# KyungMinJin/OTPose

Hardware: AMD Instinct MI355X
Metric: frames/sec at 384x288, 5-frame window, batch 16; heatmap max-abs delta vs ref (higher is better)
Workload: dtype f32 storage+accumulate / f16x3 split products; 1 GPU; BASELINE configs[1]: batch 16 x 5-frame x 384x288, HRNet-W48 + DCN warp + ConvVideoTransformer, fp32 forward (eval), seeded synthetic weights; clips_per_gpu=16, parallelism=dp1, outputs_finite=True

## Files before the change

### include/otpose_hip.h

```cpp
#ifndef OTPOSE_HIP_H
#define OTPOSE_HIP_H

#include <stddef.h>

#ifdef __cplusplus
extern "C" {
#endif

#define OTP_OK 0
#define OTP_ERR_BAD_ARG (-1)
#define OTP_ERR_UNSUPPORTED (-2)
#define OTP_ERR_LAUNCH (-3)
#define OTP_ERR_WORKSPACE (-4)

#define OTP_DTYPE_F32 0
#define OTP_DTYPE_F16 1
#define OTP_DTYPE_BF16 2
#define OTP_DTYPE_F64 3

#define OTP_ACT_NONE 0
#define OTP_ACT_RELU 1
#define OTP_ACT_GELU 2

int otp_version(void);

int otp_range_flag_read(int reset);
int otp_range_poison(void* out, size_t n, void* stream);

typedef struct otp_h16_conv_desc {
    int N, Cin, H, W, Cout, stride, act;
    int in_gtot, in_goff, out_gtot, out_goff, res_gtot, res_goff;
    float out_scale;
} otp_h16_conv_desc;
size_t otp_h8_bytes(int N, int C, int H, int W);
int otp_h8_pack(const void* in_f32, void* out_h8, int N, int C, int H, int W, int in_ctot, int in_coff, int out_gtot, int out_goff,
                void* stream);
int otp_h8_unpack(const void* in_h8, void* out_f32, int N, int C, int H, int W, int in_gtot, int in_goff, void* stream);
int otp_h16_conv3x3_supported(const otp_h16_conv_desc* desc);
size_t otp_h16_conv3x3_weight_bytes(int Cout, int Cin);
int otp_h16_conv3x3_pack_weight(const void* weight, const void* scale, void* wpacked, int Cout, int Cin, float pre, void* stream);
int otp_h16_conv3x3(const void* in_h8, const void* wpacked, const void* shift, const void* res_h8, void* out_h8,
                    const otp_h16_conv_desc* desc, void* stream);
int otp_h16_pointwise_supported(int Cin, int Cout);
size_t otp_h16_pointwise_weight_bytes(int Cin, int Cout);
int otp_h16_pointwise_pack(const void* w, const void* scale, const void* shift, void* packed, int Cin, int Cout, float pre,
                           void* stream);
int otp_h16_pointwise(const void* in_h8, const void* packed, const void* res_h8, void* out, int out_f32_nchw, int N, int Cin, int Cout,
                      int HW, int in_gtot, int in_goff, int res_gtot, int res_goff, int out_tot, int out_off, int relu,
                      float out_scale, void* stream);
int otp_h16_stem_supported(int B, int F, int H, int W, int Cout);
size_t otp_h16_stem_weight_bytes(int Cout);
int otp_h16_stem_pack(const void* w, const void* scale, const void* shift, void* packed, int Cout, void* stream);
int otp_h16_stem(const void* in, const void* packed, void* out_h8, int B, int F, int H, int W, int Cout, void* stream);
int otp_h16_upsample_add(const void* const* lows_h8, const int* factors, int nlow, const void* res_h8, void* out_h8, int N, int C,
                         int Hh, int Wh, int relu, void* stream);
size_t otp_mlp_h1_weight_bytes(int C, int HID);
int otp_mlp_h1_pack(const void* w1, const void* b1, const void* w2, void* packed, int C, int HID, void* stream);
int otp_ln_mlp_h1(const void* y, const void* ln_gamma, const void* ln_beta, float ln_eps, const void* packed, const void* scale,
                  const void* shift, void* out, int B, int C, int HID, int T, void* stream);
int otp_dense_h1(const void* const* x, const void* const* packed, const void* const* res, void* const* out, int nprob, int B, int C,
                 int T, void* stream);
int otp_qkv_front_h1(const void* x, const void* table, const void* packed_q, const void* packed_k, const void* packed_v, void* q,
                     void* k, void* v, int B, int C, int T, float eps, void* stream);

int otp_mdcn_forward(const void* x, const void* offset, const void* mask, const void* weight,
                     const void* bias, void* out,
                     int N, int C, int H, int W, int Cout, int kh, int kw,
                     int stride, int pad, int dil, int groups, int deformable_groups,
                     float alpha, float beta, int dtype, void* stream);

int otp_mdcn_forward_ex(const void* x, const void* offset, const void* mask, const void* weight, const void* bias, void* out,
                        int N, int C, int H, int W, int Cout, int kh, int kw, int stride_h, int stride_w, int pad_h, int pad_w,
                        int dil_h, int dil_w, int groups, int deformable_groups, float alpha, float beta, int dtype,
                        void* stream);

size_t otp_mdcn_backward_workspace(int N, int C, int H, int W, int Cout, int kh, int kw);
size_t otp_mdcn_backward_workspace_ex(int N, int C, int H, int W, int Cout, int kh, int kw, int stride_h, int stride_w, int pad_h,
                                      int pad_w, int dil_h, int dil_w, int groups, int deformable_groups, int dtype,
                                      int has_mask);
int otp_mdcn_backward(const void* x, const void* offset, const void* mask, const void* weight,
                      const void* grad_out, void* grad_x, void* grad_offset, void* grad_mask,
                      void* grad_weight, void* grad_bias, void* workspace, size_t workspace_bytes,
                      int N, int C, int H, int W, int Cout, int kh, int kw,
                      int stride, int pad, int dil, int groups, int deformable_groups,
                      int dtype, void* stream);
int otp_mdcn_backward_ex(const void* x, const void* offset, const void* mask, const void* weight, const void* grad_out,
                         void* grad_x, void* grad_offset, void* grad_mask, void* grad_weight, void* grad_bias, void* workspace,
                         size_t workspace_bytes, int N, int C, int H, int W, int Cout, int kh, int kw, int stride_h, int stride_w,
                         int pad_h, int pad_w, int dil_h, int dil_w, int groups, int deformable_groups, int dtype, void* stream);

int otp_deform_psroi_pool_forward(const void* data, const void* rois, const void* offset, void* out, void* out_count, int N, int C,
                                  int H, int W, int num_rois, int offset_channels, int no_trans, float spatial_scale,
                                  int out_channels, int group_size, int pooled_size, int part_size, int sample_per_part,
                                  float trans_std, int dtype, void* stream);
size_t otp_deform_psroi_pool_backward_workspace(int N, int C, int H, int W, int num_rois, int offset_channels, int no_trans,
                                                int out_channels, int group_size, int pooled_size, int part_size,
                                                int sample_per_part, int dtype);
int otp_deform_psroi_pool_backward(const void* grad_out, const void* data, const void* rois, const void* offset,
                                   const void* out_count, void* grad_input, void* grad_offset, int N, int C, int H, int W,
                                   int num_rois, int offset_channels, int no_trans, float spatial_scale, int out_channels,
                                   int group_size, int pooled_size, int part_size, int sample_per_part, float trans_std,
                                   void* workspace, size_t workspace_bytes, int dtype, void* stream);

typedef struct otp_conv_desc {
    int N, Cin, H, W, Cout, kh, kw, stride, pad, dil;
    int in_ctot, in_coff, in2_ctot, in2_coff, out_ctot, out_coff;
    int res_ctot, res_coff, res_up, act, Ho, Wo, frame_split;
    float out_scale;
    int res_layout;
} otp_conv_desc;

int otp_conv2d_set_tile(int MB, int PB, int WM, int WP);
int otp_conv2d_last_plan(int* out8);
int otp_conv2d_plan(const otp_conv_desc* desc, int* out8);
int otp_conv2d_pack_weight(const void* weight, void* wpacked, int Cout, int Cin, int kh, int kw, void* stream);
int otp_conv2d(const void* in, const void* in2, const void* wpacked, const void* scale, const void* shift,
               const void* res, void* out, const otp_conv_desc* desc, void* stream);

size_t otp_conv2d_wino_weight_bytes(int Cout, int Cin);
int otp_conv2d_wino_pack_weight(const void* weight, void* upacked, int Cout, int Cin, void* stream);
int otp_conv2d_wino_supported(const otp_conv_desc* desc);
int otp_conv2d_wino_last_plan(int* out4);
int otp_conv2d_wino(const void* in, const void* upacked, const void* scale, const void* shift, const void* res, void* out,
                    const otp_conv_desc* desc, void* stream);

int otp_conv3x3_small_supported(const otp_conv_desc* desc);
size_t otp_conv3x3_small_weight_bytes(int Cout, int Cin);
int otp_conv3x3_small_pack(const void* weight, void* wpacked, int Cout, int Cin, void* stream);
int otp_conv3x3_small(const void* in, const void* in2, const void* wpacked, const void* scale, const void* shift, void* out,
                      const otp_conv_desc* desc, void* stream);

size_t otp_conv2d_x3_weight_bytes(int Cout, int Cin, int k, int stride);
int otp_conv2d_x3_pack_weight(const void* weight, const void* scale, void* wpacked, int Cout, int Cin, int k, int stride,
                              void* stream);
int otp_conv2d_x3_supported(const otp_conv_desc* desc);
int otp_conv2d_x3(const void* in, const void* wpacked, const void* shift, const void* res, void* out,
                  const otp_conv_desc* desc, void* stream);

#define OTP_S8_F32_C4 1
#define OTP_S8_F32_NCHW 2
size_t otp_s8_bytes(int N, int C, int H, int W);
int otp_s8_pack(const void* in_f32, void* out_s8, void* out_c4, int N, int C, int H, int W, int in_ctot, int in_coff, void* stream);
int otp_s8_upsample_add(const void* const* lows, const int* factors, int nlow, const void* res, void* out_nchw, void* out_s8,
                        void* out_c4, int N, int C, int Hh, int Wh, int relu, int res_ctot, int res_coff, int out_ctot,
                        int out_coff, void* stream);
int otp_s8_upsample_add_ex(const void* const* lows, const int* factors, int nlow, const void* res, int res_layout, void* out_nchw,
                           void* out_s8, void* out_c4, int N, int C, int Hh, int Wh, int relu, int res_ctot, int res_coff,
                           int out_ctot, int out_coff, void* stream);
int otp_s8_unpack(const void* in_s8, void* out_f32, int N, int C, int H, int W, void* stream);
int otp_c4_unpack(const void* in_c4, void* out_f32, int N, int C, int H, int W, void* stream);
int otp_conv3x3_s8_supported(const otp_conv_desc* desc);
size_t otp_conv3x3_s8_weight_bytes(int Cout, int Cin);
int otp_conv3x3_s8_pack_weight(const void* weight, const void* scale, void* wpacked, int Cout, int Cin, void* stream);
int otp_conv3x3_s8(const void* in_s8, const void* wpacked, const void* shift, const void* res_c4, void* out_f32,
                   int out_f32_layout, void* out_s8, const otp_conv_desc* desc, void* stream);
int otp_conv3x3_s2_s8_supported(const otp_conv_desc* desc, int nchw_out);
int otp_conv3x3_s2_s8(const void* in_s8, const void* wpacked, const void* shift, const void* res_nchw, void* out_nchw,
                      void* out_s8, const otp_conv_desc* desc, void* stream);

int otp_conv2d_pack_weight_dgrad(const void* weight, void* wpacked, int Cout, int Cin, int kh, int kw, void* stream);
int otp_dilate(const void* in, void* out, int planes, int Hi, int Wi, int s, int H, int W, void* stream);
size_t otp_conv2d_wgrad_workspace(int Cin, int Cout);
int otp_conv2d_wgrad(const void* x, const void* grad_out, void* grad_weight, int N, int Cin, int H, int W, int Cout,
                     int kh, int kw, int stride, int pad, int dil, int x_ctot, int x_coff, int dy_ctot, int dy_coff,
                     void* workspace, size_t workspace_bytes, void* stream);
size_t otp_bn_workspace(int N, int C, int HW);
int otp_bn_train_forward(const void* x, const void* gamma, const void* beta, const void* res, void* y, void* save_mean,
                         void* save_rstd, void* running_mean, void* running_var, void* workspace, size_t workspace_bytes,
                         int N, int C, int HW, float eps, float momentum, int relu, int x_ctot, int x_coff, int res_ctot,
                         int res_coff, int y_ctot, int y_coff, void* stream);
int otp_bn_train_backward(const void* grad_y, const void* x, const void* y_relu, const void* save_mean,
                          const void* save_rstd, const void* gamma, void* grad_x, void* grad_res, void* grad_gamma,
                          void* grad_beta, void* workspace, size_t workspace_bytes, int N, int C, int HW, int dy_ctot,
                          int dy_coff, int x_ctot, int x_coff, int y_ctot, int y_coff, void* stream);
int otp_channel_sum(const void* a, void* out, void* workspace, size_t workspace_bytes, int N, int C, int HW, int a_ctot,
                    int a_coff, void* stream);

int otp_dcn_fused_supported(int Cin, int J, int H, int W, int ND);
size_t otp_dcn_fused_weight_bytes(int ND, int J);
int otp_dcn_fused_pack(const void* const* w_off, const void* const* w_mask, const void* const* w_dcn, const void* const* bias,
                       void* packed, int ND, int J, void* stream);
size_t otp_dcn_fused_workspace(int B, int H, int W);
int otp_dcn_fused_forward(const void* trans, const void* x, const void* packed, void* out, void* workspace,
                          size_t workspace_bytes, int B, int Cin, int J, int H, int W, const int* dilations, int ND, float alpha,
                          void* stream);

int otp_glue_total(const void* rough, void* total, void* squeezed, void* inter, void* flow_in, const void* pe,
                   int B, int J, int HW, void* stream);
int otp_glue_stack(const void* rough, const void* margin, const void* squeezed, const void* inter,
                   const void* ctx, const void* pe1, const void* pe2, void* x1, void* x2, void* prev_b,
                   int B, int J, int HW, void* stream);

int otp_glue_total_n(const void* rough, void* total, void* squeezed, void* inter, void* flow_in, const void* pe,
                     int B, int J, int HW, int F, void* stream);
int otp_glue_stack_n(const void* rough, const void* margin, const void* squeezed, const void* inter,
                     const void* ctx, const void* pe1, const void* pe2, void* x1, void* x2, void* prev_b,
                     int B, int J, int HW, int F, void* stream);

int otp_ln_channel(const void* x, const void* gamma, const void* beta, void* y, void* pool,
                   int B, int C, int T, float eps, void* stream);
int otp_dwconv_ln3(const void* x, const void* dwq, const void* dwk, const void* dwv,
                   const void* gq, const void* bq, const void* gk, const void* bk, const void* gv, const void* bv,
                   void* q, void* k, void* v, int B, int C, int T, int stride, float eps, void* stream);
size_t otp_chan_attn_workspace(int B, int C, int T, int n_head);
int otp_chan_attn(const void* q, const void* k, const void* v, void* out, void* workspace, size_t workspace_bytes,
                  int B, int C, int T, int n_head, float scale, void* stream);
int otp_upsample_linear(const void* x, void* out, int B, int C, int T, int f, int out_ctot, int out_coff, void* stream);

int otp_mlp_fused_supported(int C, int HID, int T);
size_t otp_mlp_fused_weight_bytes(int C, int HID);
int otp_mlp_fused_pack(const void* w1, const void* b1, const void* w2, void* packed, int C, int HID, void* stream);
int otp_mlp_fused(const void* x, const void* packed, const void* scale, const void* shift, const void* res, void* out,
                  int B, int C, int HID, int T, void* stream);
int otp_ln_mlp_fused(const void* y, const void* ln_gamma, const void* ln_beta, float ln_eps, const void* packed,
                     const void* scale, const void* shift, void* out, int B, int C, int HID, int T, void* stream);

int otp_dense_x3_supported(int C, int T);
size_t otp_dense_x3_weight_bytes(int C);
int otp_dense_x3_pack(const void* w, const void* scale, const void* shift, void* packed, int C, void* stream);
int otp_dense_x3(const void* const* x, const void* const* packed, const void* const* res, void* const* out, int nprob, int B,
                 int C, int T, void* stream);
int otp_dense_x3_pack_bf16p(const void* w, const void* scale, const void* shift, void* packed, int C, void* stream);
int otp_dense_x3_bf16p(const void* const* x, const void* const* packed, const void* const* res, void* const* out, int nprob, int B,
                 int C, int T, void* stream);
int otp_qkv_front_x3(const void* x, const void* table, const void* packed_q, const void* packed_k, const void* packed_v,
                     void* q, void* k, void* v, int B, int C, int T, float eps, void* stream);

int otp_stem_conv_x3_supported(int B, int F, int H, int W, int Cout);
size_t otp_stem_conv_x3_weight_bytes(int Cout);
int otp_stem_conv_x3_pack(const void* w, const void* scale, const void* shift, void* packed, int Cout, void* stream);
int otp_stem_conv_x3(const void* in, const void* packed, void* out, int B, int F, int H, int W, int Cout, void* stream);

int otp_pointwise_x3_supported(int Cin, int Cout, int T);
size_t otp_pointwise_x3_weight_bytes(int Cin, int Cout);
int otp_pointwise_x3_pack(const void* w, const void* scale, const void* shift, void* packed, int Cin, int Cout, void* stream);
int otp_pointwise_x3(const void* x, const void* packed, const void* res, void* out, int B, int Cin, int Cout, int T, int x_ctot,
                     int x_coff, int res_ctot, int res_coff, int out_ctot, int out_coff, int relu, void* stream);
int otp_pointwise_x3_s8_supported(int Cin, int Cout, int T);
size_t otp_pointwise_x3_s8_weight_bytes(int Cin, int Cout);
int otp_pointwise_x3_s8_pack(const void* w, const void* scale, const void* shift, void* packed, int Cin, int Cout, void* stream);
int otp_pointwise_x3_s8(const void* x, const void* packed, void* out_s8, int B, int Cin, int Cout, int T, int x_ctot, int x_coff,
                        int relu, void* stream);
int otp_pointwise_x3_s8_res(const void* x, const void* packed, const void* res, void* out_s8, int B, int Cin, int Cout, int T,
                            int x_ctot, int x_coff, int r_ctot, int r_coff, int relu, void* stream);
int otp_pointwise_x3_pair_supported(int Cin, int Cmid, int Cout2, int T);
size_t otp_pointwise_x3_pair_weight_bytes(int Cin, int Cmid, int Cout2);
int otp_pointwise_x3_pair_pack(const void* w1, const void* scale1, const void* shift1, const void* w2, const void* scale2,
                               const void* shift2, void* packed, int Cin, int Cmid, int Cout2, void* stream);
int otp_pointwise_x3_pair(const void* x, const void* packed, const void* res, void* out, void* out_s8, int B, int Cin, int Cmid,
                          int Cout2, int T, int x_ctot, int x_coff, int res_ctot, int res_coff, int out_ctot, int out_coff,
                          int relu1, int relu2, void* stream);

int otp_mlp_x3_supported(int C, int HID, int T);
size_t otp_mlp_x3_weight_bytes(int C, int HID);
int otp_mlp_x3_pack(const void* w1, const void* b1, const void* w2, void* packed, int C, int HID, void* stream);
int otp_mlp_x3(const void* x, const void* packed, const void* scale, const void* shift, const void* res, void* out, int B,
               int C, int HID, int T, void* stream);
int otp_ln_mlp_x3(const void* y, const void* ln_gamma, const void* ln_beta, float ln_eps, const void* packed,
                  const void* scale, const void* shift, void* out, int B, int C, int HID, int T, void* stream);

int otp_flow_block_supported(int C, int hidden, int T);
size_t otp_flow_front_param_floats(int C);
size_t otp_flow_back_param_floats(int C, int hidden);
int otp_flow_front(const void* x, const void* params, void* q, void* k, void* v, int B, int C, int T, float eps, void* stream);
int otp_flow_back(const void* x, const void* att, const void* params, void* out, int B, int C, int hidden, int T, float eps,
                  void* stream);

int otp_dense_cc_supported(int C, int T);
size_t otp_dense_cc_weight_bytes(int C);
int otp_dense_cc_pack(const void* w, const void* scale, const void* shift, void* packed, int C, void* stream);
int otp_dense_cc(const void* const* x, const void* const* packed, const void* const* res, void* const* out, int nprob,
                 int B, int C, int T, void* stream);

size_t otp_qkv_front_table_bytes(int C);
int otp_qkv_front_pack_table(const void* dwq, const void* dwk, const void* dwv, const void* gq, const void* bq,
                             const void* gk, const void* bk, const void* gv, const void* bv, void* table, int C,
                             void* stream);
int otp_qkv_front(const void* x, const void* table, const void* packed_q, const void* packed_k, const void* packed_v,
                  void* q, void* k, void* v, int B, int C, int T, float eps, void* stream);

int otp_upsample_add(const void* low, const void* res, void* out, int N, int C, int Hl, int Wl, int f, int relu,
                     int low_ctot, int low_coff, int res_ctot, int res_coff, int out_ctot, int out_coff, void* stream);
int otp_upsample_add_multi(const void* const* lows, const int* factors, int nlow, const void* res, void* out, int N, int C,
                           int Hh, int Wh, int relu, int res_ctot, int res_coff, int out_ctot, int out_coff, void* stream);

int otp_chan_attn_set_split(int on);
int otp_chan_attn_splits(int BH, int T);
int otp_chan_attn_scores(const void* a, const void* b, void* slabs, int BH, int hs, int T, void* stream);
int otp_chan_attn_apply(const void* v, const void* M, void* out, int BH, int hs, int T, void* stream);
int otp_chan_attn_scores_bf16p(const void* a, const void* b, void* slabs, int BH, int hs, int T, void* stream);
int otp_chan_attn_apply_bf16p(const void* v, const void* M, void* out, int BH, int hs, int T, void* stream);
int otp_transpose_scale(const void* in, void* out, int batches, int R, int Cc, float scale, void* stream);
int otp_softmax_backward(const void* slabs, const void* P, void* dS, void* dST, void* PT, int BH, int hs, int NS,
                         void* stream);
int otp_ln_channel_backward(const void* x, const void* grad_y, const void* gamma, void* grad_x, void* dy_xhat, int B, int C,
                            int T, float eps, void* stream);
size_t otp_ln_channel_backward_workspace(int B, int C, int T);
int otp_ln_channel_backward_params(const void* x, const void* grad_y, const void* gamma, void* grad_x, void* grad_gamma,
                                   void* grad_beta, void* workspace, size_t workspace_bytes, int B, int C, int T, float eps,
                                   void* stream);
int otp_dwconv3_forward(const void* x, const void* w, void* y, int B, int C, int T, int stride, void* stream);
int otp_dwconv3_backward(const void* x, const void* w, const void* grad_y, void* grad_x, void* grad_w, int B, int C, int T,
                         int stride, void* stream);
int otp_gelu_forward(const void* x, void* y, size_t n, void* stream);
int otp_gelu_backward(const void* x, const void* grad_y, void* grad_x, size_t n, void* stream);
int otp_maxpool3s2_forward(const void* x, void* y, int rows, int T, void* stream);
int otp_maxpool3s2_backward(const void* x, const void* grad_y, void* grad_x, int rows, int T, void* stream);
int otp_upsample_linear_backward(const void* grad_out, void* grad_x, int B, int C, int T, int f, int out_ctot, int out_coff,
                                 void* stream);

int otp_upsample_add_backward(const void* grad_out, const void* out_relu, void* grad_res, void* grad_low, int planes, int Hl,
                              int Wl, int f, void* stream);

int otp_axpby(const void* x, void* y, float alpha, float beta, size_t n, void* stream);

int otp_heatmap_decode(const void* heatmaps, void* preds, void* maxvals, const void* center, const void* scale,
                       int N, int J, int H, int W, int refine, void* stream);

int otp_heatmap_flip_decode(const void* heatmaps, const int* perm, void* merged, void* preds, void* maxvals,
                            const void* center, const void* scale, int B, int J, int H, int W, int shift, void* stream);
int otp_clip_mirror_pair(const void* x, void* out, int B, int C, int H, int W, void* stream);

int otp_pck_accuracy(const void* pred_coords, const void* target_coords, void* acc, void* cnt, int N, int J, int H, int W,
                     float thr, void* stream);

size_t otp_grad_sumsq_scratch(void);
int otp_grad_sumsq(const void* grad, size_t n, void* acc_f64, void* stream);
int otp_adamw_step(void* param, const void* grad, void* exp_avg, void* exp_avg_sq, size_t n, float lr, float beta1,
                   float beta2, float eps, float weight_decay, int step, const void* gradnorm_sq_f64, float max_norm,
                   void* stream);

int otp_frames_u8_to_clip(const void* frames_u8, void* out, int B, int F, int H, int W, float mean_r, float mean_g,
                          float mean_b, float std_r, float std_g, float std_b, void* stream);

int otp_crop_clips_u8(const void* pool_u8, int S, int Hp, int Wp, const void* frame_idx, const void* M, const void* flip,
                      void* out, int B, int F, int H, int W, float mean_r, float mean_g, float mean_b, float std_r,
                      float std_g, float std_b, void* stream);
int otp_crop_clips_blur_u8(const void* pool_u8, int S, int Hp, int Wp, const void* frame_idx, const void* M,
                           const void* flip, void* out, int B, int F, int H, int W, float mean_r, float mean_g,
                           float mean_b, float std_r, float std_g, float std_b, const void* blur, const void* blur_on,
                           void* stream);
int otp_crop_clips_pair_u8(const void* pool_u8, int S, int Hp, int Wp, const void* frame_idx, const void* M, void* out,
                           int B, int F, int H, int W, float mean_r, float mean_g, float mean_b, float std_r, float std_g,
                           float std_b, void* stream);
int otp_pose_targets(const void* joints, const void* vis, const void* M, const void* gauss, void* target,
                     void* target_weight, int B, int J, int W, int H, int w, int h, int sigma3, void* stream);

size_t otp_loss_workspace(int B, int J);
int otp_loss_st_ohkw_grads(const void* s, const void* t, const void* g, const void* w, void* flags, void* result,
                           void* grad_s, void* grad_t, void* grad_g, void* workspace, size_t workspace_bytes, int B, int J,
                           int HW, int topk, int flags_given, void* stream);
int otp_loss_st_ohkw(const void* s, const void* t, const void* g, const void* w, void* flags,
                     void* result, void* grad_s, void* grad_t, void* workspace, size_t workspace_bytes,
                     int B, int J, int HW, int topk, int flags_given, void* stream);
int otp_loss_joints_mse(const void* o, const void* g, const void* w, void* result, void* grad_o, void* workspace,
                        size_t workspace_bytes, int B, int J, int HW, int topk, int ohkm, int effective_num_joints,
                        void* stream);


typedef struct otp_nhwc_conv_desc {
    int N, H, W, Cin, Cout, kh, kw, stride, pad, dil;
    int out_mode;
} otp_nhwc_conv_desc;
size_t otp_nhwc_conv_weight_bytes(const otp_nhwc_conv_desc* desc);
int otp_nhwc_conv_stats_rows(const otp_nhwc_conv_desc* desc);
int otp_nhwc_conv_plan(const otp_nhwc_conv_desc* desc, int* out8);
int otp_nhwc_conv_pack(const void* weight, void* wpacked, const otp_nhwc_conv_desc* desc, int dgrad, void* stream);
size_t otp_nhwc_conv_pack_job_bytes(void);
int otp_nhwc_conv_pack_job(const void* weight, void* wpacked, const otp_nhwc_conv_desc* desc, int dgrad, void* job_host);
int otp_nhwc_conv_pack_batch(const void* jobs_device, int n_jobs, void* stream);
int otp_nhwc_conv_bf16(const void* x, const void* wpacked, const void* bias, void* out, void* stats,
                       const otp_nhwc_conv_desc* desc, void* stream);
int otp_nhwc_conv_bf16_res(const void* x, const void* wpacked, const void* bias, const void* res, void* out, void* stats,
                           const otp_nhwc_conv_desc* desc, void* stream);
size_t otp_nhwc_wgrad_workspace(const otp_nhwc_conv_desc* desc);
int otp_nhwc_wgrad_bf16(const void* x, const void* grad_out, void* grad_weight, void* workspace, size_t workspace_bytes,
                        const otp_nhwc_conv_desc* desc, void* stream);
int otp_nhwc_bn_finalize(const void* partials, int rows, int C, int CS, float count, const void* gamma, const void* beta,
                         void* mean, void* rstd, void* scale, void* shift, void* running_mean, void* running_var, float eps,
                         float momentum, void* stream);
int otp_nhwc_bn_apply(const void* x, const void* scale, const void* shift, const void* res, void* y, void* relu_mask,
                      size_t pixels, int CS, int relu, void* stream);
int otp_nhwc_conv_bn_bf16(const void* x, const void* wpacked, const void* res, void* conv_out, void* stats, void* vec,
                          const void* gamma, const void* beta, void* running_mean, void* running_var, float eps, float momentum,
                          void* y, void* relu_mask, int relu, const otp_nhwc_conv_desc* desc, void* stream);
size_t otp_nhwc_bn_backward_workspace(size_t pixels, int CS);
int otp_nhwc_bn_backward(const void* gy, const void* y, const void* x, const void* mean, const void* rstd, const void* gamma,
                         void* gx, void* gres, void* dgamma, void* dbeta, void* workspace, size_t workspace_bytes,
                         size_t pixels, int C, int CS, int relu, void* stream);
int otp_nhwc_upsample_add(const void* low, const void* res, void* out, int N, int H, int W, int CS, int f, int relu,
                          void* stream);
int otp_nhwc_upsample_add_backward(const void* gy, const void* out, void* gres, void* glow, int N, int Hl, int Wl, int CS,
                                   int f, int relu, void* stream);
int otp_nchw_f32_to_nhwc_bf16(const void* in, void* out, int N, int C, int H, int W, int frame_split, void* stream);
int otp_nhwc_bf16_to_nchw_f32(const void* in, void* out, int N, int C, int H, int W, void* stream);
int otp_nhwc_dilate(const void* in, void* out, int N, int Hi, int Wi, int s, int H, int W, int CS, void* stream);


int otp_scale_residual(const void* x, const void* a, const void* scale, const void* mask, void* out, int B, int C, int T,
                       void* stream);
size_t otp_scale_residual_backward_workspace(int B, int C, int T);
int otp_scale_residual_backward(const void* grad_out, const void* a, const void* scale, const void* mask, void* grad_a,
                                void* grad_scale, void* workspace, size_t workspace_bytes, int B, int C, int T, void* stream);


size_t otp_nhwc_channel_sum_workspace(size_t pixels, int CS);
int otp_nhwc_channel_sum(const void* g, void* out, void* workspace, size_t workspace_bytes, size_t pixels, int C, int CS,
                         void* stream);
int otp_gelu_bf16_forward(const void* x, void* y, size_t n, void* stream);
int otp_gelu_bf16_backward(const void* x, const void* grad_y, void* grad_x, size_t n, void* stream);
int otp_nhwc_mlp_fused_supported(const otp_nhwc_conv_desc* desc);
int otp_nhwc_mlp_up_bf16(const void* x, const void* wpacked, const void* bias, void* pre, void* act, void* keep_bits, float p,
// ... 28 lines not shown
```

### otpose_amd/csrc/densex.hip

```cpp
#include "x3.h"
#ifndef OTP_ENTRY
#define OTP_ENTRY(name) name
#endif

namespace {

constexpr int dx_ks(int C) { return (C + 31) / 32; }
constexpr int dx_block_bytes(int C) { return (dx_ks(C) * 2 * 1024 + 128 + 4095) / 4096 * 4096; }

__global__ void densex_pack_kernel(const float* __restrict__ w, const float* __restrict__ scale, const float* __restrict__ shift,
                                   unsigned char* __restrict__ packed, int C) {
    const int KS = dx_ks(C), MT = (C + 15) / 16, BLKB = dx_block_bytes(C), units = BLKB / 16;
    const int idx = blockIdx.x * blockDim.x + threadIdx.x;
    if (idx >= MT * units) return;
    const int mt = idx / units, u = idx - mt * units;
    otp_u32x4 o = {0u, 0u, 0u, 0u};
    if (u < KS * 2 * 64) {
        const int frag = u >> 6, lane = u & 63, row = 16 * mt + (lane & 15), kq = lane >> 4, ks = frag >> 1;
        float v[8];
#pragma unroll
        for (int j = 0; j < 8; ++j) {
            const int c = 32 * ks + 8 * kq + j;
            v[j] = (row < C && c < C) ? w[(size_t)row * C + c] : 0.f;
        }
        otp_x3x8 hi, lo;
        otp_x3_split8(v, hi, lo);
        o = __builtin_bit_cast(otp_u32x4, (frag & 1) ? lo : hi);
    } else if (u < KS * 2 * 64 + 8) {
        const int k = (u - KS * 2 * 64) * 4;
        float v[4];
#pragma unroll
        for (int i = 0; i < 4; ++i) {
            const int e = k + i, c = 16 * mt + (e & 15);
            v[i] = c < C ? (e < 16 ? (scale ? scale[c] : 1.f) : (shift ? shift[c] : 0.f)) : 0.f;
        }
        o = (otp_u32x4){__builtin_bit_cast(uint32_t, v[0]), __builtin_bit_cast(uint32_t, v[1]), __builtin_bit_cast(uint32_t, v[2]),
                    __builtin_bit_cast(uint32_t, v[3])};
    }
    reinterpret_cast<otp_u32x4*>(packed)[idx] = o;
}

template <int C, bool RES, bool H1 = false>
__device__ __forceinline__ void dx_project(const otp_x3x8 (&Xh)[dx_ks(C)][2], const otp_x3x8 (&Xl)[dx_ks(C)][2],
                                           const unsigned char* __restrict__ packed, unsigned char* lds,
                                           const float* __restrict__ res, float* __restrict__ out, size_t base, int T, int tok,
                                           bool valid, unsigned* rflag) {
    constexpr int KS = dx_ks(C), MT = (C + 15) / 16, BLKB = dx_block_bytes(C);
    bool bad = false;
    const int lane = threadIdx.x & 63, kq = lane >> 4;
    const unsigned plane = (unsigned)((size_t)C * T * sizeof(float));
    const otp_rsrc ro = make_rsrc32(out + base, plane);
    const otp_rsrc rr = make_rsrc32(RES && res ? res + base : out, RES && res ? plane : 0u);
#pragma unroll 1
    for (int mt = 0; mt < MT; ++mt) {
        int voff[4];
        otp_f32x2 r[4];
#pragma unroll
        for (int i = 0; i < 4; ++i) {
            const int c = 16 * mt + 4 * kq + i;
            voff[i] = (valid && c < C) ? (c * T + tok) * 4 : -16;
            if (RES) r[i] = __builtin_bit_cast(otp_f32x2, __builtin_amdgcn_raw_buffer_load_b64(rr, voff[i], 0, 0));
        }
        asm volatile("" ::: "memory");
        if (mt + 1 < MT) otp_lds_stage<256, BLKB>(packed + (size_t)(mt + 1) * BLKB, lds + ((mt + 1) & 1) * BLKB);
        asm volatile("" ::: "memory");
        const unsigned char* P = lds + (mt & 1) * BLKB;
        otp_f32x4 acc0 = {0.f, 0.f, 0.f, 0.f}, acc1 = {0.f, 0.f, 0.f, 0.f};
#pragma unroll
        for (int ks = 0; ks < KS; ++ks) {
            const otp_x3x8 ah = *reinterpret_cast<const otp_x3x8*>(P + (ks * 2) * 1024 + lane * 16);
            if constexpr (!H1) {
                const otp_x3x8 al = *reinterpret_cast<const otp_x3x8*>(P + (ks * 2 + 1) * 1024 + lane * 16);
                acc0 = OTP_X3_MFMA(al, Xh[ks][0], acc0, 0, 0, 0);
                acc1 = OTP_X3_MFMA(al, Xh[ks][1], acc1, 0, 0, 0);
                acc0 = OTP_X3_MFMA(ah, Xl[ks][0], acc0, 0, 0, 0);
                acc1 = OTP_X3_MFMA(ah, Xl[ks][1], acc1, 0, 0, 0);
            }
            acc0 = OTP_X3_MFMA(ah, Xh[ks][0], acc0, 0, 0, 0);
            acc1 = OTP_X3_MFMA(ah, Xh[ks][1], acc1, 0, 0, 0);
        }
        const otp_f32x4 sc = *reinterpret_cast<const otp_f32x4*>(P + KS * 2048 + 16 * kq);
        const otp_f32x4 sh = *reinterpret_cast<const otp_f32x4*>(P + KS * 2048 + 64 + 16 * kq);
#pragma unroll
        for (int i = 0; i < 4; ++i) {
            otp_f32x2 v = {acc0[i] * sc[i] + sh[i], acc1[i] * sc[i] + sh[i]};
            if (RES) v += r[i];
            bad |= otp_out_of_range(v.x);
                bad |= otp_out_of_range(v.y);
            __builtin_amdgcn_raw_buffer_store_b64(__builtin_bit_cast(otp_u32x2, v), ro, voff[i], 0, 0);
        }
        if (mt + 1 < MT) {
            asm volatile("s_waitcnt vmcnt(4)" ::: "memory");
            __builtin_amdgcn_s_barrier();
            asm volatile("" ::: "memory");
        }
    }
    otp_range_report(rflag, bad, OTP_RANGE_DENSEX);
}

struct DxArgs {
    const float* x[3];
    const unsigned char* packed[3];
    const float* res[3];
    float* out[3];
};

template <int C, bool H1 = false>
__global__ __launch_bounds__(256, 2) void densex_cc_kernel(DxArgs A, int T, int tiles_per_b, unsigned* rflag) {
    constexpr int KS = dx_ks(C), BLKB = dx_block_bytes(C);
    __shared__ __attribute__((aligned(16))) unsigned char lds[2 * BLKB];
    const int tid = threadIdx.x, lane = tid & 63, wave = tid >> 6, kq = lane >> 4, n = lane & 15;
    const int b = blockIdx.x / tiles_per_b, tile = blockIdx.x - b * tiles_per_b;
    const int tok = tile * 128 + wave * 32 + 2 * n;
    const bool valid = tok < T;
    const size_t base = (size_t)b * C * T;
    const float* __restrict__ x = A.x[blockIdx.y];
    otp_lds_stage<256, BLKB>(A.packed[blockIdx.y], lds);
    otp_x3x8 Xh[KS][2], Xl[KS][2];
#pragma unroll
    for (int ks = 0; ks < KS; ++ks) {
        float v0[8], v1[8];
#pragma unroll
        for (int j = 0; j < 8; ++j) {
            const int c = 32 * ks + 8 * kq + j;
            const bool live = 32 * ks + 24 + j < C || c < C;
            const otp_f32x2 v = *reinterpret_cast<const otp_f32x2*>(x + base + (size_t)(live ? c : 0) * T + (valid ? tok : T - 2));
            v0[j] = live ? v.x : 0.f;
            v1[j] = live ? v.y : 0.f;
        }
        otp_x3_split8(v0, Xh[ks][0], Xl[ks][0]);
        otp_x3_split8(v1, Xh[ks][1], Xl[ks][1]);
    }
    __syncthreads();
    dx_project<C, true, H1>(Xh, Xl, A.packed[blockIdx.y], lds, A.res[blockIdx.y], A.out[blockIdx.y], base, T, tok, valid, rflag);
}

struct QxArgs {
    const unsigned char* packed[3];
    float* out[3];
};

template <int C, bool H1 = false>
__global__ __launch_bounds__(256, C <= 136 ? 3 : 1) void qkvx_front_kernel(const float* __restrict__ x, const float* __restrict__ table,
                                                            QxArgs A, int T, int tiles_per_b, float eps, unsigned* rflag) {
    constexpr int KS = dx_ks(C), BLKB = dx_block_bytes(C), TAB = 3 * C * 8;
    __shared__ __attribute__((aligned(16))) unsigned char lds[2 * BLKB];
    __shared__ __attribute__((aligned(16))) float tab[TAB];
    const int tid = threadIdx.x, lane = tid & 63, wave = tid >> 6, kq = lane >> 4, n = lane & 15;
    const int b = blockIdx.x / tiles_per_b, tile = blockIdx.x - b * tiles_per_b;
    const int tok = tile * 128 + wave * 32 + 2 * n;
    const bool valid = tok < T;
    const int tokc = valid ? tok : T - 2;
    const bool l_ok = tokc >= 1, r_ok = tokc + 2 < T;
    const size_t base = (size_t)b * C * T;
    const otp_rsrc rx = make_rsrc(x + base, (size_t)C * T * sizeof(float));
    constexpr float inv_c = 1.f / (float)C;
    const int vb0 = (8 * kq * T + tokc) * 4;
    for (int i = tid; i < TAB / 4; i += 256)
        reinterpret_cast<otp_f32x4*>(tab)[i] = reinterpret_cast<const otp_f32x4*>(table)[i];
    __syncthreads();

    for (int p = (int)blockIdx.y; p <= (int)blockIdx.y; ++p) {
        otp_lds_stage<256, BLKB>(A.packed[p], lds);
        const float* tp = tab + p * C * 8;
        float X0[KS][8], X1[KS][8];
        float s0 = 0.f, s1 = 0.f;
#pragma unroll
        for (int ks = 0; ks < KS; ++ks) {
#pragma unroll
            for (int j = 0; j < 8; ++j) {
                const int c = 32 * ks + 8 * kq + j;
                const bool live = 32 * ks + 24 + j < C || c < C;
                const int so = (32 * ks + j) * T * 4;
                const otp_f32x2 m = __builtin_bit_cast(otp_f32x2, __builtin_amdgcn_raw_buffer_load_b64(rx, live ? vb0 : -16, so, 0));
                const float la = bload(rx, live ? vb0 - 4 : -16, so), ld = bload(rx, live ? vb0 + 8 : -16, so);
                const float a = l_ok ? la : 0.f, d = r_ok ? ld : 0.f;
                const otp_f32x4 w = *reinterpret_cast<const otp_f32x4*>(tp + (live ? c : 0) * 8);
                X0[ks][j] = live ? w[0] * a + w[1] * m.x + w[2] * m.y : 0.f;
                X1[ks][j] = live ? w[0] * m.x + w[1] * m.y + w[2] * d : 0.f;
                s0 += X0[ks][j];
                s1 += X1[ks][j];
            }
        }
        const float m0 = otp_kslot_sum(s0) * inv_c, m1 = otp_kslot_sum(s1) * inv_c;
        float v0 = 0.f, v1 = 0.f;
#pragma unroll
        for (int ks = 0; ks < KS; ++ks)
#pragma unroll
            for (int j = 0; j < 8; ++j) {
                const bool live = 32 * ks + 24 + j < C || 32 * ks + 8 * kq + j < C;
                X0[ks][j] = live ? X0[ks][j] - m0 : 0.f;
                X1[ks][j] = live ? X1[ks][j] - m1 : 0.f;
                v0 += X0[ks][j] * X0[ks][j];
                v1 += X1[ks][j] * X1[ks][j];
            }
        const float r0 = 1.f / sqrtf(otp_kslot_sum(v0) * inv_c + eps), r1 = 1.f / sqrtf(otp_kslot_sum(v1) * inv_c + eps);
        otp_x3x8 Xh[KS][2], Xl[KS][2];
#pragma unroll
        for (int ks = 0; ks < KS; ++ks) {
#pragma unroll
            for (int j = 0; j < 8; ++j) {
                const int c = 32 * ks + 8 * kq + j;
                const bool live = 32 * ks + 24 + j < C || c < C;
                const float g = tp[(live ? c : 0) * 8 + 3], be = tp[(live ? c : 0) * 8 + 4];
                X0[ks][j] = live ? X0[ks][j] * r0 * g + be : 0.f;
                X1[ks][j] = live ? X1[ks][j] * r1 * g + be : 0.f;
            }
            otp_x3_split8(X0[ks], Xh[ks][0], Xl[ks][0]);
            otp_x3_split8(X1[ks], Xh[ks][1], Xl[ks][1]);
        }
        __syncthreads();
        dx_project<C, false, H1>(Xh, Xl, A.packed[p], lds, nullptr, A.out[p], base, T, tok, valid, rflag);
    }
}

}

#ifndef OTP_X3_GRAD_COPY
extern "C" int otp_dense_x3_supported(int C, int T) { return ((C == 136 || C == 204) && T > 0 && T % 2 == 0) ? 1 : 0; }

extern "C" size_t otp_dense_x3_weight_bytes(int C) {
    if (C <= 0 || C % 4) return 0;
    return (size_t)((C + 15) / 16) * dx_block_bytes(C);
}
#endif

extern "C" int OTP_ENTRY(otp_dense_x3_pack)(const void* w, const void* scale, const void* shift, void* packed, int C, void* stream) {
    if (!w || !packed) return OTP_ERR_BAD_ARG;
    const size_t bytes = otp_dense_x3_weight_bytes(C);
    if (!bytes) return OTP_ERR_UNSUPPORTED;
    const int total = (int)(bytes / 16);
    hipLaunchKernelGGL(densex_pack_kernel, dim3(otp_ceil_div(total, 256)), dim3(256), 0, static_cast<hipStream_t>(stream),
                       static_cast<const float*>(w), static_cast<const float*>(scale), static_cast<const float*>(shift),
                       static_cast<unsigned char*>(packed), C);
    return otp_launch_status();
}

namespace {
int dx_dense_launch(const void* const* x, const void* const* packed, const void* const* res, void* const* out, int nprob, int B, int C,
                    int T, void* stream, bool h1) {
    if (!x || !packed || !out || nprob < 1 || nprob > 3 || B <= 0) return OTP_ERR_BAD_ARG;
    if (!otp_dense_x3_supported(C, T)) return OTP_ERR_UNSUPPORTED;
    DxArgs a = {};
    for (int i = 0; i < nprob; ++i) {
        a.x[i] = static_cast<const float*>(x[i]);
        a.packed[i] = static_cast<const unsigned char*>(packed[i]);
        a.res[i] = res ? static_cast<const float*>(res[i]) : nullptr;
        a.out[i] = static_cast<float*>(out[i]);
        if (!a.x[i] || !a.packed[i] || !a.out[i]) return OTP_ERR_BAD_ARG;
        if ((reinterpret_cast<uintptr_t>(a.x[i]) | reinterpret_cast<uintptr_t>(a.res[i]) | reinterpret_cast<uintptr_t>(a.out[i])) & 7 ||
            reinterpret_cast<uintptr_t>(a.packed[i]) & 15)
            return OTP_ERR_BAD_ARG;
    }
    const int tiles = otp_ceil_div(T, 128);
    const dim3 grid((unsigned)(B * tiles), (unsigned)nprob);
    auto st = static_cast<hipStream_t>(stream);
    if (C == 204) {
        if (h1) hipLaunchKernelGGL((densex_cc_kernel<204, true>), grid, dim3(256), 0, st, a, T, tiles, otp_range_word());
        else hipLaunchKernelGGL((densex_cc_kernel<204, false>), grid, dim3(256), 0, st, a, T, tiles, otp_range_word());
    } else {
        if (h1) hipLaunchKernelGGL((densex_cc_kernel<136, true>), grid, dim3(256), 0, st, a, T, tiles, otp_range_word());
        else hipLaunchKernelGGL((densex_cc_kernel<136, false>), grid, dim3(256), 0, st, a, T, tiles, otp_range_word());
    }
    return otp_launch_status();
}
}

extern "C" int OTP_ENTRY(otp_dense_x3)(const void* const* x, const void* const* packed, const void* const* res, void* const* out,
                            int nprob, int B, int C, int T, void* stream) {
    return dx_dense_launch(x, packed, res, out, nprob, B, C, T, stream, false);
}

#ifndef OTP_X3_GRAD_COPY
extern "C" int otp_dense_h1(const void* const* x, const void* const* packed, const void* const* res, void* const* out, int nprob, int B,
                            int C, int T, void* stream) {
    return dx_dense_launch(x, packed, res, out, nprob, B, C, T, stream, true);
}
#endif

#ifndef OTP_X3_GRAD_COPY
namespace {
int dx_qkv_launch(const void* x, const void* table, const void* packed_q, const void* packed_k, const void* packed_v, void* q, void* k,
                  void* v, int B, int C, int T, float eps, void* stream, bool h1) {
    if (!x || !table || !packed_q || !packed_k || !packed_v || !q || !k || !v || B <= 0) return OTP_ERR_BAD_ARG;
    if (!otp_dense_x3_supported(C, T)) return OTP_ERR_UNSUPPORTED;
    if ((reinterpret_cast<uintptr_t>(x) | reinterpret_cast<uintptr_t>(q) | reinterpret_cast<uintptr_t>(k) |
         reinterpret_cast<uintptr_t>(v)) & 7 ||
        (reinterpret_cast<uintptr_t>(table) | reinterpret_cast<uintptr_t>(packed_q) | reinterpret_cast<uintptr_t>(packed_k) |
         reinterpret_cast<uintptr_t>(packed_v)) & 15)
        return OTP_ERR_BAD_ARG;
    if ((size_t)C * T * sizeof(float) >= (1ull << 31)) return OTP_ERR_UNSUPPORTED;
    QxArgs a;
    a.packed[0] = static_cast<const unsigned char*>(packed_q); a.packed[1] = static_cast<const unsigned char*>(packed_k);
    a.packed[2] = static_cast<const unsigned char*>(packed_v);
    a.out[0] = static_cast<float*>(q); a.out[1] = static_cast<float*>(k); a.out[2] = static_cast<float*>(v);
    const int tiles = otp_ceil_div(T, 128);
    const dim3 grid((unsigned)(B * tiles), 3u);
    auto st = static_cast<hipStream_t>(stream);
    auto xf = static_cast<const float*>(x), tf = static_cast<const float*>(table);
    if (C == 204) {
        if (h1) hipLaunchKernelGGL((qkvx_front_kernel<204, true>), grid, dim3(256), 0, st, xf, tf, a, T, tiles, eps, otp_range_word());
        else hipLaunchKernelGGL((qkvx_front_kernel<204, false>), grid, dim3(256), 0, st, xf, tf, a, T, tiles, eps, otp_range_word());
    } else {
        if (h1) hipLaunchKernelGGL((qkvx_front_kernel<136, true>), grid, dim3(256), 0, st, xf, tf, a, T, tiles, eps, otp_range_word());
        else hipLaunchKernelGGL((qkvx_front_kernel<136, false>), grid, dim3(256), 0, st, xf, tf, a, T, tiles, eps, otp_range_word());
    }
    return otp_launch_status();
}
}

extern "C" int otp_qkv_front_x3(const void* x, const void* table, const void* packed_q, const void* packed_k,
                                const void* packed_v, void* q, void* k, void* v, int B, int C, int T, float eps, void* stream) {
    return dx_qkv_launch(x, table, packed_q, packed_k, packed_v, q, k, v, B, C, T, eps, stream, false);
}

extern "C" int otp_qkv_front_h1(const void* x, const void* table, const void* packed_q, const void* packed_k,
                                const void* packed_v, void* q, void* k, void* v, int B, int C, int T, float eps, void* stream) {
    return dx_qkv_launch(x, table, packed_q, packed_k, packed_v, q, k, v, B, C, T, eps, stream, true);
}
#endif
```

### otpose_amd/csrc/mlpx.hip

```cpp
#include <math.h>
#include <stdlib.h>

#include "x3.h"

namespace {

__device__ __forceinline__ float mx_gelu_h(float x) {
    const float xc = __builtin_amdgcn_fmed3f(x, -4.2f, 4.2f), s2 = xc * xc;
    float r = 4.711542158e-11f;
    r = r * s2 + -4.627826316e-09f;
    r = r * s2 + 2.017249231e-07f;
    r = r * s2 + -5.191738396e-06f;
    r = r * s2 + 8.882890530e-05f;
    r = r * s2 + -1.080400373e-03f;
    r = r * s2 + 9.720675326e-03f;
    r = r * s2 + -6.618899545e-02f;
    r = r * s2 + 3.988157481e-01f;
    return x * (xc * r + 0.5f);
}

__device__ __forceinline__ otp_x3x8 mx_half8(const float (&v)[8]) {
    uint32_t h[4];
#pragma unroll
    for (int i = 0; i < 4; ++i) h[i] = __builtin_bit_cast(uint32_t, __builtin_convertvector((otp_f32x2){v[2 * i], v[2 * i + 1]}, otp_x3x2));
    return __builtin_bit_cast(otp_x3x8, (otp_u32x4){h[0], h[1], h[2], h[3]});
}

constexpr int mx_ks1(int C) { return (C + 31) / 32; }
constexpr int mx_mt(int C) { return (C + 15) / 16; }
constexpr int mx_w1_bytes(int C, int PS = 2) { return 2 * mx_ks1(C) * PS * 1024; }
constexpr int mx_w2_bytes(int C, int PS = 2) { return mx_mt(C) * PS * 1024; }
constexpr int mx_block_bytes(int C, int PS = 2) { return (mx_w1_bytes(C, PS) + mx_w2_bytes(C, PS) + 128 + 1023) / 1024 * 1024; }

__global__ void mlpx_pack_kernel(const float* __restrict__ w1, const float* __restrict__ b1, const float* __restrict__ w2,
                                 unsigned char* __restrict__ packed, int C, int HID, int PS) {
    const int KS1 = mx_ks1(C), W1B = mx_w1_bytes(C, PS), W2B = mx_w2_bytes(C, PS), BLKB = mx_block_bytes(C, PS);
    const int units = BLKB / 16;
    const int idx = blockIdx.x * blockDim.x + threadIdx.x;
    if (idx >= ((HID + 31) / 32) * units) return;
    const int hb = idx / units, u = idx - hb * units;
    otp_u32x4 o = {0u, 0u, 0u, 0u};
    float v[8] = {0.f, 0.f, 0.f, 0.f, 0.f, 0.f, 0.f, 0.f};
    if (u < (W1B + W2B) / 16) {
        const int frag = u >> 6, lane = u & 63, row = lane & 15, kq = lane >> 4;
        const bool lo_part = PS == 2 && (frag & 1);
        if (u < W1B / 16) {
            const int f2 = frag / PS, tile = f2 / KS1, ks = f2 - tile * KS1;
            const int hid = 32 * hb + 16 * tile + row;
#pragma unroll
            for (int j = 0; j < 8; ++j) {
                const int c = 32 * ks + 8 * kq + j;
                if (c < C && hid < HID) v[j] = w1[(size_t)hid * C + c];
            }
        } else {
            const int mt = (frag - W1B / 1024) / PS, c = 16 * mt + row;
#pragma unroll
            for (int j = 0; j < 8; ++j) {
                const int hid = 32 * hb + (j < 4 ? 4 * kq + j : 16 + 4 * kq + j - 4);
                if (c < C && hid < HID) v[j] = w2[(size_t)c * HID + hid];
            }
        }
        otp_x3x8 hi, lo;
        otp_x3_split8(v, hi, lo);
        o = __builtin_bit_cast(otp_u32x4, lo_part ? lo : hi);
    } else if (u < (W1B + W2B) / 16 + 8) {
        const int k = (u - (W1B + W2B) / 16) * 4;
        const bool in = 32 * hb + k < HID;
        o = in ? (otp_u32x4){__builtin_bit_cast(uint32_t, b1[32 * hb + k]), __builtin_bit_cast(uint32_t, b1[32 * hb + k + 1]),
                         __builtin_bit_cast(uint32_t, b1[32 * hb + k + 2]), __builtin_bit_cast(uint32_t, b1[32 * hb + k + 3])}
               : (otp_u32x4){0u, 0u, 0u, 0u};
    }
    reinterpret_cast<otp_u32x4*>(packed)[idx] = o;
}

template <int C, int HID, int NTHR, bool LN, int NT, bool H1 = false>
__device__ __forceinline__ void mlpx_pass(const float* __restrict__ x, const unsigned char* __restrict__ packed,
                                          const float* __restrict__ scale, const float* __restrict__ shift,
                                          const float* __restrict__ res, float* __restrict__ out, int T, size_t base, int tok0,
                                          unsigned char* lds, const float* __restrict__ ln_gamma,
                                          const float* __restrict__ ln_beta, float ln_eps, unsigned* rflag) {
    constexpr int KS1 = mx_ks1(C), MT = mx_mt(C), HB = (HID + 31) / 32, PS = H1 ? 1 : 2;
    constexpr int W1B = mx_w1_bytes(C, PS), W2B = mx_w2_bytes(C, PS), BLKB = mx_block_bytes(C, PS);
    const int lane = threadIdx.x & 63, kq = lane >> 4, n = lane & 15;
    const int tok = tok0 + NT * n;
    const bool valid = tok < T;

    otp_lds_stage<NTHR, BLKB>(packed, lds);

    float X[KS1][8][NT];
#pragma unroll
    for (int ks = 0; ks < KS1; ++ks)
#pragma unroll
        for (int j = 0; j < 8; ++j) {
            const int c = 32 * ks + 8 * kq + j;
            const bool live = 32 * ks + 24 + j < C || c < C;
            const float* src = x + base + (size_t)(live ? c : 0) * T + (valid ? tok : T - NT);
            if (NT == 2) {
                const otp_f32x2 v = *reinterpret_cast<const otp_f32x2*>(src);
                X[ks][j][0] = live ? v.x : 0.f;
                X[ks][j][NT - 1] = live ? v.y : 0.f;
            } else {
                X[ks][j][0] = live ? *src : 0.f;
            }
        }
    if (LN) {
        constexpr float inv_c = 1.f / (float)C;
#pragma unroll
        for (int t = 0; t < NT; ++t) {
            float s0 = 0.f;
#pragma unroll
            for (int ks = 0; ks < KS1; ++ks)
#pragma unroll
                for (int j = 0; j < 8; ++j) s0 += X[ks][j][t];
            const float m0 = otp_kslot_sum(s0) * inv_c;
            float v0 = 0.f;
#pragma unroll
            for (int ks = 0; ks < KS1; ++ks)
#pragma unroll
                for (int j = 0; j < 8; ++j) {
                    const bool live = 32 * ks + 24 + j < C || 32 * ks + 8 * kq + j < C;
                    X[ks][j][t] = live ? X[ks][j][t] - m0 : 0.f;
                    v0 += X[ks][j][t] * X[ks][j][t];
                }
            const float r0 = 1.f / sqrtf(otp_kslot_sum(v0) * inv_c + ln_eps);
#pragma unroll
            for (int ks = 0; ks < KS1; ++ks)
#pragma unroll
                for (int j = 0; j < 8; ++j) {
                    const int c = 32 * ks + 8 * kq + j;
                    const bool live = 32 * ks + 24 + j < C || c < C;
                    X[ks][j][t] = live ? X[ks][j][t] * r0 * ln_gamma[live ? c : 0] + ln_beta[live ? c : 0] : 0.f;
                }
        }
    }
    otp_x3x8 Xh[KS1][NT], Xl[H1 ? 1 : KS1][NT];
#pragma unroll
    for (int ks = 0; ks < KS1; ++ks)
#pragma unroll
        for (int t = 0; t < NT; ++t) {
            float v[8];
#pragma unroll
            for (int j = 0; j < 8; ++j) v[j] = X[ks][j][t];
            if constexpr (H1) Xh[ks][t] = mx_half8(v);
            else otp_x3_split8(v, Xh[ks][t], Xl[H1 ? 0 : ks][t]);
        }
    otp_f32x4 Y[MT][NT];
#pragma unroll
    for (int mt = 0; mt < MT; ++mt)
#pragma unroll
        for (int t = 0; t < NT; ++t) Y[mt][t] = otp_f32x4{0.f, 0.f, 0.f, 0.f};
    __syncthreads();

    for (int hb = 0; hb < HB; ++hb) {
        if (hb + 1 < HB) otp_lds_stage<NTHR, BLKB>(packed + (size_t)(hb + 1) * BLKB, lds + ((hb + 1) & 1) * BLKB);
        const unsigned char* P1 = lds + (hb & 1) * BLKB + lane * 16;
        const unsigned char* P2 = P1 + W1B;
        const float* PB = reinterpret_cast<const float*>(lds + (hb & 1) * BLKB + W1B + W2B);
        otp_f32x4 H[2][NT];
#pragma unroll
        for (int tile = 0; tile < 2; ++tile) {
#pragma unroll
            for (int t = 0; t < NT; ++t) H[tile][t] = *reinterpret_cast<const otp_f32x4*>(PB + 16 * tile + 4 * kq);
#pragma unroll
            for (int ks = 0; ks < KS1; ++ks) {
                const otp_x3x8 ah = *reinterpret_cast<const otp_x3x8*>(P1 + ((tile * KS1 + ks) * PS) * 1024);
                if constexpr (H1) {
#pragma unroll
                    for (int t = 0; t < NT; ++t) H[tile][t] = OTP_X3_MFMA(ah, Xh[ks][t], H[tile][t], 0, 0, 0);
                } else {
                    const otp_x3x8 al = *reinterpret_cast<const otp_x3x8*>(P1 + ((tile * KS1 + ks) * 2 + 1) * 1024);
#pragma unroll
                    for (int t = 0; t < NT; ++t) {
                        H[tile][t] = OTP_X3_MFMA(al, Xh[ks][t], H[tile][t], 0, 0, 0);
                        H[tile][t] = OTP_X3_MFMA(ah, Xl[H1 ? 0 : ks][t], H[tile][t], 0, 0, 0);
                        H[tile][t] = OTP_X3_MFMA(ah, Xh[ks][t], H[tile][t], 0, 0, 0);
                    }
                }
            }
        }
        otp_x3x8 Gh[NT], Gl[NT];
#pragma unroll
        for (int t = 0; t < NT; ++t) {
            if constexpr (H1) {
                const float v[8] = {mx_gelu_h(H[0][t][0]), mx_gelu_h(H[0][t][1]), mx_gelu_h(H[0][t][2]), mx_gelu_h(H[0][t][3]),
                                    mx_gelu_h(H[1][t][0]), mx_gelu_h(H[1][t][1]), mx_gelu_h(H[1][t][2]), mx_gelu_h(H[1][t][3])};
                Gh[t] = mx_half8(v);
            } else {
                const otp_f32x2 g0 = otp_gelu2(otp_f32x2{H[0][t][0], H[0][t][1]}), g1 = otp_gelu2(otp_f32x2{H[0][t][2], H[0][t][3]});
                const otp_f32x2 g2 = otp_gelu2(otp_f32x2{H[1][t][0], H[1][t][1]}), g3 = otp_gelu2(otp_f32x2{H[1][t][2], H[1][t][3]});
                const float v[8] = {g0.x, g0.y, g1.x, g1.y, g2.x, g2.y, g3.x, g3.y};
                otp_x3_split8(v, Gh[t], Gl[t]);
            }
        }
#pragma unroll
        for (int mt = 0; mt < MT; ++mt) {
            const otp_x3x8 ah = *reinterpret_cast<const otp_x3x8*>(P2 + (mt * PS) * 1024);
            if constexpr (H1) {
#pragma unroll
                for (int t = 0; t < NT; ++t) Y[mt][t] = OTP_X3_MFMA(ah, Gh[t], Y[mt][t], 0, 0, 0);
            } else {
                const otp_x3x8 al = *reinterpret_cast<const otp_x3x8*>(P2 + (mt * 2 + 1) * 1024);
#pragma unroll
                for (int t = 0; t < NT; ++t) {
                    Y[mt][t] = OTP_X3_MFMA(al, Gh[t], Y[mt][t], 0, 0, 0);
                    Y[mt][t] = OTP_X3_MFMA(ah, Gl[t], Y[mt][t], 0, 0, 0);
                    Y[mt][t] = OTP_X3_MFMA(ah, Gh[t], Y[mt][t], 0, 0, 0);
                }
            }
        }
        __syncthreads();
    }

    {
        bool bad = false;
#pragma unroll
        for (int mt = 0; mt < MT; ++mt)
#pragma unroll
            for (int t = 0; t < NT; ++t)
#pragma unroll
                for (int i = 0; i < 4; ++i) bad |= otp_out_of_range(Y[mt][t][i]);
        otp_range_report(rflag, bad, OTP_RANGE_MLPX);
    }
    if (!valid) return;
#pragma unroll
    for (int mt = 0; mt < MT; ++mt) {
#pragma unroll
        for (int i = 0; i < 4; ++i) {
            const int c = 16 * mt + 4 * kq + i;
            if (c < C) {
                const size_t o = base + (size_t)c * T + tok;
                const float sc = scale[c], sh = shift[c];
                if (NT == 2) {
                    const otp_f32x2 r = *reinterpret_cast<const otp_f32x2*>(res + o);
                    otp_f32x2 v;
                    v.x = r.x + Y[mt][0][i] * sc + sh;
                    v.y = r.y + Y[mt][NT - 1][i] * sc + sh;
                    *reinterpret_cast<otp_f32x2*>(out + o) = v;
                } else {
                    out[o] = res[o] + Y[mt][0][i] * sc + sh;
                }
            }
        }
    }
}

template <int C, int HID, int WAVES, bool LN, int NT, bool H1 = false>
__global__ __launch_bounds__(WAVES * 64, (NT == 1 && (C <= 136 || H1)) ? 4 : 2) void mlpx_kernel(
    const float* __restrict__ x, const unsigned char* __restrict__ packed, const float* __restrict__ scale,
    const float* __restrict__ shift, const float* __restrict__ res, float* __restrict__ out, int T, int tiles_per_b,
    const float* __restrict__ ln_gamma, const float* __restrict__ ln_beta, float ln_eps, unsigned* rflag) {
    extern __shared__ __attribute__((aligned(16))) unsigned char mx_lds[];
    const int wave = threadIdx.x >> 6;
    const int b = blockIdx.x / tiles_per_b, tile = blockIdx.x - b * tiles_per_b;
    mlpx_pass<C, HID, WAVES * 64, LN, NT, H1>(x, packed, scale, shift, res, out, T, (size_t)b * C * T,
                                          tile * (WAVES * 16 * NT) + wave * 16 * NT, mx_lds, ln_gamma, ln_beta, ln_eps, rflag);
}

template <int C, int HID, bool LN>
__global__ __launch_bounds__(512, 2) void mlpx_balanced_kernel(
    const float* __restrict__ x, const unsigned char* __restrict__ packed, const float* __restrict__ scale,
    const float* __restrict__ shift, const float* __restrict__ res, float* __restrict__ out, int T, int wgs_per_b,
    const float* __restrict__ ln_gamma, const float* __restrict__ ln_beta, float ln_eps, unsigned* rflag) {
    extern __shared__ __attribute__((aligned(16))) unsigned char mx_lds[];
    const int wave = __builtin_amdgcn_readfirstlane(threadIdx.x >> 6);
    const int b = blockIdx.x / wgs_per_b, part = blockIdx.x - b * wgs_per_b;
    const size_t base = (size_t)b * C * T;
    const int t0 = part * (27 * 16);
    mlpx_pass<C, HID, 512, LN, 2>(x, packed, scale, shift, res, out, T, base, t0 + wave * 32, mx_lds, ln_gamma, ln_beta, ln_eps, rflag);
    if (wave < 3) {
        mlpx_pass<C, HID, 512, LN, 2>(x, packed, scale, shift, res, out, T, base, t0 + (16 + 2 * wave) * 16, mx_lds, ln_gamma,
                                      ln_beta, ln_eps, rflag);
    } else {
        const int tile = wave == 3 ? 25 : (wave == 7 ? 26 : 18 + wave);
        mlpx_pass<C, HID, 512, LN, 1>(x, packed, scale, shift, res, out, T, base, t0 + tile * 16, mx_lds, ln_gamma, ln_beta,
                                      ln_eps, rflag);
    }
}

}

extern "C" int otp_mlp_x3_supported(int C, int HID, int T) {
    return (((C == 136 && HID == 544) || (C == 204 && HID == 816)) && T > 0 && T % 2 == 0) ? 1 : 0;
}

extern "C" size_t otp_mlp_x3_weight_bytes(int C, int HID) {
    if (C <= 0 || C % 4 || HID <= 0 || HID % 16) return 0;
    return (size_t)((HID + 31) / 32) * mx_block_bytes(C);
}

extern "C" size_t otp_mlp_h1_weight_bytes(int C, int HID) {
    if (C <= 0 || C % 4 || HID <= 0 || HID % 16) return 0;
    return (size_t)((HID + 31) / 32) * mx_block_bytes(C, 1);
}

extern "C" int otp_mlp_x3_pack(const void* w1, const void* b1, const void* w2, void* packed, int C, int HID, void* stream) {
    if (!w1 || !b1 || !w2 || !packed) return OTP_ERR_BAD_ARG;
    const size_t bytes = otp_mlp_x3_weight_bytes(C, HID);
    if (!bytes) return OTP_ERR_UNSUPPORTED;
    const int total = (int)(bytes / 16);
    hipLaunchKernelGGL(mlpx_pack_kernel, dim3(otp_ceil_div(total, 256)), dim3(256), 0, static_cast<hipStream_t>(stream),
                       static_cast<const float*>(w1), static_cast<const float*>(b1), static_cast<const float*>(w2),
                       static_cast<unsigned char*>(packed), C, HID, 2);
    return otp_launch_status();
}

extern "C" int otp_mlp_h1_pack(const void* w1, const void* b1, const void* w2, void* packed, int C, int HID, void* stream) {
    if (!w1 || !b1 || !w2 || !packed) return OTP_ERR_BAD_ARG;
    const size_t bytes = otp_mlp_h1_weight_bytes(C, HID);
    if (!bytes) return OTP_ERR_UNSUPPORTED;
    const int total = (int)(bytes / 16);
    hipLaunchKernelGGL(mlpx_pack_kernel, dim3(otp_ceil_div(total, 256)), dim3(256), 0, static_cast<hipStream_t>(stream),
                       static_cast<const float*>(w1), static_cast<const float*>(b1), static_cast<const float*>(w2),
                       static_cast<unsigned char*>(packed), C, HID, 1);
    return otp_launch_status();
}

namespace {
int mlpx_launch(const void* x, const void* packed, const void* scale, const void* shift, const void* res, void* out,
                const void* ln_gamma, const void* ln_beta, float ln_eps, int B, int C, int HID, int T, void* stream, bool h1 = false) {
    if (!x || !packed || !scale || !shift || !res || !out || B <= 0) return OTP_ERR_BAD_ARG;
    if (h1 && !ln_gamma) return OTP_ERR_UNSUPPORTED;
    if (!otp_mlp_x3_supported(C, HID, T)) return OTP_ERR_UNSUPPORTED;
    if ((reinterpret_cast<uintptr_t>(x) | reinterpret_cast<uintptr_t>(res) | reinterpret_cast<uintptr_t>(out)) & 7 ||
        reinterpret_cast<uintptr_t>(packed) & 15)
        return OTP_ERR_BAD_ARG;
    auto f = [](const void* p) { return static_cast<const float*>(p); };
    auto pk = static_cast<const unsigned char*>(packed);
    if (C == 204) {
        constexpr int WAVES = 8;
        const size_t lds204 = 2 * (size_t)mx_block_bytes(204, h1 ? 1 : 2);
        const int tiles = otp_ceil_div(T, WAVES * 16);
        auto kern = h1 ? mlpx_kernel<204, 816, WAVES, true, 1, true>
                       : (ln_gamma ? mlpx_kernel<204, 816, WAVES, true, 1> : mlpx_kernel<204, 816, WAVES, false, 1>);
        OTP_ALLOW_BIG_LDS(kern, lds204);
        hipLaunchKernelGGL(kern, dim3((unsigned)(B * tiles)), dim3(WAVES * 64), lds204, static_cast<hipStream_t>(stream), f(x), pk,
                           f(scale), f(shift), f(res), static_cast<float*>(out), T, tiles, f(ln_gamma), f(ln_beta), ln_eps, otp_range_word());
        return otp_launch_status();
    }
    const size_t lds = 2 * (size_t)mx_block_bytes(136, h1 ? 1 : 2);
    const char* bal = getenv("OTP_MLP_BALANCED");
    const bool bal_off = bal && bal[0] == '0', bal_force = bal && bal[0] == '2';
    const char* e1 = getenv("OTP_MLP_NT1");
    const bool nt1 = !(e1 && e1[0] == '0');
    if (h1 || (nt1 && !bal_force)) {
        constexpr int WAVES = 8;
        const int tiles = otp_ceil_div(T, WAVES * 16);
        auto kern = h1 ? mlpx_kernel<136, 544, WAVES, true, 1, true>
                       : (ln_gamma ? mlpx_kernel<136, 544, WAVES, true, 1> : mlpx_kernel<136, 544, WAVES, false, 1>);
        OTP_ALLOW_BIG_LDS(kern, lds);
        hipLaunchKernelGGL(kern, dim3((unsigned)(B * tiles)), dim3(WAVES * 64), lds, static_cast<hipStream_t>(stream), f(x), pk,
                           f(scale), f(shift), f(res), static_cast<float*>(out), T, tiles, f(ln_gamma), f(ln_beta), ln_eps, otp_range_word());
        return otp_launch_status();
    }
    if (!bal_off && T % (27 * 16) == 0 && (bal_force || (long)B * (T / (27 * 16)) >= 192)) {
        auto bk = ln_gamma ? mlpx_balanced_kernel<136, 544, true> : mlpx_balanced_kernel<136, 544, false>;
        OTP_ALLOW_BIG_LDS(bk, lds);
        const int per_b = T / (27 * 16);
        hipLaunchKernelGGL(bk, dim3((unsigned)(B * per_b)), dim3(512), lds, static_cast<hipStream_t>(stream), f(x), pk,
                           f(scale), f(shift), f(res), static_cast<float*>(out), T, per_b, f(ln_gamma), f(ln_beta), ln_eps, otp_range_word());
        return otp_launch_status();
    }
    constexpr int WAVES = 8;
    const int tiles = otp_ceil_div(T, WAVES * 32);
    auto kern = ln_gamma ? mlpx_kernel<136, 544, WAVES, true, 2> : mlpx_kernel<136, 544, WAVES, false, 2>;
    OTP_ALLOW_BIG_LDS(kern, lds);
    hipLaunchKernelGGL(kern, dim3((unsigned)(B * tiles)), dim3(WAVES * 64), lds, static_cast<hipStream_t>(stream), f(x), pk,
                       f(scale), f(shift), f(res), static_cast<float*>(out), T, tiles, f(ln_gamma), f(ln_beta), ln_eps, otp_range_word());
    return otp_launch_status();
}
}

extern "C" int otp_mlp_x3(const void* x, const void* packed, const void* scale, const void* shift, const void* res, void* out,
                          int B, int C, int HID, int T, void* stream) {
    return mlpx_launch(x, packed, scale, shift, res, out, nullptr, nullptr, 0.f, B, C, HID, T, stream);
}

extern "C" int otp_ln_mlp_x3(const void* y, const void* ln_gamma, const void* ln_beta, float ln_eps, const void* packed,
                             const void* scale, const void* shift, void* out, int B, int C, int HID, int T, void* stream) {
    if (!ln_gamma || !ln_beta) return OTP_ERR_BAD_ARG;
    return mlpx_launch(y, packed, scale, shift, y, out, ln_gamma, ln_beta, ln_eps, B, C, HID, T, stream);
}

extern "C" int otp_ln_mlp_h1(const void* y, const void* ln_gamma, const void* ln_beta, float ln_eps, const void* packed,
                             const void* scale, const void* shift, void* out, int B, int C, int HID, int T, void* stream) {
    if (!ln_gamma || !ln_beta) return OTP_ERR_BAD_ARG;
    return mlpx_launch(y, packed, scale, shift, y, out, ln_gamma, ln_beta, ln_eps, B, C, HID, T, stream, true);
}
```

### otpose_amd/engine.py

```python
from __future__ import annotations

import ctypes
import dataclasses
import os
import sys
import warnings
from typing import Callable, List, Optional, Tuple

import torch

from . import hip, ops
from .ops import ACT_GELU, ACT_NONE, ACT_RELU, View

def _pair(v):
    return (int(v), int(v)) if isinstance(v, int) else (int(v[0]), int(v[1]))


def plain_conv(cv, k, stride=1, pad="same", dil=1, groups=1, bias=False, cin=None, cout=None) -> bool:
    if pad == "same":
        pad = (dil or 1) * (k // 2)
    return (cv.kernel_size == (k, k) and (stride is None or cv.stride == (stride, stride))
            and (pad is None or tuple(cv.padding) == (pad, pad)) and (dil is None or tuple(cv.dilation) == (dil, dil))
            and (groups is None or cv.groups == groups) and (bias is None or (cv.bias is not None) == bias)
            and (cin is None or cv.in_channels == cin) and (cout is None or cv.out_channels == cout))


@dataclasses.dataclass(frozen=True)
class Routes:
    use_graph: bool = True
    use_winograd: bool = True
    use_x3: bool = True
    use_dcn_fused: bool = True
    use_s8: bool = True
    use_flow_fused: bool = True
    use_small_conv: bool = True
    use_fused_mlp: bool = True
    fuse_shortcut: bool = True
    fuse_upsample: bool = True
    use_dense_cc: bool = True
    use_qkv_front: bool = True
    use_pointx: bool = True
    pointx_fuse: bool = True
    pointx_any: bool = False
    multi_stream: bool = True
    f32_tail: int = 0
    h16_tail: bool = True
    range_check: str = "defer"
    s8_residual: bool = True
    s8_lazy_nchw: bool = True
    s8_stride2: bool = True
    t1_s8: bool = True
    l1_s8: bool = True
    l1_pair: bool = True
    stem_x3: bool = True
    chain_modules: bool = True
    up_any_width: bool = True
    conv_log: bool = False
    poison: Optional[Tuple[int, int]] = None
    te_serial: bool = False

    @classmethod
    def from_env(cls) -> "Routes":
        env = os.environ.get
        on = lambda name: env("OTPOSE_" + name, "1") != "0"
        x3 = env("OTPOSE_CONV_MATH", "x3") != "f32"
        poison = env("OTPOSE_POISON")
        return cls(use_graph=on("HIP_GRAPH"), use_winograd=on("WINOGRAD"), use_x3=x3, use_dcn_fused=x3 and on("DCN_FUSED"),
                   use_s8=x3 and on("S8"), use_flow_fused=on("FLOW_FUSED"), use_small_conv=on("SMALL_CONV"),
                   use_fused_mlp=on("FUSED_MLP"), fuse_shortcut=on("FUSE_SHORTCUT"), fuse_upsample=on("FUSE_UPSAMPLE"),
                   use_dense_cc=on("DENSE_CC"), use_qkv_front=on("QKV_FRONT"), use_pointx=x3 and on("POINTX"),
                   pointx_fuse=on("POINTX_FUSE"), pointx_any=env("OTPOSE_POINTX_ANY", "0") == "1", multi_stream=on("STREAMS"),
                   f32_tail=int(env("OTPOSE_F32_TAIL", "0")) if x3 else 0, h16_tail=on("H16_TAIL"),
                   range_check=env("OTPOSE_RANGE_CHECK", "defer"), s8_residual=on("S8_RESIDUAL"), s8_lazy_nchw=on("S8_LAZY_NCHW"),
                   s8_stride2=on("S8_STRIDE2"), t1_s8=on("T1_S8"), l1_s8=on("L1_S8"), l1_pair=on("L1_PAIR"), stem_x3=on("STEM_X3"),
                   chain_modules=on("CHAIN_MODULES"), up_any_width=on("UP_ANY_WIDTH"), conv_log=bool(env("OTPOSE_CONV_LOG")),
                   poison=tuple(int(v) for v in poison.split(":")) if poison else None, te_serial=env("OTPOSE_TE_SERIAL") == "1")

    @property
    def lazy_nchw(self) -> bool:
        return self.s8_residual and self.s8_lazy_nchw


class Aux:
    __slots__ = ("s8", "c4", "nchw_needed")

    def __init__(self, s8=None, c4=None, nchw_needed=False):
        self.s8, self.c4, self.nchw_needed = s8, c4, nchw_needed


class InferenceEngine:
    h16 = False

    def __init__(self, model, batch: int, device, use_graph: bool | None = None, stream_set: int = 0, inp=None, margin=None):
        routes = Routes.from_env()
        self._init(device, routes, routes.use_graph if use_graph is None else use_graph, stream_set)
        self.B = batch
        self.model = model
        cfg = model.cfg
        self.J = model.num_joints
        self.F = getattr(model, "window_frames", 5)
        self.W_img, self.H_img = cfg.MODEL.IMAGE_SIZE
        self.h, self.w = model.pe_h, model.pe_w
        self._given = (inp, margin)
        self.param_version = self._param_version()
        with torch.no_grad():
            self._build()

    def _init(self, device, routes: Routes, use_graph: bool, stream_set: int = 0):
        device = torch.device(device)
        if device.type != "cuda" or not torch.cuda.is_available():
            raise RuntimeError("otpose_amd.OTPose runs on an MI355X through libotpose_hip.so; "
                               f"got device '{device}' (there is no CPU or PyTorch-op fallback)")
        self.lib, self.dev, self.routes = hip.lib(), device, routes
        self.model, self.B, self.inp, self.margin = None, 0, None, None
        self.ops: List[Callable] = []
        self._pair_s8 = {}
        self.l1_pairs = 0
        self._aux = {}
        self._keep = []
        self._bufs = []
        self._stream = None
        self.use_graph, self.graph = use_graph, None
        self._exact = False
        self._sid = 0
        self._side = hip.side_streams(device, 3, 4 * stream_set) if routes.multi_stream else []

    @classmethod
    def bare(cls, device, multi_stream=False):
        self = cls.__new__(cls)
        self._init(device, dataclasses.replace(Routes.from_env(), multi_stream=bool(multi_stream)), use_graph=False)
        return self

    use_x3 = property(lambda self: self.routes.use_x3)
    use_dcn_fused = property(lambda self: self.routes.use_dcn_fused)
    multi_stream = property(lambda self: self.routes.multi_stream)
    f32_tail = property(lambda self: self.routes.f32_tail)
    range_check = property(lambda self: self.routes.range_check)
    half_products = property(lambda self: self.h16 and self.routes.use_x3 and self.routes.h16_tail)

    @property
    def s8_here(self) -> bool:
        return self.routes.use_s8 and not self._exact

    @property
    def s2_here(self) -> bool:
        return self.routes.use_s8 and not self._exact and self.routes.s8_stride2

    def matches(self, x) -> bool:
        return (x.shape[0] == self.B and x.device == self.dev and tuple(x.shape[2:]) == (self.H_img, self.W_img)
                and self._param_version() == self.param_version)

    def matches_shape(self, b, c, h, w, dev) -> bool:
        return (b == self.B and dev == self.dev and (h, w) == (self.H_img, self.W_img) and c == 3 * self.F
                and self._param_version() == self.param_version)

    def _param_version(self):
        ts = getattr(self, "_tracked", None)
        if ts is None:
            ts = self._tracked = list(self.model.parameters()) + list(self.model.buffers())
        v = a = 0
        for t in ts:
            v += t._version
            a ^= t.data_ptr()
        return (len(ts), v, a)

    def new(self, *shape):
        t = torch.empty(shape, dtype=torch.float32, device=self.dev)
        rng = self.routes.poison
        if rng and rng[0] <= len(self._bufs) < rng[1]:
            t.fill_(float("nan"))
        self._bufs.append(t)
        return t

    def dev_param(self, t):
        t = t.detach().to(self.dev, torch.float32).contiguous()
        self._keep.append(t)
        return t

    @staticmethod
    def winograd_pays(cin, cout):
        cout16 = (cout + 15) // 16 * 16
        if cin == 64 and cout16 == 64:
            return True
        return cin >= 32 and cin % 8 == 0 and cout16 >= 48 and ((cout16 + 47) // 48) * 48 <= 1.15 * cout16

    def _emit(self, fn):
        self.ops.append((fn, self._sid))

    def fork(self, sids):
        if not self.multi_stream:
            return
        sids = [s for s in sids if 0 < s <= len(self._side)]

        def run():
            main = torch.cuda.current_stream(self.dev)
            for s_ in sids:
                self._side[s_ - 1].wait_stream(main)
        self.ops.append((run, -1))

    def join(self, sids):
        if not self.multi_stream:
            return
        sids = [s for s in sids if 0 < s <= len(self._side)]

        def run():
            main = torch.cuda.current_stream(self.dev)
            for s_ in sids:
                main.wait_stream(self._side[s_ - 1])
        self.ops.append((run, -1))

    def on_stream(self, sid):
        self._sid = sid if (self.multi_stream and 0 <= sid <= len(self._side)) else 0

    def call(self, fn, name, *args):
        def run():
            hip.check(fn(*args, self._stream), name)
        self._emit(run)

    def call_lazy_nchw(self, aux: Aux, fn, name, args_of, unpack=None):
        full, lean = args_of(True), args_of(False)
        if unpack is None:
            def run():
                hip.check(fn(*(full if aux.nchw_needed else lean), self._stream), name)
        else:
            s8_unpack = self.lib.otp_s8_unpack

            def run():
                hip.check(fn(*lean, self._stream), name)
                if aux.nchw_needed:
                    hip.check(s8_unpack(*unpack, self._stream), "otp_s8_unpack")
        self._emit(run)

    def _bn_fold(self, bn, bias=None):
        g, b = self.dev_param(bn.weight), self.dev_param(bn.bias)
        mu, var = self.dev_param(bn.running_mean), self.dev_param(bn.running_var)
        sc = (g / torch.sqrt(var + bn.eps)).contiguous()
        sh = b - mu * sc
        if bias is not None:
            sh = sh + self.dev_param(bias) * sc
        sh = sh.contiguous()
        self._keep += [sc, sh]
        return sc, sh

    def conv(self, inp: View, weight, out: View, stride=1, pad=0, dil=1, bn=None, bias=None, act=ACT_NONE,
             res: View = None, in2: View = None, res_up=1, frame_split=0, cin=None, scale=None, shift=None):
        for v_ in (inp, in2, res):
            self._needs_nchw(v_)
        r = self.routes
        w = self.dev_param(weight)
        if w.dim() == 3:
            w = w.unsqueeze(-1)
        cout, cin_w, kh, kw = w.shape
        if bn is not None:
            sc, sh = self._bn_fold(bn, bias)
        else:
            sc = self.dev_param(scale) if scale is not None else None
            sh = shift if shift is not None else bias
            sh = self.dev_param(sh) if sh is not None else None
        d = ops.conv_desc(inp, out, cout, kh, kw, stride, pad, dil, act, in2, res, res_up, frame_split, cin)
        self._keep.append(d)
        L = self.lib
        if r.conv_log:
            route = ("x3" if r.use_x3 and in2 is None and (kh, kw) in ((3, 3), (1, 1)) and ops.x3_supported(d) else
                     "wino" if r.use_winograd and in2 is None and self.winograd_pays(cin_w, cout) and ops.wino_supported(d)
                     else "direct")
            print(f"conv {d.N}x{d.Cin}->{cout} k{kh} s{stride} p{pad} d{dil} {d.H}x{d.W} in2={in2 is not None} "
                  f"res={res is not None} up={res_up} fs={frame_split} {route}", file=sys.stderr)
        if r.use_small_conv and in2 is not None and res is None and (kh, kw) == (3, 3) and ops.small_conv_supported(d):
            wc = ops.pack_small_conv_weight(w)
            self._keep.append(wc)
# ... 335 lines not shown
                last = idx == len(terms) - 1 and not ups
                act = ACT_RELU if last else ACT_NONE
                res = xs[i] if y is None else y
                fl = mod.fuse_layers[i][j]
                tgt = y if y is not None else View(self.new(*xs[i].t.shape))
                if j > i:
                    f = 2 ** (j - i)
                    if f >= 2 and ((xs[j].t.shape[3] * f) % 4 == 0 or r.up_any_width):
                        low = self.conv_bn(xs[j], fl[0], fl[1], ACT_NONE)
                        if act == ACT_RELU and low.coff == 0 and low.C == low.ctot and self.fuse_s8([low], [f], res, tgt):
                            y = tgt
                            continue
                        self._needs_nchw(res)
                        self.call(self.lib.otp_upsample_add, "otp_upsample_add", *ops.upsample_add_args(low, res, tgt, f, act == ACT_RELU))
                        y = tgt
                    else:
                        y = self.conv_bn(xs[j], fl[0], fl[1], act, res=res, out=tgt, res_up=f)
                else:
                    chain = [(fl[k][0], fl[k][1], k < len(fl) - 1) for k in range(len(fl))]
                    if self.s2_chain_s8(chain, xs[j], act, res=res, out=tgt) is not None:
                        y = tgt
                        continue
                    t = xs[j]
                    for k in range(len(fl) - 1):
                        t = self.conv_bn(t, fl[k][0], fl[k][1], ACT_RELU)
                    y = self.conv_bn(t, fl[-1][0], fl[-1][1], act, res=res, out=tgt)
            if ups:
                res = xs[i] if y is None else y
                tgt = y if y is not None else View(self.new(*xs[i].t.shape))
                lows = [self.conv_bn(xs[j], mod.fuse_layers[i][j][0], mod.fuse_layers[i][j][1], ACT_NONE) for j in ups]
                factors = [2 ** (j - i) for j in ups]
                if self.fuse_s8(lows, factors, res, tgt):
                    outs.append(tgt)
                    continue
                self._needs_nchw(res)
                args, arrays = ops.upsample_add_multi_args(lows, factors, res, tgt, relu=True)
                self._keep += arrays
                self.call(self.lib.otp_upsample_add_multi, "otp_upsample_add_multi", *args)
                y = tgt
            outs.append(y)
        self.on_stream(0)
        if join_out:
            self.join(range(1, len(mod.fuse_layers)))
        return outs

    def hr_stages(self, net, x, width_change, new_branch, module, before_fork=None):
        ys = [x]
        for s in (2, 3, 4):
            trans = getattr(net, f"transition{s - 1}")
            live = [i for i, tr in enumerate(trans) if tr is not None]
            if before_fork is not None:
                before_fork(s, ys)
            self.fork(range(1, len(live)))
            xs = []
            for i, tr in enumerate(trans):
                if tr is None:
                    xs.append(ys[i])
                    continue
                self.on_stream(live.index(i))
                if isinstance(tr[0], torch.nn.Conv2d):
                    xs.append(width_change(s, ys[i], tr))
                else:
                    xs.append(new_branch(s, ys[-1], tr))
            self.on_stream(0)
            self.join(range(1, len(live)))
            ys = xs
            mods = list(getattr(net, f"stage{s}"))
            cont = False
            for mi, mod in enumerate(mods):
                fork_in, nxt = not cont, (mods[mi + 1] if mi + 1 < len(mods) else None)
                cont = (self.routes.chain_modules and nxt is not None and len(mod.fuse_layers) == nxt.num_branches
                        and mod.num_branches > 1)
                ys = module(s, mi, len(mods), mod, ys, fork_in, not cont)
        return ys

    def hrnet(self, net, x_in: View) -> View:
        c1 = net.conv1
        r = self.routes
        n_in, c_in, h_in, w_in = x_in.t.shape
        if (r.use_x3 and r.stem_x3 and x_in.coff == 0 and x_in.C == c_in and c_in == 3 * self.F and plain_conv(c1, 3, stride=2, cin=3)
                and ops.stem_conv_x3_supported(n_in, self.F, h_in, w_in, c1.out_channels)):
            sc, sh = self._bn_fold(net.bn1)
            pk = ops.pack_stem_conv_x3(self.dev_param(c1.weight), sc, sh)
            self._keep.append(pk)
            x = View(self.new(self.F * n_in, c1.out_channels, (h_in - 1) // 2 + 1, (w_in - 1) // 2 + 1))
            self.call(self.lib.otp_stem_conv_x3, "otp_stem_conv_x3", *ops.stem_conv_x3_args(x_in.t, pk, x.t, self.F, c1.out_channels))
        else:
            x = self.conv_bn(x_in, net.conv1, net.bn1, ACT_RELU, frame_split=self.B, cin=3)
        blocks = list(net.layer1)
        b0 = blocks[0]
        if (r.fuse_shortcut and b0.downsample is not None and plain_conv(b0.conv3, 1) and plain_conv(b0.downsample[0], 1)):
            n, _, h, w = x.t.shape
            c2 = net.conv2
            ho = (h + 2 * c2.padding[0] - c2.kernel_size[0]) // c2.stride[0] + 1
            wo = (w + 2 * c2.padding[0] - c2.kernel_size[0]) // c2.stride[0] + 1
            cx, cy = c2.out_channels, b0.conv2.out_channels
            cat = self.new(n, cx + cy, ho, wo)
            xin = self.conv_bn(x, c2, net.bn2, ACT_RELU, out=View(cat, 0, cx))
            if self.conv1_conv2_s8(xin, b0.conv1, b0.bn1, b0.conv2, b0.bn2, out=View(cat, cx, cy)) is None:
                y = self.conv_bn(xin, b0.conv1, b0.bn1, ACT_RELU)
                self.conv_bn(y, b0.conv2, b0.bn2, ACT_RELU, out=View(cat, cx, cy))

            def fold(conv, bn):
                sc, sh = self._bn_fold(bn)
                return self.dev_param(conv.weight) * sc[:, None, None, None], sh
            wd, shd = fold(b0.downsample[0], b0.downsample[1])
            w3, sh3 = fold(b0.conv3, b0.bn3)
            cout = b0.conv3.out_channels
            wcat, ones, shcat = torch.cat([wd, w3], 1), torch.ones(cout, device=self.dev), shd + sh3
            x = self.pointx_pair(View(cat), wcat, ones, shcat, None, blocks[1]) if len(blocks) > 1 else None
            if x is None:
                x = self.conv(View(cat), wcat, View(self.new(n, cout, ho, wo)), scale=ones, shift=shcat, act=ACT_RELU)
            blocks = blocks[1:]
        else:
            x = self.conv_bn(x, net.conv2, net.bn2, ACT_RELU)
        for bi, blk in enumerate(blocks):
            x = self.bottleneck(blk, x, s8_only=self.s2_here and r.t1_s8 and bi == len(blocks) - 1,
                                nxt=blocks[bi + 1] if bi + 1 < len(blocks) else None)

        def t1_s8(s):
            return s == 2 and self.s8_here and r.t1_s8

        def before_fork(s, ys):
            if (s >= 3 or t1_s8(s)) and self.s2_here:
                self.s8_image(ys[-1], want_c4=s >= 3 and not r.s8_residual)

        def width_change(s, x, tr):
            y = self.conv_bn_s8(x, tr[0], tr[1], ACT_RELU) if t1_s8(s) else None
            return y if y is not None else self.conv_bn(x, tr[0], tr[1], ACT_RELU)

        def new_branch(s, z, tr):
            zs = self.s2_chain_s8([(step[0], step[1], True) for step in tr], z, ACT_RELU) if (s >= 3 or t1_s8(s)) else None
            if zs is not None:
                return zs
            for step in tr:
                z = self.conv_bn(z, step[0], step[1], ACT_RELU)
            return z

        def module(s, mi, n_mods, mod, xs, fork_in, join_out):
            self._exact = s == 4 and mi >= n_mods - r.f32_tail
            return self.hr_module(mod, xs, fork_in, join_out)
        ys = self.hr_stages(net, x, width_change, new_branch, module, before_fork)
        fl = net.final_layer
        rough = View(self.new(self.F * self.B, self.J, self.h, self.w))
        self._exact = r.f32_tail > 0
        out = self.conv(ys[0], fl.weight, rough, 1, fl.padding[0], 1, bias=fl.bias)
        self._exact = False
        return out

    def v3(self, t3):
        b, c, t = t3.shape
        return View(t3.view(b, c, 1, t))

    def tblock(self, blk, x, stride):
        B, C, T = x.shape
        To = T if stride == 1 else (T + 2 - 3) // 2 + 1
        L = self.lib
        a = blk.attn
        r = self.routes
        if r.use_flow_fused and stride == 1 and ops.flow_block_supported(blk, C, T):
            fp, bp = ops.pack_flow_front(blk, self.dev), ops.pack_flow_back(blk, self.dev)
            self._keep += [fp, bp]
            q, k, v, att, out = (self.new(B, C, T) for _ in range(5))
            self.call(L.otp_flow_front, "otp_flow_front", *ops.flow_front_args(x, fp, q, k, v, blk.ln1.eps))
            self.chan_attn(q, k, v, att, a)
            self.call(L.otp_flow_back, "otp_flow_back", *ops.flow_back_args(x, att, bp, out, blk.mlp[0].out_channels, blk.ln2.eps))
            return out
        ln1 = self.new(B, C, T)
        skip = self.new(B, C, To) if stride > 1 else None
        p = self.dev_param
        self.call(L.otp_ln_channel, "otp_ln_channel", hip.ptr(x), hip.ptr(p(blk.ln1.weight)), hip.ptr(p(blk.ln1.bias)),
                  hip.ptr(ln1), hip.ptr(skip), B, C, T, blk.ln1.eps)
        q, k, v = self.new(B, C, To), self.new(B, C, To), self.new(B, C, To)
        dx3 = r.use_dense_cc and r.use_x3 and ops.dense_x3_supported(C, To)
        dense = dx3 or (r.use_dense_cc and ops.dense_cc_supported(C, To))
        if dense:
            packs = [ops.pack_dense_cc(m.weight.to(self.dev), None, m.bias.to(self.dev), x3=dx3)
                     for m in (a.query, a.key, a.value)]
        if dense and stride == 1 and r.use_qkv_front:
            table = ops.pack_qkv_table(*[p(t) for t in (a.query_conv.weight, a.key_conv.weight, a.value_conv.weight,
                                                         a.query_norm.weight, a.query_norm.bias, a.key_norm.weight,
                                                         a.key_norm.bias, a.value_norm.weight, a.value_norm.bias)])
            self._keep += [table, *packs]
            self.call((L.otp_qkv_front_h1 if self.half_products else L.otp_qkv_front_x3) if dx3 else L.otp_qkv_front, "otp_qkv_front",
                      *ops.qkv_front_args(ln1, table, packs, (q, k, v), a.query_norm.eps))
        else:
            qn, kn, vn = self.new(B, C, To), self.new(B, C, To), self.new(B, C, To)
            self.call(L.otp_dwconv_ln3, "otp_dwconv_ln3", hip.ptr(ln1), hip.ptr(p(a.query_conv.weight)),
                      hip.ptr(p(a.key_conv.weight)), hip.ptr(p(a.value_conv.weight)),
                      hip.ptr(p(a.query_norm.weight)), hip.ptr(p(a.query_norm.bias)),
                      hip.ptr(p(a.key_norm.weight)), hip.ptr(p(a.key_norm.bias)),
                      hip.ptr(p(a.value_norm.weight)), hip.ptr(p(a.value_norm.bias)),
                      hip.ptr(qn), hip.ptr(kn), hip.ptr(vn), B, C, T, stride, a.query_norm.eps)
            if dense:
                self.dense((qn, kn, vn), packs, None, (q, k, v), B, C, To)
            else:
                self.conv(self.v3(qn), a.query.weight, self.v3(q), bias=a.query.bias)
                self.conv(self.v3(kn), a.key.weight, self.v3(k), bias=a.key.bias)
                self.conv(self.v3(vn), a.value.weight, self.v3(v), bias=a.value.bias)
        att = self.new(B, C, To)
        self.chan_attn(q, k, v, att, a)
        sa = blk.drop_path_attn.scale.detach().reshape(-1)
        y = self.new(B, C, To)
        if dense:
            sad = sa.to(self.dev, torch.float32)
            pk = ops.pack_dense_cc(a.proj.weight.to(self.dev), sad, a.proj.bias.detach().to(self.dev) * sad,
                                   x3=r.use_x3 and ops.dense_x3_supported(C, To))
            self.dense((att,), [pk], (skip if stride > 1 else x,), (y,), B, C, To)
        else:
            self.conv(self.v3(att), a.proj.weight, self.v3(y), scale=sa,
                      shift=a.proj.bias.detach() * sa.to(a.proj.bias.device), res=self.v3(skip if stride > 1 else x))
        sm = blk.drop_path_mlp.scale.detach().reshape(-1)
        out = self.new(B, C, To)
        hid = blk.mlp[0].out_channels
        mlp_x3 = r.use_fused_mlp and r.use_x3 and ops.mlp_x3_supported(C, hid, To)
        if mlp_x3 or (r.use_fused_mlp and ops.mlp_fused_supported(C, hid, To)):
            dev = lambda t: t.detach().to(self.dev, torch.float32)
            w1, b1, w2 = dev(blk.mlp[0].weight), dev(blk.mlp[0].bias), dev(blk.mlp[3].weight)
            packed = ops.pack_mlp_x3_weights(w1, b1, w2, half=self.half_products) if mlp_x3 else ops.pack_mlp_weights(w1, b1, w2)
            scd = dev(sm).contiguous()
            shd = (dev(blk.mlp[3].bias) * scd).contiguous()
            self._keep += [packed, scd, shd]
            fn, name = ((L.otp_ln_mlp_h1 if self.half_products else L.otp_ln_mlp_x3, "otp_ln_mlp_x3") if mlp_x3
                        else (L.otp_ln_mlp_fused, "otp_ln_mlp_fused"))
            self.call(fn, name, *ops.ln_mlp_args(y, p(blk.ln2.weight), p(blk.ln2.bias), blk.ln2.eps, packed, scd, shd, out, hid))
            return out
        ln2 = self.new(B, C, To)
        self.call(L.otp_ln_channel, "otp_ln_channel", hip.ptr(y), hip.ptr(p(blk.ln2.weight)), hip.ptr(p(blk.ln2.bias)),
                  hip.ptr(ln2), None, B, C, To, blk.ln2.eps)
        hdn = self.new(B, 4 * C, To)
        self.conv(self.v3(ln2), blk.mlp[0].weight, self.v3(hdn), bias=blk.mlp[0].bias, act=ACT_GELU)
        self.conv(self.v3(hdn), blk.mlp[3].weight, self.v3(out), scale=sm,
                  shift=blk.mlp[3].bias.detach() * sm.to(blk.mlp[3].bias.device), res=self.v3(y))
        return out

    def chan_attn(self, q, k, v, att, a):
        B, C, T = q.shape
        nbytes = self.lib.otp_chan_attn_workspace(B, C, T, a.n_head)
        ws = self.new(max(nbytes // 4, 1))
        self.call(self.lib.otp_chan_attn, "otp_chan_attn", *ops.chan_attn_args(q, k, v, att, ws, nbytes, a.n_head, a.scale))

    def conv_transformer(self, ct, x, stacked):
        _, C, T = x.shape
        L = self.lib
        for blk in ct.stem:
            x = self.tblock(blk, x, 1)
        self.call(L.otp_upsample_linear, "otp_upsample_linear", *ops.upsample_linear_args(x, stacked, 1, 0))
        for i, blk in enumerate(ct.branch):
            x = self.tblock(blk, x, 2)
            f = 2 ** (i + 1)
            if x.shape[2] * f != T:
                raise RuntimeError("heat-map size must make every pyramid level divide evenly (T % 4 == 0)")
            self.call(L.otp_upsample_linear, "otp_upsample_linear", *ops.upsample_linear_args(x, stacked, f, (i + 1) * C))

    def rsb_block(self, blk, x: View) -> View:
        n, _, h, w = x.t.shape
        bc = blk.branch_ch
        cbr = lambda m, inp, out, act, in2=None, res=None: self.conv(
            inp, m.conv.weight, out, 1, m.conv.padding[0], 1, bn=m.bn, bias=m.conv.bias, act=act, in2=in2, res=res)
        t = self.new(n, 4 * bc, h, w)
        cat = self.new(n, 4 * bc, h, w)
        cbr(blk.conv_bn_relu1, x, View(t), ACT_RELU)
        s = [View(t, i * bc, bc) for i in range(4)]
        tmp = lambda: View(self.new(n, bc, h, w))
        par = self.multi_stream and self._sid == 0
        side = (lambda: (self.fork((1,)), self.on_stream(1))) if par else (lambda: None)
        main = (lambda: self.on_stream(0)) if par else (lambda: None)
        o11 = cbr(blk.conv_bn_relu2_1_1, s[0], View(cat, 0, bc), ACT_RELU)
        o21 = cbr(blk.conv_bn_relu2_2_1, s[1], tmp(), ACT_RELU, in2=o11)
        side()
        o22 = cbr(blk.conv_bn_relu2_2_2, o21, View(cat, bc, bc), ACT_RELU)
        main()
        o31 = cbr(blk.conv_bn_relu2_3_1, s[2], tmp(), ACT_RELU, in2=o21)
        side()
        o32 = cbr(blk.conv_bn_relu2_3_2, o31, tmp(), ACT_RELU, in2=o22)
        main()
        o41 = cbr(blk.conv_bn_relu2_4_1, s[3], tmp(), ACT_RELU, in2=o31)
        if par:
            self.join((1,))
        o42 = cbr(blk.conv_bn_relu2_4_2, o41, tmp(), ACT_RELU, in2=o32)
        if par:
            self.on_stream(1)
        o33 = cbr(blk.conv_bn_relu2_3_3, o32, View(cat, 2 * bc, bc), ACT_RELU)
        if par:
            self.on_stream(0)
            self.join((1,))
        o43 = cbr(blk.conv_bn_relu2_4_3, o42, tmp(), ACT_RELU, in2=o33)
        cbr(blk.conv_bn_relu2_4_4, o43, View(cat, 3 * bc, bc), ACT_RELU)
        res = x
        if blk.downsample is not None:
            res = cbr(blk.downsample, x, View(self.new(n, blk.conv_bn_relu3.conv.out_channels, h, w)), ACT_NONE)
        out = View(self.new(n, blk.conv_bn_relu3.conv.out_channels, h, w))
        return cbr(blk.conv_bn_relu3, View(cat), out, ACT_RELU, res=res)

    def rsb_chain(self, chain, x: View) -> View:
        for blk in chain.layers:
            x = self.rsb_block(blk, x)
        return x

    def _build(self):
        m, B, J, h, w = self.model, self.B, self.J, self.h, self.w
        L, T = self.lib, self.h * self.w
        self.inp = self._given[0] if self._given[0] is not None else self.new(B, 3 * self.F, self.H_img, self.W_img)
        self.margin = self._given[1] if self._given[1] is not None else self.new(B, self.F - 1)
        assert tuple(self.inp.shape) == (B, 3 * self.F, self.H_img, self.W_img) and self.inp.is_contiguous()
        rough = self.hrnet(m.rough_pose_estimation_net, View(self.inp)).t
        self.hr_end = len(self.ops)

        total, squeezed, inter = self.new(B, J, h, w), self.new(B, J, h, w), self.new(B, J, h, w)
        flow_in = self.new(B, J, T)
        pe_f = self.dev_param(m.flow_encoder.pos_embd[0, :, :T])
        self.call(L.otp_glue_total_n, "otp_glue_total", hip.ptr(rough), hip.ptr(total), hip.ptr(squeezed), hip.ptr(inter),
                  hip.ptr(flow_in), hip.ptr(pe_f), B, J, T, self.F)
        ctx = self.new(B, J, T)
        self.fork((2,))
        self.on_stream(2)
        def_h = self.rsb_chain(m.def_fuse, View(total))
        self.on_stream(0)
        self.conv_transformer(m.flow_encoder, flow_in, ctx)
        D = m.num_frames * J
        x1, x2, prev_b = self.new(B, D, T), self.new(B, D, T), self.new(B, J, h, w)
        pe1 = self.dev_param(m.temporal_encoder1.pos_embd[0, :, :T])
        pe2 = self.dev_param(m.temporal_encoder2.pos_embd[0, :, :T])
        self.call(L.otp_glue_stack_n, "otp_glue_stack", hip.ptr(rough), hip.ptr(self.margin), hip.ptr(squeezed),
                  hip.ptr(inter), hip.ptr(ctx), hip.ptr(pe1), hip.ptr(pe2), hip.ptr(x1), hip.ptr(x2), hip.ptr(prev_b),
                  B, J, T, self.F)
        levels = m.scale_arch[-1] + 1
        cs_ = levels * D
        cpad = (-cs_) % 32 if (self.use_x3 and m.final_layer1.kernel_size == (1, 1)) else 0
        s1, s2 = self.new(B, cs_ + cpad, T), self.new(B, cs_ + cpad, T)
        if cpad:
            s1[:, cs_:].zero_()
            s2[:, cs_:].zero_()
        cat3 = self.new(B, 3 * J, h, w)
        def final(fl, s, i):
            wt = fl.weight
            if cpad:
                wt = torch.cat([wt.detach().to(self.dev, torch.float32),
                                torch.zeros(wt.shape[0], cpad, 1, 1, device=self.dev)], 1)
            self.conv(View(s.view(B, cs_ + cpad, h, w)), wt, View(cat3, i * J, J), 1, fl.padding[0], 1, bias=fl.bias)

        self.on_stream(2)
        self.copy_into(def_h, View(cat3, 2 * J, J))
        self.on_stream(0)
        self.fork((1,))
        self.conv_transformer(m.temporal_encoder1, x1, s1)
        final(m.final_layer1, s1, 0)
        self.on_stream(0 if self.routes.te_serial else 1)
        self.conv_transformer(m.temporal_encoder2, x2, s2)
        final(m.final_layer2, s2, 1)
        self.on_stream(0)
        self.join((1, 2))
        trans = self.rsb_chain(m.offset_mask_combine_conv, View(cat3))
        out = self.new(B, J, h, w)
        nd = len(m.deformable_conv_dilations)
        dils = [int(d) for d in m.deformable_conv_dilations]
        cin_t = trans.C
        if (self.use_dcn_fused and trans.coff == 0 and trans.C == trans.ctot and ops.dcn_fused_supported(cin_t, J, h, w, nd)
                and all(plain_conv(c[0], 3, dil=d, groups=None) for cs in (m.offsets_list, m.masks_list) for c, d in zip(cs, dils))
                and all(tuple(mm.deform_conv.weight.shape) == (J, J, 3, 3) and mm.deform_conv.deformable_groups == J
                        and mm.deform_conv.groups == 1 and _pair(mm.deform_conv.stride) == (1, 1)
                        and _pair(mm.deform_conv.padding) == (d, d) == _pair(mm.deform_conv.dilation)
                        for mm, d in zip(m.modulated_deform_conv_list, dils))):
            dcs = [mm.deform_conv for mm in m.modulated_deform_conv_list]
            packed = ops.pack_dcn_fused([self.dev_param(c[0].weight) for c in m.offsets_list],
                                        [self.dev_param(c[0].weight) for c in m.masks_list],
                                        [self.dev_param(dc.weight) for dc in dcs],
                                        [None if dc.bias is None else self.dev_param(dc.bias) for dc in dcs])
            ws = self.new(int(L.otp_dcn_fused_workspace(B, h, w)) // 4)
            dl = (ctypes.c_int * nd)(*dils)
            self._keep += [packed, dl]
            self.call(L.otp_dcn_fused_forward, "otp_dcn_fused_forward", hip.ptr(trans.t), hip.ptr(def_h.t), hip.ptr(packed),
                      hip.ptr(out), hip.ptr(ws), ws.numel() * 4, B, cin_t, J, h, w, dl, nd, 1.0 / nd)
            self._finish(out, rough, inter, prev_b, ctx, squeezed, total)
            return
        off_buf, msk_buf = self.new(B, J * 18, h, w), self.new(B, J * 9, h, w)
        for i, d in enumerate(m.deformable_conv_dilations):
            self.conv(trans, m.offsets_list[i][0].weight, View(off_buf), 1, d, d)
            self.conv(trans, m.masks_list[i][0].weight, View(msk_buf), 1, d, d)
            dc = m.modulated_deform_conv_list[i].deform_conv
            wt, bs = self.dev_param(dc.weight), self.dev_param(dc.bias)
            self.call(L.otp_mdcn_forward, "otp_mdcn_forward", hip.ptr(def_h.t), hip.ptr(off_buf), hip.ptr(msk_buf),
                      hip.ptr(wt), hip.ptr(bs), hip.ptr(out), B, J, h, w, J, 3, 3, 1, d, d, 1, J,
                      1.0 / nd, 0.0 if i == 0 else 1.0, 0)
        self._finish(out, rough, inter, prev_b, ctx, squeezed, total)

    def _finish(self, out, rough, inter, prev_b, ctx, squeezed, total):
        B, J, h, w = self.B, self.J, self.h, self.w
        if self.use_x3 or self.h16:
            self.call(self.lib.otp_range_poison, "otp_range_poison", hip.ptr(out), out.numel())
        self.outputs = (out, rough, inter, prev_b, ctx.view(B, J, h, w), squeezed, total)
        torch.cuda.synchronize(self.dev)

    _RANGE_KERNELS = {1: "convx (3x3 / 1x1 convolutions from fp32 NCHW)", 2: "convs (BasicBlock convolutions on S8 records)",
                      3: "convs2 (stride-2 convolutions on S8 records)", 4: "pointx (1x1 convolutions)", 5: "stem convolution",
                      6: "S8 conversion / fuse passes", 7: "mlpx (TransformerBlock MLP)", 8: "densex (q / k / v / proj projections)",
                      9: "channel attention", 10: "dcn_fused (warping head)", 11: "fp16 engine kernels"}

    def _raise_range(self, code):
        raise FloatingPointError(
            "otpose_amd: a value left the range of the half-precision operand pieces (|x| >= 65504, or a non-finite sum) in the "
            f"{self._RANGE_KERNELS.get(code, 'kernel family %d' % code)} of an eval forward; the heat-maps of that forward were "
# ... 68 lines not shown
```

### otpose_amd/hip.py

```python
from __future__ import annotations

import ctypes
import os
import threading
from ctypes import c_float, c_int, c_size_t, c_void_p

_HERE = os.path.dirname(os.path.abspath(__file__))
LIB_PATH = os.environ.get("OTPOSE_HIP_LIB") or os.path.join(_HERE, "csrc", "libotpose_hip.so")
_lib = None
_tls = threading.local()

OTP_OK = 0
_ERRORS = {
    -1: "OTP_ERR_BAD_ARG (null pointer or non-positive dimension)",
    -2: "OTP_ERR_UNSUPPORTED (shape / dtype / stride combination not implemented)",
    -3: "OTP_ERR_LAUNCH (HIP launch error)",
    -4: "OTP_ERR_WORKSPACE (workspace too small)",
}


class ConvDesc(ctypes.Structure):
    _fields_ = [(n, c_int) for n in (
        "N", "Cin", "H", "W", "Cout", "kh", "kw", "stride", "pad", "dil",
        "in_ctot", "in_coff", "in2_ctot", "in2_coff", "out_ctot", "out_coff",
        "res_ctot", "res_coff", "res_up", "act", "Ho", "Wo", "frame_split")] + [("out_scale", ctypes.c_float), ("res_layout", ctypes.c_int)]


class NhwcConvDesc(ctypes.Structure):
    _fields_ = [(n, c_int) for n in ("N", "H", "W", "Cin", "Cout", "kh", "kw", "stride", "pad", "dil", "out_mode")]


_ND = ctypes.POINTER(NhwcConvDesc)


class H16ConvDesc(ctypes.Structure):
    _fields_ = [(n, c_int) for n in ("N", "Cin", "H", "W", "Cout", "stride", "act", "in_gtot", "in_goff", "out_gtot", "out_goff",
                                     "res_gtot", "res_goff")] + [("out_scale", ctypes.c_float)]


_HD = ctypes.POINTER(H16ConvDesc)

SIGNATURES = {
    "otp_version": (c_int, []),
    "otp_range_flag_read": (c_int, [c_int]),
    "otp_range_poison": (c_int, [c_void_p, c_size_t, c_void_p]),
    "otp_h8_bytes": (c_size_t, [c_int] * 4),
    "otp_h8_pack": (c_int, [c_void_p, c_void_p] + [c_int] * 8 + [c_void_p]),
    "otp_h8_unpack": (c_int, [c_void_p, c_void_p] + [c_int] * 6 + [c_void_p]),
    "otp_h16_conv3x3_supported": (c_int, [_HD]),
    "otp_h16_conv3x3_weight_bytes": (c_size_t, [c_int, c_int]),
    "otp_h16_conv3x3_pack_weight": (c_int, [c_void_p] * 3 + [c_int, c_int, c_float, c_void_p]),
    "otp_h16_conv3x3": (c_int, [c_void_p] * 5 + [_HD, c_void_p]),
    "otp_h16_pointwise_supported": (c_int, [c_int, c_int]),
    "otp_h16_pointwise_weight_bytes": (c_size_t, [c_int, c_int]),
    "otp_h16_pointwise_pack": (c_int, [c_void_p] * 4 + [c_int, c_int, c_float, c_void_p]),
    "otp_h16_pointwise": (c_int, [c_void_p] * 4 + [c_int] * 12 + [c_float, c_void_p]),
    "otp_h16_stem_supported": (c_int, [c_int] * 5),
    "otp_h16_stem_weight_bytes": (c_size_t, [c_int]),
    "otp_h16_stem_pack": (c_int, [c_void_p] * 4 + [c_int, c_void_p]),
    "otp_h16_stem": (c_int, [c_void_p] * 3 + [c_int] * 5 + [c_void_p]),
    "otp_mlp_h1_weight_bytes": (c_size_t, [c_int] * 2),
    "otp_mlp_h1_pack": (c_int, [c_void_p] * 4 + [c_int] * 2 + [c_void_p]),
    "otp_ln_mlp_h1": (c_int, [c_void_p] * 3 + [c_float] + [c_void_p] * 4 + [c_int] * 4 + [c_void_p]),
    "otp_dense_h1": (c_int, [ctypes.POINTER(c_void_p)] * 4 + [c_int] * 4 + [c_void_p]),
    "otp_qkv_front_h1": (c_int, [c_void_p] * 8 + [c_int] * 3 + [c_float, c_void_p]),
    "otp_h16_upsample_add": (c_int, [ctypes.POINTER(c_void_p), ctypes.POINTER(c_int), c_int, c_void_p, c_void_p] + [c_int] * 5 + [c_void_p]),
    "otp_mdcn_forward": (c_int, [c_void_p] * 6 + [c_int] * 12 + [c_float, c_float, c_int, c_void_p]),
    "otp_mdcn_forward_ex": (c_int, [c_void_p] * 6 + [c_int] * 15 + [c_float, c_float, c_int, c_void_p]),
    "otp_mdcn_backward_ex": (c_int, [c_void_p] * 10 + [c_void_p, c_size_t] + [c_int] * 15 + [c_int, c_void_p]),
    "otp_mdcn_backward_workspace": (c_size_t, [c_int] * 7),
    "otp_mdcn_backward_workspace_ex": (c_size_t, [c_int] * 17),
    "otp_mdcn_backward": (c_int, [c_void_p] * 10 + [c_void_p, c_size_t] + [c_int] * 12 + [c_int, c_void_p]),
    "otp_deform_psroi_pool_forward": (c_int, [c_void_p] * 5 + [c_int] * 7 + [c_float] + [c_int] * 5 + [c_float, c_int, c_void_p]),
    "otp_deform_psroi_pool_backward_workspace": (c_size_t, [c_int] * 13),
    "otp_deform_psroi_pool_backward": (c_int, [c_void_p] * 7 + [c_int] * 7 + [c_float] + [c_int] * 5 + [c_float]
                                       + [c_void_p, c_size_t, c_int, c_void_p]),
    "otp_conv2d_pack_weight": (c_int, [c_void_p, c_void_p, c_int, c_int, c_int, c_int, c_void_p]),
    "otp_conv2d": (c_int, [c_void_p] * 7 + [ctypes.POINTER(ConvDesc), c_void_p]),
    "otp_conv2d_wino_weight_bytes": (c_size_t, [c_int, c_int]),
    "otp_conv2d_wino_pack_weight": (c_int, [c_void_p, c_void_p, c_int, c_int, c_void_p]),
    "otp_conv2d_wino_supported": (c_int, [ctypes.POINTER(ConvDesc)]),
    "otp_conv2d_wino_last_plan": (c_int, [ctypes.POINTER(c_int)]),
    "otp_conv2d_wino": (c_int, [c_void_p] * 6 + [ctypes.POINTER(ConvDesc), c_void_p]),
    "otp_conv3x3_small_supported": (c_int, [ctypes.POINTER(ConvDesc)]),
    "otp_conv3x3_small_weight_bytes": (c_size_t, [c_int, c_int]),
    "otp_conv3x3_small_pack": (c_int, [c_void_p, c_void_p, c_int, c_int, c_void_p]),
    "otp_conv3x3_small": (c_int, [c_void_p] * 6 + [ctypes.POINTER(ConvDesc), c_void_p]),
    "otp_conv2d_x3_weight_bytes": (c_size_t, [c_int, c_int, c_int, c_int]),
    "otp_conv2d_x3_pack_weight": (c_int, [c_void_p, c_void_p, c_void_p, c_int, c_int, c_int, c_int, c_void_p]),
    "otp_conv2d_x3_supported": (c_int, [ctypes.POINTER(ConvDesc)]),
    "otp_conv2d_x3": (c_int, [c_void_p] * 5 + [ctypes.POINTER(ConvDesc), c_void_p]),
    "otp_s8_bytes": (c_size_t, [c_int] * 4),
    "otp_s8_pack": (c_int, [c_void_p] * 3 + [c_int] * 6 + [c_void_p]),
    "otp_s8_upsample_add": (c_int, [ctypes.POINTER(c_void_p), ctypes.POINTER(c_int), c_int] + [c_void_p] * 4 + [c_int] * 9 + [c_void_p]),
    "otp_s8_upsample_add_ex": (c_int, [ctypes.POINTER(c_void_p), ctypes.POINTER(c_int), c_int, c_void_p, c_int] + [c_void_p] * 3
                               + [c_int] * 9 + [c_void_p]),
    "otp_s8_unpack": (c_int, [c_void_p, c_void_p] + [c_int] * 4 + [c_void_p]),
    "otp_c4_unpack": (c_int, [c_void_p, c_void_p] + [c_int] * 4 + [c_void_p]),
    "otp_conv3x3_s8_supported": (c_int, [ctypes.POINTER(ConvDesc)]),
    "otp_conv3x3_s8_weight_bytes": (c_size_t, [c_int, c_int]),
    "otp_conv3x3_s8_pack_weight": (c_int, [c_void_p] * 3 + [c_int, c_int, c_void_p]),
    "otp_conv3x3_s8": (c_int, [c_void_p] * 5 + [c_int, c_void_p, ctypes.POINTER(ConvDesc), c_void_p]),
    "otp_conv3x3_s2_s8_supported": (c_int, [ctypes.POINTER(ConvDesc), c_int]),
    "otp_conv3x3_s2_s8": (c_int, [c_void_p] * 6 + [ctypes.POINTER(ConvDesc), c_void_p]),
    "otp_conv2d_set_tile": (c_int, [c_int] * 4),
    "otp_conv2d_last_plan": (c_int, [ctypes.POINTER(c_int)]),
    "otp_conv2d_plan": (c_int, [ctypes.POINTER(ConvDesc), ctypes.POINTER(c_int)]),
    "otp_conv2d_pack_weight_dgrad": (c_int, [c_void_p, c_void_p, c_int, c_int, c_int, c_int, c_void_p]),
    "otp_dilate": (c_int, [c_void_p, c_void_p] + [c_int] * 6 + [c_void_p]),
    "otp_grad_sumsq_scratch": (c_size_t, []),
    "otp_grad_sumsq": (c_int, [c_void_p, c_size_t, c_void_p, c_void_p]),
    "otp_adamw_step": (c_int, [c_void_p] * 4 + [c_size_t] + [c_float] * 5 + [c_int, c_void_p, c_float, c_void_p]),
    "otp_pck_accuracy": (c_int, [c_void_p] * 4 + [c_int] * 4 + [c_float, c_void_p]),
    "otp_frames_u8_to_clip": (c_int, [c_void_p] * 2 + [c_int] * 4 + [c_float] * 6 + [c_void_p]),
    "otp_crop_clips_u8": (c_int, [c_void_p] + [c_int] * 3 + [c_void_p] * 4 + [c_int] * 4 + [c_float] * 6 + [c_void_p]),
    "otp_crop_clips_blur_u8": (c_int, [c_void_p] + [c_int] * 3 + [c_void_p] * 4 + [c_int] * 4 + [c_float] * 6
                               + [c_void_p] * 3),
    "otp_crop_clips_pair_u8": (c_int, [c_void_p] + [c_int] * 3 + [c_void_p] * 3 + [c_int] * 4 + [c_float] * 6 + [c_void_p]),
    "otp_pose_targets": (c_int, [c_void_p] * 6 + [c_int] * 7 + [c_void_p]),
    "otp_conv2d_wgrad_workspace": (c_size_t, [c_int] * 2),
    "otp_conv2d_wgrad": (c_int, [c_void_p] * 3 + [c_int] * 14 + [c_void_p, c_size_t, c_void_p]),
    "otp_bn_workspace": (c_size_t, [c_int] * 3),
    "otp_bn_train_forward": (c_int, [c_void_p] * 9 + [c_void_p, c_size_t] + [c_int] * 3 + [c_float, c_float] +
                             [c_int] * 7 + [c_void_p]),
    "otp_bn_train_backward": (c_int, [c_void_p] * 10 + [c_void_p, c_size_t] + [c_int] * 9 + [c_void_p]),
    "otp_channel_sum": (c_int, [c_void_p, c_void_p, c_void_p, c_size_t] + [c_int] * 5 + [c_void_p]),
    "otp_glue_total": (c_int, [c_void_p] * 6 + [c_int] * 3 + [c_void_p]),
    "otp_glue_stack": (c_int, [c_void_p] * 10 + [c_int] * 3 + [c_void_p]),
    "otp_glue_total_n": (c_int, [c_void_p] * 6 + [c_int] * 4 + [c_void_p]),
    "otp_glue_stack_n": (c_int, [c_void_p] * 10 + [c_int] * 4 + [c_void_p]),
    "otp_ln_channel": (c_int, [c_void_p] * 5 + [c_int] * 3 + [c_float, c_void_p]),
    "otp_dwconv_ln3": (c_int, [c_void_p] * 13 + [c_int] * 4 + [c_float, c_void_p]),
    "otp_chan_attn_workspace": (c_size_t, [c_int] * 4),
    "otp_dense_cc_supported": (c_int, [c_int] * 2),
    "otp_dense_cc_weight_bytes": (c_size_t, [c_int]),
    "otp_dense_cc_pack": (c_int, [c_void_p] * 4 + [c_int, c_void_p]),
    "otp_dense_cc": (c_int, [ctypes.POINTER(c_void_p)] * 4 + [c_int] * 4 + [c_void_p]),
    "otp_qkv_front_table_bytes": (c_size_t, [c_int]),
    "otp_qkv_front_pack_table": (c_int, [c_void_p] * 10 + [c_int, c_void_p]),
    "otp_qkv_front": (c_int, [c_void_p] * 8 + [c_int] * 3 + [c_float, c_void_p]),
    "otp_mlp_fused_supported": (c_int, [c_int] * 3),
    "otp_mlp_fused_weight_bytes": (c_size_t, [c_int] * 2),
    "otp_mlp_fused_pack": (c_int, [c_void_p] * 4 + [c_int] * 2 + [c_void_p]),
    "otp_mlp_fused": (c_int, [c_void_p] * 6 + [c_int] * 4 + [c_void_p]),
    "otp_ln_mlp_fused": (c_int, [c_void_p] * 3 + [c_float] + [c_void_p] * 4 + [c_int] * 4 + [c_void_p]),
    "otp_dcn_fused_supported": (c_int, [c_int] * 5),
    "otp_dcn_fused_weight_bytes": (c_size_t, [c_int] * 2),
    "otp_dcn_fused_pack": (c_int, [c_void_p] * 5 + [c_int, c_int, c_void_p]),
    "otp_dcn_fused_workspace": (c_size_t, [c_int] * 3),
    "otp_dcn_fused_forward": (c_int, [c_void_p] * 5 + [c_size_t] + [c_int] * 5 + [ctypes.POINTER(c_int), c_int, c_float, c_void_p]),
    "otp_dense_x3_supported": (c_int, [c_int] * 2),
    "otp_dense_x3_weight_bytes": (c_size_t, [c_int]),
    "otp_dense_x3_pack": (c_int, [c_void_p] * 4 + [c_int, c_void_p]),
    "otp_dense_x3": (c_int, [ctypes.POINTER(c_void_p)] * 4 + [c_int] * 4 + [c_void_p]),
    "otp_dense_x3_pack_bf16p": (c_int, [c_void_p] * 4 + [c_int, c_void_p]),
    "otp_dense_x3_bf16p": (c_int, [ctypes.POINTER(c_void_p)] * 4 + [c_int] * 4 + [c_void_p]),
    "otp_stem_conv_x3_supported": (c_int, [c_int] * 5),
    "otp_stem_conv_x3_weight_bytes": (c_size_t, [c_int]),
    "otp_stem_conv_x3_pack": (c_int, [c_void_p] * 4 + [c_int, c_void_p]),
    "otp_stem_conv_x3": (c_int, [c_void_p] * 3 + [c_int] * 5 + [c_void_p]),
    "otp_pointwise_x3_supported": (c_int, [c_int] * 3),
    "otp_pointwise_x3_weight_bytes": (c_size_t, [c_int] * 2),
    "otp_pointwise_x3_pack": (c_int, [c_void_p] * 4 + [c_int, c_int, c_void_p]),
    "otp_pointwise_x3": (c_int, [c_void_p] * 4 + [c_int] * 11 + [c_void_p]),
    "otp_pointwise_x3_s8_supported": (c_int, [c_int] * 3),
    "otp_pointwise_x3_s8_weight_bytes": (c_size_t, [c_int] * 2),
    "otp_pointwise_x3_s8_pack": (c_int, [c_void_p] * 4 + [c_int, c_int, c_void_p]),
    "otp_pointwise_x3_s8": (c_int, [c_void_p] * 3 + [c_int] * 7 + [c_void_p]),
    "otp_pointwise_x3_s8_res": (c_int, [c_void_p] * 4 + [c_int] * 9 + [c_void_p]),
    "otp_pointwise_x3_pair_supported": (c_int, [c_int] * 4),
    "otp_pointwise_x3_pair_weight_bytes": (c_size_t, [c_int] * 3),
    "otp_pointwise_x3_pair_pack": (c_int, [c_void_p] * 7 + [c_int] * 3 + [c_void_p]),
    "otp_pointwise_x3_pair": (c_int, [c_void_p] * 5 + [c_int] * 13 + [c_void_p]),
    "otp_qkv_front_x3": (c_int, [c_void_p] * 8 + [c_int] * 3 + [c_float, c_void_p]),
    "otp_mlp_x3_supported": (c_int, [c_int] * 3),
    "otp_mlp_x3_weight_bytes": (c_size_t, [c_int] * 2),
    "otp_mlp_x3_pack": (c_int, [c_void_p] * 4 + [c_int] * 2 + [c_void_p]),
    "otp_mlp_x3": (c_int, [c_void_p] * 6 + [c_int] * 4 + [c_void_p]),
    "otp_flow_block_supported": (c_int, [c_int] * 3),
    "otp_flow_front_param_floats": (c_size_t, [c_int]),
    "otp_flow_back_param_floats": (c_size_t, [c_int, c_int]),
    "otp_flow_front": (c_int, [c_void_p] * 5 + [c_int] * 3 + [c_float, c_void_p]),
    "otp_flow_back": (c_int, [c_void_p] * 4 + [c_int] * 4 + [c_float, c_void_p]),
    "otp_ln_mlp_x3": (c_int, [c_void_p] * 3 + [c_float] + [c_void_p] * 4 + [c_int] * 4 + [c_void_p]),
    "otp_chan_attn": (c_int, [c_void_p] * 4 + [c_void_p, c_size_t] + [c_int] * 4 + [c_float, c_void_p]),
    "otp_chan_attn_splits": (c_int, [c_int, c_int]),
    "otp_chan_attn_scores": (c_int, [c_void_p] * 3 + [c_int] * 3 + [c_void_p]),
    "otp_chan_attn_set_split": (c_int, [c_int]),
    "otp_chan_attn_apply": (c_int, [c_void_p] * 3 + [c_int] * 3 + [c_void_p]),
    "otp_chan_attn_scores_bf16p": (c_int, [c_void_p] * 3 + [c_int] * 3 + [c_void_p]),
    "otp_chan_attn_apply_bf16p": (c_int, [c_void_p] * 3 + [c_int] * 3 + [c_void_p]),
    "otp_transpose_scale": (c_int, [c_void_p, c_void_p, c_int, c_int, c_int, c_float, c_void_p]),
    "otp_softmax_backward": (c_int, [c_void_p] * 5 + [c_int] * 3 + [c_void_p]),
    "otp_ln_channel_backward": (c_int, [c_void_p] * 5 + [c_int] * 3 + [c_float, c_void_p]),
    "otp_ln_channel_backward_workspace": (c_size_t, [c_int] * 3),
    "otp_ln_channel_backward_params": (c_int, [c_void_p] * 6 + [c_void_p, c_size_t] + [c_int] * 3 + [c_float, c_void_p]),
    "otp_dwconv3_forward": (c_int, [c_void_p] * 3 + [c_int] * 4 + [c_void_p]),
    "otp_dwconv3_backward": (c_int, [c_void_p] * 5 + [c_int] * 4 + [c_void_p]),
    "otp_gelu_forward": (c_int, [c_void_p, c_void_p, c_size_t, c_void_p]),
    "otp_gelu_backward": (c_int, [c_void_p] * 3 + [c_size_t, c_void_p]),
    "otp_maxpool3s2_forward": (c_int, [c_void_p, c_void_p, c_int, c_int, c_void_p]),
    "otp_maxpool3s2_backward": (c_int, [c_void_p] * 3 + [c_int, c_int, c_void_p]),
    "otp_upsample_linear_backward": (c_int, [c_void_p, c_void_p] + [c_int] * 6 + [c_void_p]),
    "otp_upsample_linear": (c_int, [c_void_p, c_void_p] + [c_int] * 6 + [c_void_p]),
    "otp_upsample_add": (c_int, [c_void_p] * 3 + [c_int] * 12 + [c_void_p]),
    "otp_upsample_add_multi": (c_int, [ctypes.POINTER(c_void_p), ctypes.POINTER(c_int), c_int, c_void_p, c_void_p] + [c_int] * 9 + [c_void_p]),
    "otp_upsample_add_backward": (c_int, [c_void_p] * 4 + [c_int] * 4 + [c_void_p]),
    "otp_axpby": (c_int, [c_void_p, c_void_p, c_float, c_float, c_size_t, c_void_p]),
    "otp_heatmap_decode": (c_int, [c_void_p] * 5 + [c_int] * 5 + [c_void_p]),
    "otp_heatmap_flip_decode": (c_int, [c_void_p] * 7 + [c_int] * 5 + [c_void_p]),
    "otp_clip_mirror_pair": (c_int, [c_void_p] * 2 + [c_int] * 4 + [c_void_p]),
    "otp_loss_workspace": (c_size_t, [c_int, c_int]),
    "otp_loss_st_ohkw_grads": (c_int, [c_void_p] * 9 + [c_void_p, c_size_t] + [c_int] * 5 + [c_void_p]),
    "otp_loss_st_ohkw": (c_int, [c_void_p] * 8 + [c_void_p, c_size_t] + [c_int] * 5 + [c_void_p]),
    "otp_nhwc_conv_weight_bytes": (c_size_t, [_ND]),
    "otp_nhwc_conv_stats_rows": (c_int, [_ND]),
    "otp_nhwc_conv_plan": (c_int, [_ND, ctypes.POINTER(c_int)]),
    "otp_nhwc_conv_pack": (c_int, [c_void_p, c_void_p, _ND, c_int, c_void_p]),
    "otp_nhwc_conv_pack_job_bytes": (c_size_t, []),
    "otp_nhwc_conv_pack_job": (c_int, [c_void_p, c_void_p, _ND, c_int, c_void_p]),
    "otp_nhwc_conv_pack_batch": (c_int, [c_void_p, c_int, c_void_p]),
    "otp_nhwc_conv_bf16": (c_int, [c_void_p] * 5 + [_ND, c_void_p]),
    "otp_nhwc_conv_bf16_res": (c_int, [c_void_p, c_void_p, c_void_p, c_void_p, c_void_p, c_void_p, _ND, c_void_p]),
    "otp_nhwc_wgrad_workspace": (c_size_t, [_ND]),
    "otp_nhwc_wgrad_bf16": (c_int, [c_void_p] * 4 + [c_size_t, _ND, c_void_p]),
    "otp_nhwc_bn_finalize": (c_int, [c_void_p, c_int, c_int, c_int, c_float] + [c_void_p] * 8 + [c_float, c_float, c_void_p]),
    "otp_nhwc_bn_apply": (c_int, [c_void_p] * 6 + [c_size_t, c_int, c_int, c_void_p]),
    "otp_nhwc_bn_backward_workspace": (c_size_t, [c_size_t, c_int]),
    "otp_nhwc_bn_backward": (c_int, [c_void_p] * 11 + [c_size_t, c_size_t, c_int, c_int, c_int, c_void_p]),
    "otp_nhwc_upsample_add": (c_int, [c_void_p] * 3 + [c_int] * 6 + [c_void_p]),
    "otp_nhwc_upsample_add_backward": (c_int, [c_void_p] * 4 + [c_int] * 6 + [c_void_p]),
    "otp_nchw_f32_to_nhwc_bf16": (c_int, [c_void_p, c_void_p] + [c_int] * 5 + [c_void_p]),
    "otp_nhwc_bf16_to_nchw_f32": (c_int, [c_void_p, c_void_p] + [c_int] * 4 + [c_void_p]),
    "otp_nhwc_dilate": (c_int, [c_void_p, c_void_p] + [c_int] * 7 + [c_void_p]),
    "otp_scale_residual": (c_int, [c_void_p] * 5 + [c_int] * 3 + [c_void_p]),
    "otp_scale_residual_backward_workspace": (c_size_t, [c_int] * 3),
    "otp_scale_residual_backward": (c_int, [c_void_p] * 7 + [c_size_t] + [c_int] * 3 + [c_void_p]),
    "otp_nhwc_channel_sum_workspace": (c_size_t, [c_size_t, c_int]),
    "otp_nhwc_channel_sum": (c_int, [c_void_p] * 3 + [c_size_t, c_size_t, c_int, c_int, c_void_p]),
    "otp_gelu_bf16_forward": (c_int, [c_void_p, c_void_p, c_size_t, c_void_p]),
    "otp_gelu_bf16_backward": (c_int, [c_void_p] * 3 + [c_size_t, c_void_p]),
    "otp_nhwc_conv_bn_bf16": (c_int, [c_void_p] * 10 + [ctypes.c_float, ctypes.c_float, c_void_p, c_void_p, c_int, _ND, c_void_p]),
    "otp_nhwc_mlp_fused_supported": (c_int, [_ND]),
    "otp_nhwc_mlp_up_bf16": (c_int, [c_void_p] * 6 + [ctypes.c_float, ctypes.c_ulonglong, _ND, c_void_p]),
    "otp_nhwc_mlp_down_dgrad_bf16": (c_int, [c_void_p] * 5 + [ctypes.c_float, _ND, c_void_p]),
    "otp_gelu_dropout_bf16_forward": (c_int, [c_void_p] * 3 + [c_size_t, ctypes.c_float, ctypes.c_ulonglong, c_void_p]),
    "otp_gelu_dropout_bf16_backward": (c_int, [c_void_p] * 4 + [c_size_t, ctypes.c_float, c_void_p]),
    "otp_loss_joints_mse": (c_int, [c_void_p] * 5 + [c_void_p, c_size_t] + [c_int] * 6 + [c_void_p]),
    "otp_pose_assign": (c_int, [c_void_p] * 12 + [ctypes.c_double] + [c_void_p] * 3 + [c_int] * 4 + [c_void_p]),
    "otp_ap_curve": (c_int, [c_void_p] * 6 + [c_int, c_void_p]),
    "otp_pose_nms": (c_int, [c_void_p] * 6 + [ctypes.POINTER(ctypes.c_double)] + [ctypes.c_double] * 3 + [c_int] * 2
                     + [c_void_p] * 4 + [c_int] * 3 + [c_void_p]),
}


def lib():
    global _lib
    if _lib is None:
        if not os.path.isfile(LIB_PATH):
            raise RuntimeError(
                f"HIP library {LIB_PATH} is missing - run `python -c 'import __graft_entry__ as g; g.build()'` "
                "(or `make -C otpose_amd/csrc`). otpose_amd has no CPU or PyTorch-op fallback.")
        cdll = ctypes.CDLL(LIB_PATH)
        for name, (res, args) in SIGNATURES.items():
            fn = getattr(cdll, name)
            fn.restype = res
            fn.argtypes = args
        cdll.otp_chan_attn_set_split(0 if os.environ.get("OTPOSE_CONV_MATH", "x3") == "f32" else 1)
        import torch
        if torch.cuda.is_available():
            cdll.otp_range_flag_read(0)
        _lib = _DeviceGuarded(cdll)
    return _lib


class _DeviceGuarded:

    def __init__(self, cdll):
        self._cdll = cdll
        for name in SIGNATURES:
            setattr(self, name, self._wrap(getattr(cdll, name)))

    @staticmethod
    def _wrap(fn):
        import torch

        cur = getattr(torch._C, "_cuda_getDevice", None) or torch.cuda.current_device

        def call(*args):
            dev = getattr(_tls, "dev", None)
            if dev is not None and dev != cur():
                with torch.cuda.device(dev):
                    return fn(*args)
            return fn(*args)
        return call


def check(status: int, what: str):
    if status != OTP_OK:
        raise RuntimeError(f"{what} failed: {_ERRORS.get(status, status)}")


def ptr(t):
    return None if t is None else c_void_p(t.data_ptr())


def stream_of(t):
    import torch
    dev = t.device.index
    _tls.dev = dev
    raw = getattr(torch._C, "_cuda_getCurrentRawStream", None)
    if raw is not None:
        return c_void_p(raw(dev))
    return c_void_p(torch.cuda.current_stream(t.device).cuda_stream)


_SIDE_STREAMS = {}


def side_streams(device, n, first=0):
    import torch
    device = torch.device(device)
    if device.index is None:
        device = torch.device("cuda", torch.cuda.current_device())
    pool = _SIDE_STREAMS.setdefault(device, [])
    while len(pool) < first + n:
        pool.append(torch.cuda.Stream(device))
    return pool[first:first + n]
```

### otpose_amd/ops.py

```python
from __future__ import annotations

import ctypes
import math
import os

import torch
from torch.autograd import Function

from . import hip
from .augment import FLIP_PAIRS

_DTYPE_F32 = 0


def _require_gpu(*tensors):
    for t in tensors:
        if t is not None and not t.is_cuda:
            raise NotImplementedError("otpose_amd operators run on the GPU only (no CPU path)")


def _check_f32(*tensors):
    for t in tensors:
        if t is not None and t.dtype != torch.float32:
            raise RuntimeError(f"otpose_amd HIP operators are built for float32, got {t.dtype}")
# ... 471 lines not shown
    rv = View(res.contiguous()) if res is not None else None
    d = conv_desc(iv, ov, cout, k, k, stride, pad, dil, act, None, rv)
    e = x3_weight_exponent(weight, scale)
    d.out_scale = 2.0 ** -e
    conv2d_x3_launch(iv, pack_x3_weight(weight, scale, stride, e), shift, ov, d, rv)
    return out


S8_F32_C4, S8_F32_NCHW = 1, 2


def s8_empty(n, c, h, w, device):
    nbytes = hip.lib().otp_s8_bytes(n, c, h, w)
    if not nbytes:
        raise ValueError(f"S8 images need a channel count that is a multiple of 8, got {c}")
    return torch.empty(nbytes // 4, dtype=torch.int32, device=device)


def c4_empty(n, c, h, w, device):
    assert c % 4 == 0
    return torch.empty(n * c * h * w, dtype=torch.float32, device=device)


def s8_pack(inp, out=None, out_c4=None, stream=None):
    iv = inp if isinstance(inp, View) else View(inp.contiguous())
    _require_gpu(iv.t)
    n, _, h, w = iv.t.shape
    out = s8_empty(n, iv.C, h, w, iv.t.device) if out is None else out
    hip.check(hip.lib().otp_s8_pack(hip.ptr(iv.t), hip.ptr(out), hip.ptr(out_c4), n, iv.C, h, w, iv.ctot, iv.coff,
                                    stream if stream is not None else hip.stream_of(iv.t)), "otp_s8_pack")
    return out


def s8_unpack(s8, n, c, h, w):
    _require_gpu(s8)
    out = torch.empty(n, c, h, w, dtype=torch.float32, device=s8.device)
    hip.check(hip.lib().otp_s8_unpack(hip.ptr(s8), hip.ptr(out), n, c, h, w, hip.stream_of(s8)), "otp_s8_unpack")
    return out


def c4_unpack(c4, n, c, h, w):
    _require_gpu(c4)
    out = torch.empty(n, c, h, w, dtype=torch.float32, device=c4.device)
    hip.check(hip.lib().otp_c4_unpack(hip.ptr(c4), hip.ptr(out), n, c, h, w, hip.stream_of(c4)), "otp_c4_unpack")
    return out


def s8_conv_supported(desc) -> bool:
    return bool(hip.lib().otp_conv3x3_s8_supported(desc))


def s8_conv_desc(n, cin, cout, h, w, act=ACT_NONE, out: View = None, res: View = None, stride=1):
    d = hip.ConvDesc()
    d.N, d.Cin, d.H, d.W, d.Cout = n, cin, h, w, cout
    d.kh = d.kw = 3
    d.stride, d.pad, d.dil = stride, 1, 1
    d.in_ctot, d.in_coff, d.in2_ctot, d.in2_coff = cin, 0, 0, 0
    d.out_ctot, d.out_coff = (out.ctot, out.coff) if out is not None else (cout, 0)
    d.res_ctot, d.res_coff = (res.ctot, res.coff) if res is not None else (0, 0)
    d.res_up = 1
    d.act, d.Ho, d.Wo, d.frame_split = act, h // stride, w // stride, 0
    return d


def s8_s2_conv_desc(n, cin, cout, h, w, act=ACT_NONE, out: View = None, res: View = None):
    return s8_conv_desc(n, cin, cout, h, w, act, out, res, stride=2)


def s8_s2_conv_supported(desc, nchw_out=True):
    return bool(hip.lib().otp_conv3x3_s2_s8_supported(desc, int(nchw_out)))


def conv3x3_s2_s8_args(in_s8, wpacked, shift, desc, res: View = None, out: View = None, out_s8=None):
    return (hip.ptr(in_s8), hip.ptr(wpacked), hip.ptr(shift), _vp(res), _vp(out), hip.ptr(out_s8), desc)


def conv3x3_s2_s8(x_s8, shape, weight, scale=None, shift=None, act=ACT_NONE, res=None, out="nchw"):
    _require_gpu(x_s8, weight)
    n, cin, h, w = shape
    cout = weight.shape[0]
    e = x3_weight_exponent(weight, scale)
    wp = pack_s8_weight(weight, scale, e)
    sh = shift.detach().contiguous().float() if shift is not None else None
    L = hip.lib()
    if out == "s8":
        assert res is None
        d = s8_s2_conv_desc(n, cin, cout, h, w, act)
        d.out_scale = 2.0 ** -e
        o8 = s8_empty(n, cout, h // 2, w // 2, x_s8.device)
        _launch(L.otp_conv3x3_s2_s8, "otp_conv3x3_s2_s8", conv3x3_s2_s8_args(x_s8, wp, sh, d, out_s8=o8), x_s8)
        return o8
    o = torch.empty(n, cout, h // 2, w // 2, dtype=torch.float32, device=x_s8.device)
    rv = View(res.contiguous()) if res is not None else None
    d = s8_s2_conv_desc(n, cin, cout, h, w, act, View(o), rv)
    d.out_scale = 2.0 ** -e
    _launch(L.otp_conv3x3_s2_s8, "otp_conv3x3_s2_s8", conv3x3_s2_s8_args(x_s8, wp, sh, d, rv, View(o)), x_s8)
    return o


def pack_s8_weight(weight, scale=None, k=0):
    _require_gpu(weight)
    _check_f32(weight)
    w = weight.detach().contiguous()
    cout, cin, kh, kw = w.shape
    assert kh == kw == 3
    L = hip.lib()
    nbytes = L.otp_conv3x3_s8_weight_bytes(cout, cin)
    if not nbytes:
        raise ValueError(f"otp_conv3x3_s8: unsupported channel counts ({cout}, {cin})")
    u = torch.empty(nbytes // 4, dtype=torch.int32, device=w.device)
    sc = _scaled_vec(scale, k, cout, w.device)
    hip.check(L.otp_conv3x3_s8_pack_weight(hip.ptr(w), hip.ptr(sc), hip.ptr(u), cout, cin, hip.stream_of(w)),
              "otp_conv3x3_s8_pack_weight")
    return u


def conv3x3_s8_args(in_s8, wpacked, shift, desc, res=None, out_f32=None, f32_layout=S8_F32_C4, out_s8=None):
    return (hip.ptr(in_s8), hip.ptr(wpacked), hip.ptr(shift), hip.ptr(res), hip.ptr(out_f32), f32_layout, hip.ptr(out_s8), desc)


def conv3x3_s8_launch(in_s8, wpacked, shift, desc, res_c4=None, out_f32=None, f32_layout=S8_F32_C4, out_s8=None, stream=None):
    _launch(hip.lib().otp_conv3x3_s8, "otp_conv3x3_s8",
            conv3x3_s8_args(in_s8, wpacked, shift, desc, res_c4, out_f32, f32_layout, out_s8), in_s8, stream)


def conv3x3_s8(x_s8, shape, weight, scale=None, shift=None, act=ACT_NONE, res_c4=None, f32="nchw", want_s8=True, res_s8=None):
    _require_gpu(x_s8, weight)
    n, cin, h, w = shape
    cout = weight.shape[0]
    out = out_s8 = None
    layout = S8_F32_C4
    if f32 == "nchw":
        out, layout = torch.empty(n, cout, h, w, dtype=torch.float32, device=x_s8.device), S8_F32_NCHW
    elif f32 == "c4":
        out = c4_empty(n, cout, h, w, x_s8.device)
    if want_s8:
        out_s8 = s8_empty(n, cout, h, w, x_s8.device)
    d = s8_conv_desc(n, cin, cout, h, w, act)
    e = x3_weight_exponent(weight, scale)
    d.out_scale = 2.0 ** -e
    if res_s8 is not None:
        assert res_c4 is None
        d.res_layout = 1
    conv3x3_s8_launch(x_s8, pack_s8_weight(weight, scale, e), shift, d, res_s8 if res_s8 is not None else res_c4, out, layout,
                      out_s8)
    return out, out_s8


def ln_mlp_args(y, gamma, beta, eps, packed, scale, shift, out, hid):
    b, c, t = y.shape
    return (hip.ptr(y), hip.ptr(gamma), hip.ptr(beta), eps, hip.ptr(packed), hip.ptr(scale), hip.ptr(shift), hip.ptr(out), b, c, hid, t)


def ln_mlp_fused(y, gamma, beta, eps, packed, scale, shift, out=None, hid=None, stream=None, entry="otp_ln_mlp_fused"):
    _require_gpu(y, packed)
    _check_f32(y)
    hid = 4 * y.shape[1] if hid is None else hid
    out = torch.empty_like(y) if out is None else out
    _launch(getattr(hip.lib(), entry), entry, ln_mlp_args(y, gamma, beta, eps, packed, scale, shift, out, hid), y, stream)
    return out


def dense_cc_supported(c, t) -> bool:
    return bool(hip.lib().otp_dense_cc_supported(int(c), int(t)))


def dense_x3_supported(c, t) -> bool:
    return bool(hip.lib().otp_dense_x3_supported(int(c), int(t)))


def pack_dense_cc(weight, scale=None, shift=None, x3=False, grad=False):
    _require_gpu(weight)
    c = weight.shape[0]
    L = hip.lib()
    nbytes = (L.otp_dense_x3_weight_bytes if x3 else L.otp_dense_cc_weight_bytes)(c)
    if not nbytes or weight.shape[1] != c:
        raise RuntimeError(f"otp_dense_cc: unsupported weight shape {tuple(weight.shape)}")
    f = lambda t: None if t is None else t.detach().to(weight.device, torch.float32).contiguous()
    w, sc, sh = f(weight), f(scale), f(shift)
    packed = torch.empty(nbytes // 4, dtype=torch.float32, device=weight.device)
    pack = (L.otp_dense_x3_pack_bf16p if grad else L.otp_dense_x3_pack) if x3 else L.otp_dense_cc_pack
    hip.check(pack(hip.ptr(w), hip.ptr(sc), hip.ptr(sh), hip.ptr(packed), c, hip.stream_of(w)), "otp_dense_cc_pack")
    return packed


def dense_cc_args(xs, packs, ress, outs):
    n = len(xs)
    arr = lambda ts: (ctypes.c_void_p * n)(*[hip.ptr(t) for t in ts])
    return arr(xs), arr(packs), arr(ress if ress is not None else [None] * n), arr(outs)


def dense_cc(xs, packs, ress=None, outs=None, stream=None, x3=False, grad=False, half=False):
    _require_gpu(*xs)
    b, c, t = xs[0].shape
    outs = [torch.empty_like(x) for x in xs] if outs is None else outs
    ax, ap, ar, ao = dense_cc_args(xs, packs, ress, outs)
    fn = (hip.lib().otp_dense_x3_bf16p if grad else (hip.lib().otp_dense_h1 if half else hip.lib().otp_dense_x3)) if x3 \
        else hip.lib().otp_dense_cc
    hip.check(fn(ax, ap, ar, ao, len(xs), b, c, t, stream if stream is not None else hip.stream_of(xs[0])), "otp_dense_cc")
    return outs


def stem_conv_x3_supported(b, f, h, w, cout) -> bool:
    return bool(hip.lib().otp_stem_conv_x3_supported(int(b), int(f), int(h), int(w), int(cout)))


def pack_stem_conv_x3(weight, scale=None, shift=None):
    _require_gpu(weight)
    cout = weight.shape[0]
    L = hip.lib()
    nbytes = L.otp_stem_conv_x3_weight_bytes(cout)
    if not nbytes or tuple(weight.shape[1:]) != (3, 3, 3):
        raise RuntimeError(f"otp_stem_conv_x3: unsupported weight shape {tuple(weight.shape)}")
    f = lambda t: None if t is None else t.detach().to(weight.device, torch.float32).contiguous()
    w, sc, sh = f(weight), f(scale), f(shift)
    packed = torch.empty(nbytes // 4, dtype=torch.float32, device=weight.device)
    hip.check(L.otp_stem_conv_x3_pack(hip.ptr(w), hip.ptr(sc), hip.ptr(sh), hip.ptr(packed), cout, hip.stream_of(w)),
              "otp_stem_conv_x3_pack")
    return packed


def stem_conv_x3_args(clip, packed, out, frames, cout):
    b, _, h, w = clip.shape
    return (hip.ptr(clip), hip.ptr(packed), hip.ptr(out.t if isinstance(out, H8) else out), b, frames, h, w, cout)


def stem_conv_x3(clip, packed, cout, frames=5, out=None, stream=None):
    _require_gpu(clip)
    b, c, h, w = clip.shape
    assert c == 3 * frames and clip.is_contiguous() and clip.dtype == torch.float32
    ho, wo = (h - 1) // 2 + 1, (w - 1) // 2 + 1
    out = torch.empty(frames * b, cout, ho, wo, dtype=torch.float32, device=clip.device) if out is None else out
    _launch(hip.lib().otp_stem_conv_x3, "otp_stem_conv_x3", stem_conv_x3_args(clip, packed, out, frames, cout), clip, stream)
    return out


def pointwise_x3_supported(cin, cout, t) -> bool:
    return bool(hip.lib().otp_pointwise_x3_supported(int(cin), int(cout), int(t)))


def _pack_pointwise(entry, weight, scale, shift):
    _require_gpu(weight)
    cout, cin = weight.shape[:2]
    L = hip.lib()
    nbytes = getattr(L, entry + "_weight_bytes")(cin, cout)
    if not nbytes:
        raise RuntimeError(f"{entry}: unsupported weight shape {tuple(weight.shape)}")
    f = lambda t: None if t is None else t.detach().to(weight.device, torch.float32).contiguous()
    w, sc, sh = f(weight).reshape(cout, cin), f(scale), f(shift)
    e = x3_weight_exponent(w)
    if e:
        w, sc = w * float(2.0 ** e), _scaled_vec(sc, -e, cout, w.device)
    packed = torch.empty(nbytes // 4, dtype=torch.float32, device=weight.device)
    hip.check(getattr(L, entry + "_pack")(hip.ptr(w), hip.ptr(sc), hip.ptr(sh), hip.ptr(packed), cin, cout, hip.stream_of(w)),
              entry + "_pack")
    return packed


def pack_pointwise_x3(weight, scale=None, shift=None):
    return _pack_pointwise("otp_pointwise_x3", weight, scale, shift)


def pointwise_x3_args(x: View, packed, out: View, res: View = None, relu=False):
    b, _, h, w = x.t.shape
    return (_vp(x), hip.ptr(packed), _vp(res), _vp(out), b, x.C, out.C, h * w, x.ctot, x.coff, *_slice(res), out.ctot, out.coff,
            int(bool(relu)))


def pointwise_x3(x: View, packed, out: View, res: View = None, relu=False, stream=None):
    _require_gpu(x.t, out.t)
    _launch(hip.lib().otp_pointwise_x3, "otp_pointwise_x3", pointwise_x3_args(x, packed, out, res, relu), x.t, stream)
    return out


def pointwise_x3_s8_supported(cin, cout, t) -> bool:
    return bool(hip.lib().otp_pointwise_x3_s8_supported(int(cin), int(cout), int(t)))


def pack_pointwise_x3_s8(weight, scale=None, shift=None):
    return _pack_pointwise("otp_pointwise_x3_s8", weight, scale, shift)


def pointwise_x3_s8_res_args(x: View, packed, cout, out_s8, res: View = None, relu=False):
    b, _, h, w = x.t.shape
    return (_vp(x), hip.ptr(packed), _vp(res), hip.ptr(out_s8), b, x.C, cout, h * w, x.ctot, x.coff, *_slice(res), int(bool(relu)))


def pointwise_x3_s8(x: View, packed, cout, out_s8=None, relu=False, stream=None, res: View = None):
    _require_gpu(x.t)
    b, _, h, w = x.t.shape
    out_s8 = s8_empty(b, cout, h, w, x.t.device) if out_s8 is None else out_s8
    _launch(hip.lib().otp_pointwise_x3_s8_res, "otp_pointwise_x3_s8", pointwise_x3_s8_res_args(x, packed, cout, out_s8, res, relu),
            x.t, stream)
    return out_s8


def pointwise_x3_pair_supported(cin, cmid, cout2, t) -> bool:
    return bool(hip.lib().otp_pointwise_x3_pair_supported(int(cin), int(cmid), int(cout2), int(t)))


def pack_pointwise_x3_pair(weight1, scale1, shift1, weight2, scale2=None, shift2=None):
    _require_gpu(weight1, weight2)
    cmid, cin = weight1.shape[:2]
    cout2 = weight2.shape[0]
    L = hip.lib()
    nbytes = L.otp_pointwise_x3_pair_weight_bytes(cin, cmid, cout2) if weight2.shape[1] == cmid else 0
    if not nbytes:
        raise RuntimeError(f"otp_pointwise_x3_pair: unsupported weight shapes {tuple(weight1.shape)}, {tuple(weight2.shape)}")
    f = lambda t: None if t is None else t.detach().to(weight1.device, torch.float32).contiguous()
    ws = []
    for wt, sc, sh, co, ci in ((weight1, scale1, shift1, cmid, cin), (weight2, scale2, shift2, cout2, cmid)):
        w, sc, sh = f(wt).reshape(co, ci), f(sc), f(sh)
        e = x3_weight_exponent(w)
        if e:
            w, sc = w * float(2.0 ** e), _scaled_vec(sc, -e, co, w.device)
        ws += [w, sc, sh]
    packed = torch.empty(nbytes // 4, dtype=torch.float32, device=weight1.device)
    hip.check(L.otp_pointwise_x3_pair_pack(*[hip.ptr(t) for t in ws], hip.ptr(packed), cin, cmid, cout2, hip.stream_of(ws[0])),
              "otp_pointwise_x3_pair_pack")
    return packed


def pointwise_x3_pair_args(x: View, packed, out: View, cout2, out_s8, res: View = None, relu1=True, relu2=True):
    b, _, h, w = x.t.shape
    return (_vp(x), hip.ptr(packed), _vp(res), _vp(out), hip.ptr(out_s8), b, x.C, out.C, cout2, h * w, x.ctot, x.coff, *_slice(res),
            out.ctot, out.coff, int(bool(relu1)), int(bool(relu2)))


def pointwise_x3_pair(x: View, packed, out: View, cout2, res: View = None, out_s8=None, relu1=True, relu2=True, stream=None):
    _require_gpu(x.t, out.t)
    b, _, h, w = x.t.shape
    out_s8 = s8_empty(b, cout2, h, w, x.t.device) if out_s8 is None else out_s8
    _launch(hip.lib().otp_pointwise_x3_pair, "otp_pointwise_x3_pair",
            pointwise_x3_pair_args(x, packed, out, cout2, out_s8, res, relu1, relu2), x.t, stream)
    return out_s8


def pack_qkv_table(dwq, dwk, dwv, gq, bq, gk, bk, gv, bv):
    ts = [t.detach().float().contiguous() for t in (dwq, dwk, dwv, gq, bq, gk, bk, gv, bv)]
    _require_gpu(*ts)
    c = ts[3].numel()
    L = hip.lib()
    table = torch.empty(L.otp_qkv_front_table_bytes(c) // 4, dtype=torch.float32, device=ts[0].device)
    hip.check(L.otp_qkv_front_pack_table(*[hip.ptr(t) for t in ts], hip.ptr(table), c, hip.stream_of(ts[0])),
              "otp_qkv_front_pack_table")
    return table


def qkv_front_args(x, table, packs, outs, eps):
    b, c, t = x.shape
    return (hip.ptr(x), hip.ptr(table), *[hip.ptr(p) for p in packs], *[hip.ptr(o) for o in outs], b, c, t, eps)


def qkv_front(x, table, packs, eps=1e-5, outs=None, stream=None, x3=False, half=False):
    _require_gpu(x, table)
    outs = [torch.empty_like(x) for _ in range(3)] if outs is None else outs
    fn = (hip.lib().otp_qkv_front_h1 if half else hip.lib().otp_qkv_front_x3) if x3 else hip.lib().otp_qkv_front
    _launch(fn, "otp_qkv_front", qkv_front_args(x, table, packs, outs, eps), x, stream)
    return outs


def mlp_fused_supported(c, hid, t) -> bool:
    return bool(hip.lib().otp_mlp_fused_supported(int(c), int(hid), int(t)))


def pack_mlp_weights(w1, b1, w2):
    _require_gpu(w1, b1, w2)
    hid, c = w1.shape[:2]
    L = hip.lib()
    nbytes = L.otp_mlp_fused_weight_bytes(c, hid)
    if not nbytes:
        raise RuntimeError(f"otp_mlp_fused: unsupported widths C={c}, HID={hid}")
    packed = torch.empty(nbytes // 4, dtype=torch.float32, device=w1.device)
    w1c, w2c, b1c = (t.detach().contiguous().float() for t in (w1, w2, b1))
    hip.check(L.otp_mlp_fused_pack(hip.ptr(w1c), hip.ptr(b1c), hip.ptr(w2c), hip.ptr(packed), c, hid, hip.stream_of(w1c)),
              "otp_mlp_fused_pack")
    return packed


def mlp_fused(x, packed, scale, shift, res, out=None, hid=None, stream=None, entry="otp_mlp_fused"):
    _require_gpu(x, packed, res)
    _check_f32(x)
    b, c, t = x.shape
    hid = 4 * c if hid is None else hid
    out = torch.empty_like(x) if out is None else out
    _launch(getattr(hip.lib(), entry), entry, (hip.ptr(x), hip.ptr(packed), hip.ptr(scale), hip.ptr(shift), hip.ptr(res), hip.ptr(out),
                                                b, c, hid, t), x, stream)
    return out


def dcn_fused_supported(cin, j, h, w, nd) -> bool:
    return bool(hip.lib().otp_dcn_fused_supported(int(cin), int(j), int(h), int(w), int(nd)))


def pack_dcn_fused(w_offs, w_masks, w_dcns, biases):
    nd, j = len(w_offs), w_dcns[0].shape[0]
    dev = w_offs[0].device
    _require_gpu(*w_offs, *w_masks, *w_dcns)
    keep = [[t.detach().contiguous().float() for t in ts] for ts in (w_offs, w_masks, w_dcns)]
    keep.append([None if b is None else b.detach().contiguous().float() for b in biases])
    ptrs = [torch.tensor([0 if t is None else t.data_ptr() for t in ts], dtype=torch.int64, device=dev) for ts in keep]
    L = hip.lib()
    nbytes = L.otp_dcn_fused_weight_bytes(nd, j)
    if not nbytes:
        raise RuntimeError(f"otp_dcn_fused: unsupported ND={nd}, J={j}")
    packed = torch.empty(nbytes // 4, dtype=torch.int32, device=dev)
    hip.check(L.otp_dcn_fused_pack(*[hip.ptr(t) for t in ptrs], hip.ptr(packed), nd, j, hip.stream_of(packed)),
              "otp_dcn_fused_pack")
    torch.cuda.current_stream(dev).synchronize()
    return packed


def dcn_fused(trans, x, packed, dilations, alpha, out=None, workspace=None, stream=None):
    _require_gpu(trans, x, packed)
    _check_f32(trans)
    b, cin, h, w = trans.shape
    j = x.shape[1]
    L = hip.lib()
    out = torch.empty_like(x) if out is None else out
    nws = L.otp_dcn_fused_workspace(b, h, w)
    workspace = torch.empty(nws // 4, dtype=torch.int32, device=x.device) if workspace is None else workspace
    dl = (ctypes.c_int * len(dilations))(*[int(d) for d in dilations])
    hip.check(L.otp_dcn_fused_forward(hip.ptr(trans), hip.ptr(x), hip.ptr(packed), hip.ptr(out), hip.ptr(workspace), nws, b, cin, j,
                                      h, w, dl, len(dilations), float(alpha),
                                      stream if stream is not None else hip.stream_of(x)), "otp_dcn_fused_forward")
    return out


def mlp_x3_supported(c, hid, t) -> bool:
    return bool(hip.lib().otp_mlp_x3_supported(int(c), int(hid), int(t)))


def pack_mlp_x3_weights(w1, b1, w2, half=False):
    _require_gpu(w1, b1, w2)
    hid, c = w1.shape[:2]
    L = hip.lib()
    nbytes = (L.otp_mlp_h1_weight_bytes if half else L.otp_mlp_x3_weight_bytes)(c, hid)
    if not nbytes:
        raise RuntimeError(f"otp_mlp_x3: unsupported widths C={c}, HID={hid}")
    packed = torch.empty(nbytes // 4, dtype=torch.int32, device=w1.device)
    w1c, w2c, b1c = (t.detach().contiguous().float() for t in (w1, w2, b1))
    hip.check((L.otp_mlp_h1_pack if half else L.otp_mlp_x3_pack)(hip.ptr(w1c), hip.ptr(b1c), hip.ptr(w2c), hip.ptr(packed), c, hid,
                                                                 hip.stream_of(w1c)), "otp_mlp_x3_pack")
    return packed


def mlp_x3(x, packed, scale, shift, res, out=None, hid=None, stream=None):
    return mlp_fused(x, packed, scale, shift, res, out, hid, stream, "otp_mlp_x3")


def ln_mlp_x3(y, gamma, beta, eps, packed, scale, shift, out=None, hid=None, stream=None, half=False):
    return ln_mlp_fused(y, gamma, beta, eps, packed, scale, shift, out, hid, stream, "otp_ln_mlp_h1" if half else "otp_ln_mlp_x3")


def wino_supported(desc) -> bool:
    return bool(hip.lib().otp_conv2d_wino_supported(desc))


def conv2d_wino_args(inp: View, upacked, scale, shift, out: View, desc, res: View = None):
    return (_vp(inp), hip.ptr(upacked), hip.ptr(scale), hip.ptr(shift), _vp(res), _vp(out), desc)


def conv2d_wino_launch(inp: View, upacked, scale, shift, out: View, desc, res: View = None, stream=None):
    _launch(hip.lib().otp_conv2d_wino, "otp_conv2d_wino", conv2d_wino_args(inp, upacked, scale, shift, out, desc, res), out.t, stream)


def conv2d_wino(x, weight, scale=None, shift=None, act=ACT_NONE, res=None):
    _require_gpu(x, weight)
    cout = weight.shape[0]
    out = torch.empty((x.shape[0], cout, x.shape[2], x.shape[3]), dtype=torch.float32, device=x.device)
    iv, ov = View(x.contiguous()), View(out)
    rv = View(res.contiguous()) if res is not None else None
    d = conv_desc(iv, ov, cout, 3, 3, 1, 1, 1, act, None, rv, 1)
    conv2d_wino_launch(iv, pack_wino_weight(weight), scale, shift, ov, d, rv)
    return out


def conv2d(x, weight, scale=None, shift=None, stride=1, pad=0, dil=1, act=ACT_NONE, res=None, in2=None, res_up=1):
    _require_gpu(x, weight)
    w4 = weight if weight.dim() == 4 else weight.unsqueeze(-1)
    cout, cin, kh, kw = w4.shape
    h, w = x.shape[2:]
    ho = (h + 2 * pad - (dil * (kh - 1) + 1)) // stride + 1
    wo = (w + 2 * pad - (dil * (kw - 1) + 1)) // stride + 1
    out = torch.empty((x.shape[0], cout, ho * max(res_up, 1), wo * max(res_up, 1)), dtype=torch.float32, device=x.device)
    iv, ov = View(x.contiguous()), View(out)
    rv = View(res.contiguous()) if res is not None else None
    i2 = View(in2.contiguous()) if in2 is not None else None
    d = conv_desc(iv, ov, cout, kh, kw, stride, pad, dil, act, i2, rv, res_up)
    conv2d_launch(iv, pack_conv_weight(w4), scale, shift, ov, d, i2, rv)
    return out


def upsample_add_args(low: View, res: View, out: View, f, relu=False):
    n, _, hl, wl = low.t.shape
    return (_vp(low), _vp(res), _vp(out), n, low.C, hl, wl, f, int(relu), low.ctot, low.coff, res.ctot, res.coff, out.ctot, out.coff)


def upsample_add(low, res, f, relu=False, out=None):
    _require_gpu(low, res)
    out = torch.empty_like(res) if out is None else out
    _launch(hip.lib().otp_upsample_add, "otp_upsample_add", upsample_add_args(View(low), View(res), View(out), f, relu), low)
    return out


def upsample_add_multi_args(lows, factors, res: View, out: View, relu=False):
    n, _, hh, wh = out.t.shape
    lp = (ctypes.c_void_p * len(lows))(*[_vp(v) for v in lows])
    fp = (ctypes.c_int * len(lows))(*[int(f) for f in factors])
    return (lp, fp, len(lows), _vp(res), _vp(out), n, res.C, hh, wh, int(relu), res.ctot, res.coff, out.ctot, out.coff), (lp, fp)


def upsample_add_multi(lows, res, relu=False, out=None):
    _require_gpu(res, *lows)
    n, c, hh, wh = res.shape
    out = torch.empty_like(res) if out is None else out
    lows = [t.contiguous() for t in lows]
    args, _keep = upsample_add_multi_args([View(t) for t in lows], [hh // t.shape[2] for t in lows], View(res), View(out), relu)
    _launch(hip.lib().otp_upsample_add_multi, "otp_upsample_add_multi", args, res)
    return out


def ln_channel(x, gamma, beta, eps=1e-5, pool=False):
    _require_gpu(x)
    b, c, t = x.shape
    y = torch.empty_like(x)
    p = torch.empty((b, c, (t + 2 - 3) // 2 + 1), dtype=x.dtype, device=x.device) if pool else None
    hip.check(hip.lib().otp_ln_channel(hip.ptr(x), hip.ptr(gamma), hip.ptr(beta), hip.ptr(y), hip.ptr(p), b, c, t,
                                       eps, hip.stream_of(x)), "otp_ln_channel")
    return (y, p) if pool else y


def dwconv_ln3(x, dw, gammas, betas, stride, eps=1e-5):
    _require_gpu(x)
    b, c, t = x.shape
    to = (t + 2 - 3) // stride + 1
    outs = [torch.empty((b, c, to), dtype=x.dtype, device=x.device) for _ in range(3)]
    hip.check(hip.lib().otp_dwconv_ln3(
        hip.ptr(x), hip.ptr(dw[0]), hip.ptr(dw[1]), hip.ptr(dw[2]), hip.ptr(gammas[0]), hip.ptr(betas[0]),
        hip.ptr(gammas[1]), hip.ptr(betas[1]), hip.ptr(gammas[2]), hip.ptr(betas[2]), hip.ptr(outs[0]),
        hip.ptr(outs[1]), hip.ptr(outs[2]), b, c, t, stride, eps, hip.stream_of(x)), "otp_dwconv_ln3")
    return outs


def chan_attn_args(q, k, v, out, ws, nbytes, n_head, scale):
    b, c, t = q.shape
    return (hip.ptr(q), hip.ptr(k), hip.ptr(v), hip.ptr(out), hip.ptr(ws), nbytes, b, c, t, n_head, scale)


def chan_attn(q, k, v, n_head, scale):
    _require_gpu(q, k, v)
    b, c, t = q.shape
    out = torch.empty_like(q)
    L = hip.lib()
    nbytes = L.otp_chan_attn_workspace(b, c, t, n_head)
    ws = torch.empty(max(nbytes // 4, 1), dtype=torch.float32, device=q.device)
    _launch(L.otp_chan_attn, "otp_chan_attn", chan_attn_args(q, k, v, out, ws, nbytes, n_head, scale), q)
    return out


def upsample_linear_args(x, out, f, out_coff=0):
    b, c = x.shape[:2]
    return (hip.ptr(x), hip.ptr(out), b, c, x.numel() // (b * c), f, out.shape[1], out_coff)


def upsample_linear(x, f, out=None, out_coff=0):
    _require_gpu(x)
    b, c, t = x.shape
    if out is None:
        out = torch.empty((b, c, t * f), dtype=x.dtype, device=x.device)
    _launch(hip.lib().otp_upsample_linear, "otp_upsample_linear", upsample_linear_args(x, out, f, out_coff), x)
    return out


def get_max_preds(batch_heatmaps):
    return _decode(batch_heatmaps, None, None, refine=False)


def get_final_preds(batch_heatmaps, center=None, scale=None):
    return _decode(batch_heatmaps, center, scale, refine=True)


def _decode(hm, center, scale, refine):
    _require_gpu(hm)
    _check_f32(hm)
    if hm.dim() != 4:
        raise AssertionError("batch_images should be 4-ndim")
    hm = hm.contiguous()
    n, j, h, w = hm.shape
    preds = torch.empty((n, j, 2), dtype=torch.float32, device=hm.device)
    maxvals = torch.empty((n, j, 1), dtype=torch.float32, device=hm.device)
    c = s_ = None
    if center is not None:
        c = torch.as_tensor(center, dtype=torch.float32, device=hm.device).reshape(n, 2).contiguous()
        s_ = torch.as_tensor(scale, dtype=torch.float32, device=hm.device).reshape(n, 2).contiguous()
    hip.check(hip.lib().otp_heatmap_decode(hip.ptr(hm), hip.ptr(preds), hip.ptr(maxvals), hip.ptr(c), hip.ptr(s_),
                                           n, j, h, w, int(refine), hip.stream_of(hm)), "otp_heatmap_decode")
    return preds, maxvals


def flip_permutation(pairs, num_joints):
    import numpy as np
    j = int(num_joints)
    if j <= 0:
# ... 626 lines not shown
```

Measured before the change: 3250 frames/s.

## Fuse next block's LN1 statistics into MLP epilogue and apply LN on qkv load

The LN+MLP kernel's epilogue now applies the residual and scale/shift, computes per-token mean and reciprocal std for the next transformer block's LN1, and writes them to a small stats buffer. The next block's qkv front-end kernel normalizes its inputs on load, taking gamma and beta from spare slots in the packed table. This removes the separate channel LayerNorm pass and its full activation round trip between stem blocks. In exchange it adds cross-lane reductions to the MLP epilogue, extra register pressure and more template variants.

```diff
diff --git a/include/otpose_hip.h b/include/otpose_hip.h
--- a/include/otpose_hip.h
+++ b/include/otpose_hip.h
@@ -62,6 +62,10 @@
                  int T, void* stream);
 int otp_qkv_front_h1(const void* x, const void* table, const void* packed_q, const void* packed_k, const void* packed_v, void* q,
                      void* k, void* v, int B, int C, int T, float eps, void* stream);
+int otp_ln_mlp_h1_stats(const void* y, const void* ln_gamma, const void* ln_beta, float ln_eps, const void* packed, const void* scale,
+                        const void* shift, void* out, int B, int C, int HID, int T, void* stats, float stats_eps, void* stream);
+int otp_qkv_front_h1_ln(const void* x, const void* stats, const void* table, const void* packed_q, const void* packed_k,
+                        const void* packed_v, void* q, void* k, void* v, int B, int C, int T, float eps, void* stream);
 
 int otp_mdcn_forward(const void* x, const void* offset, const void* mask, const void* weight,
                      const void* bias, void* out,
@@ -258,6 +262,11 @@
                int C, int HID, int T, void* stream);
 int otp_ln_mlp_x3(const void* y, const void* ln_gamma, const void* ln_beta, float ln_eps, const void* packed,
                   const void* scale, const void* shift, void* out, int B, int C, int HID, int T, void* stream);
+int otp_ln_mlp_x3_stats(const void* y, const void* ln_gamma, const void* ln_beta, float ln_eps, const void* packed,
+                        const void* scale, const void* shift, void* out, int B, int C, int HID, int T, void* stats, float stats_eps,
+                        void* stream);
+int otp_qkv_front_x3_ln(const void* x, const void* stats, const void* table, const void* packed_q, const void* packed_k,
+                        const void* packed_v, void* q, void* k, void* v, int B, int C, int T, float eps, void* stream);
 
 int otp_flow_block_supported(int C, int hidden, int T);
 size_t otp_flow_front_param_floats(int C);
diff --git a/otpose_amd/csrc/densex.hip b/otpose_amd/csrc/densex.hip
--- a/otpose_amd/csrc/densex.hip
+++ b/otpose_amd/csrc/densex.hip
@@ -140,9 +140,10 @@
     float* out[3];
 };
 
-template <int C, bool H1 = false>
+template <int C, bool H1 = false, bool LN1 = false>
 __global__ __launch_bounds__(256, C <= 136 ? 3 : 1) void qkvx_front_kernel(const float* __restrict__ x, const float* __restrict__ table,
-                                                            QxArgs A, int T, int tiles_per_b, float eps, unsigned* rflag) {
+                                                            QxArgs A, int T, int tiles_per_b, float eps, unsigned* rflag,
+                                                            const otp_f32x2* __restrict__ stats) {
     constexpr int KS = dx_ks(C), BLKB = dx_block_bytes(C), TAB = 3 * C * 8;
     __shared__ __attribute__((aligned(16))) unsigned char lds[2 * BLKB];
     __shared__ __attribute__((aligned(16))) float tab[TAB];
@@ -158,6 +159,16 @@
     const int vb0 = (8 * kq * T + tokc) * 4;
     for (int i = tid; i < TAB / 4; i += 256)
         reinterpret_cast<otp_f32x4*>(tab)[i] = reinterpret_cast<const otp_f32x4*>(table)[i];
+    otp_f32x2 na = {0.f, 0.f}, n0 = na, n1 = na, nd = na;
+    if constexpr (LN1) {
+        const otp_f32x2* sb = stats + (size_t)b * T;
+        const otp_f32x4 s01 = *reinterpret_cast<const otp_f32x4*>(sb + tokc);
+        const otp_f32x2 sa = sb[l_ok ? tokc - 1 : tokc], sd = sb[r_ok ? tokc + 2 : tokc];
+        na = otp_f32x2{sa.y, -sa.x * sa.y};
+        n0 = otp_f32x2{s01[1], -s01[0] * s01[1]};
+        n1 = otp_f32x2{s01[3], -s01[2] * s01[3]};
+        nd = otp_f32x2{sd.y, -sd.x * sd.y};
+    }
     __syncthreads();
 
     for (int p = (int)blockIdx.y; p <= (int)blockIdx.y; ++p) {
@@ -172,8 +183,15 @@
                 const int c = 32 * ks + 8 * kq + j;
                 const bool live = 32 * ks + 24 + j < C || c < C;
                 const int so = (32 * ks + j) * T * 4;
-                const otp_f32x2 m = __builtin_bit_cast(otp_f32x2, __builtin_amdgcn_raw_buffer_load_b64(rx, live ? vb0 : -16, so, 0));
-                const float la = bload(rx, live ? vb0 - 4 : -16, so), ld = bload(rx, live ? vb0 + 8 : -16, so);
+                otp_f32x2 m = __builtin_bit_cast(otp_f32x2, __builtin_amdgcn_raw_buffer_load_b64(rx, live ? vb0 : -16, so, 0));
+                float la = bload(rx, live ? vb0 - 4 : -16, so), ld = bload(rx, live ? vb0 + 8 : -16, so);
+                if constexpr (LN1) {
+                    const otp_f32x2 gb = *reinterpret_cast<const otp_f32x2*>(tp + (live ? c : 0) * 8 + 6);
+                    la = (la * na.x + na.y) * gb.x + gb.y;
+                    m.x = (m.x * n0.x + n0.y) * gb.x + gb.y;
+                    m.y = (m.y * n1.x + n1.y) * gb.x + gb.y;
+                    ld = (ld * nd.x + nd.y) * gb.x + gb.y;
+                }
                 const float a = l_ok ? la : 0.f, d = r_ok ? ld : 0.f;
                 const otp_f32x4 w = *reinterpret_cast<const otp_f32x4*>(tp + (live ? c : 0) * 8);
                 X0[ks][j] = live ? w[0] * a + w[1] * m.x + w[2] * m.y : 0.f;
@@ -281,8 +299,9 @@
 #ifndef OTP_X3_GRAD_COPY
 namespace {
 int dx_qkv_launch(const void* x, const void* table, const void* packed_q, const void* packed_k, const void* packed_v, void* q, void* k,
-                  void* v, int B, int C, int T, float eps, void* stream, bool h1) {
+                  void* v, int B, int C, int T, float eps, void* stream, bool h1, const void* stats = nullptr) {
     if (!x || !table || !packed_q || !packed_k || !packed_v || !q || !k || !v || B <= 0) return OTP_ERR_BAD_ARG;
+    if (reinterpret_cast<uintptr_t>(stats) & 15) return OTP_ERR_BAD_ARG;
     if (!otp_dense_x3_supported(C, T)) return OTP_ERR_UNSUPPORTED;
     if ((reinterpret_cast<uintptr_t>(x) | reinterpret_cast<uintptr_t>(q) | reinterpret_cast<uintptr_t>(k) |
          reinterpret_cast<uintptr_t>(v)) & 7 ||
@@ -298,13 +317,12 @@
     const dim3 grid((unsigned)(B * tiles), 3u);
     auto st = static_cast<hipStream_t>(stream);
     auto xf = static_cast<const float*>(x), tf = static_cast<const float*>(table);
-    if (C == 204) {
-        if (h1) hipLaunchKernelGGL((qkvx_front_kernel<204, true>), grid, dim3(256), 0, st, xf, tf, a, T, tiles, eps, otp_range_word());
-        else hipLaunchKernelGGL((qkvx_front_kernel<204, false>), grid, dim3(256), 0, st, xf, tf, a, T, tiles, eps, otp_range_word());
-    } else {
-        if (h1) hipLaunchKernelGGL((qkvx_front_kernel<136, true>), grid, dim3(256), 0, st, xf, tf, a, T, tiles, eps, otp_range_word());
-        else hipLaunchKernelGGL((qkvx_front_kernel<136, false>), grid, dim3(256), 0, st, xf, tf, a, T, tiles, eps, otp_range_word());
-    }
+    auto sf = static_cast<const otp_f32x2*>(stats);
+    auto kern = C == 204 ? (stats ? (h1 ? qkvx_front_kernel<204, true, true> : qkvx_front_kernel<204, false, true>)
+                                  : (h1 ? qkvx_front_kernel<204, true> : qkvx_front_kernel<204, false>))
+                         : (stats ? (h1 ? qkvx_front_kernel<136, true, true> : qkvx_front_kernel<136, false, true>)
+                                  : (h1 ? qkvx_front_kernel<136, true> : qkvx_front_kernel<136, false>));
+    hipLaunchKernelGGL(kern, grid, dim3(256), 0, st, xf, tf, a, T, tiles, eps, otp_range_word(), sf);
     return otp_launch_status();
 }
 }
@@ -318,4 +336,16 @@
                                 const void* packed_v, void* q, void* k, void* v, int B, int C, int T, float eps, void* stream) {
     return dx_qkv_launch(x, table, packed_q, packed_k, packed_v, q, k, v, B, C, T, eps, stream, true);
 }
+
+extern "C" int otp_qkv_front_x3_ln(const void* x, const void* stats, const void* table, const void* packed_q, const void* packed_k,
+                                   const void* packed_v, void* q, void* k, void* v, int B, int C, int T, float eps, void* stream) {
+    if (!stats) return OTP_ERR_BAD_ARG;
+    return dx_qkv_launch(x, table, packed_q, packed_k, packed_v, q, k, v, B, C, T, eps, stream, false, stats);
+}
+
+extern "C" int otp_qkv_front_h1_ln(const void* x, const void* stats, const void* table, const void* packed_q, const void* packed_k,
+                                   const void* packed_v, void* q, void* k, void* v, int B, int C, int T, float eps, void* stream) {
+    if (!stats) return OTP_ERR_BAD_ARG;
+    return dx_qkv_launch(x, table, packed_q, packed_k, packed_v, q, k, v, B, C, T, eps, stream, true, stats);
+}
 #endif
diff --git a/otpose_amd/csrc/mlpx.hip b/otpose_amd/csrc/mlpx.hip
--- a/otpose_amd/csrc/mlpx.hip
+++ b/otpose_amd/csrc/mlpx.hip
@@ -73,12 +73,13 @@
     reinterpret_cast<otp_u32x4*>(packed)[idx] = o;
 }
 
-template <int C, int HID, int NTHR, bool LN, int NT, bool H1 = false>
+template <int C, int HID, int NTHR, bool LN, int NT, bool H1 = false, bool STATS = false>
 __device__ __forceinline__ void mlpx_pass(const float* __restrict__ x, const unsigned char* __restrict__ packed,
                                           const float* __restrict__ scale, const float* __restrict__ shift,
                                           const float* __restrict__ res, float* __restrict__ out, int T, size_t base, int tok0,
                                           unsigned char* lds, const float* __restrict__ ln_gamma,
-                                          const float* __restrict__ ln_beta, float ln_eps, unsigned* rflag) {
+                                          const float* __restrict__ ln_beta, float ln_eps, unsigned* rflag,
+                                          otp_f32x2* __restrict__ stats = nullptr, float stats_eps = 0.f) {
     constexpr int KS1 = mx_ks1(C), MT = mx_mt(C), HB = (HID + 31) / 32, PS = H1 ? 1 : 2;
     constexpr int W1B = mx_w1_bytes(C, PS), W2B = mx_w2_bytes(C, PS), BLKB = mx_block_bytes(C, PS);
     const int lane = threadIdx.x & 63, kq = lane >> 4, n = lane & 15;
@@ -220,6 +221,58 @@
 #pragma unroll
                 for (int i = 0; i < 4; ++i) bad |= otp_out_of_range(Y[mt][t][i]);
         otp_range_report(rflag, bad, OTP_RANGE_MLPX);
+    }
+    if constexpr (STATS) {
+        const int tokc = valid ? tok : T - NT;
+#pragma unroll
+        for (int mt = 0; mt < MT; ++mt)
+#pragma unroll
+            for (int i = 0; i < 4; ++i) {
+                const int c = 16 * mt + 4 * kq + i;
+                const bool live = 16 * mt + 12 + i < C || c < C;
+                const size_t o = base + (size_t)(live ? c : 0) * T + tokc;
+                const float sc = scale[live ? c : 0], sh = shift[live ? c : 0];
+                if (NT == 2) {
+                    const otp_f32x2 r = *reinterpret_cast<const otp_f32x2*>(res + o);
+                    Y[mt][0][i] = r.x + Y[mt][0][i] * sc + sh;
+                    Y[mt][NT - 1][i] = r.y + Y[mt][NT - 1][i] * sc + sh;
+                } else {
+                    Y[mt][0][i] = res[o] + Y[mt][0][i] * sc + sh;
+                }
+            }
+        constexpr float inv_c = 1.f / (float)C;
+#pragma unroll
+        for (int t = 0; t < NT; ++t) {
+            float s0 = 0.f;
+#pragma unroll
+            for (int mt = 0; mt < MT; ++mt)
+#pragma unroll
+                for (int i = 0; i < 4; ++i) s0 += (16 * mt + 12 + i < C || 16 * mt + 4 * kq + i < C) ? Y[mt][t][i] : 0.f;
+            const float m0 = otp_kslot_sum(s0) * inv_c;
+            float v0 = 0.f;
+#pragma unroll
+            for (int mt = 0; mt < MT; ++mt)
+#pragma unroll
+                for (int i = 0; i < 4; ++i) {
+                    const float d = (16 * mt + 12 + i < C || 16 * mt + 4 * kq + i < C) ? Y[mt][t][i] - m0 : 0.f;
+                    v0 += d * d;
+                }
+            const float r0 = 1.f / sqrtf(otp_kslot_sum(v0) * inv_c + stats_eps);
+            if (valid && kq == 0) stats[tok + t] = otp_f32x2{m0, r0};
+        }
+        if (!valid) return;
+#pragma unroll
+        for (int mt = 0; mt < MT; ++mt)
+#pragma unroll
+            for (int i = 0; i < 4; ++i) {
+                const int c = 16 * mt + 4 * kq + i;
+                if (c < C) {
+                    const size_t o = base + (size_t)c * T + tok;
+                    if (NT == 2) *reinterpret_cast<otp_f32x2*>(out + o) = otp_f32x2{Y[mt][0][i], Y[mt][NT - 1][i]};
+                    else out[o] = Y[mt][0][i];
+                }
+            }
+        return;
     }
     if (!valid) return;
 #pragma unroll
@@ -244,36 +297,41 @@
     }
 }
 
-template <int C, int HID, int WAVES, bool LN, int NT, bool H1 = false>
+template <int C, int HID, int WAVES, bool LN, int NT, bool H1 = false, bool STATS = false>
 __global__ __launch_bounds__(WAVES * 64, (NT == 1 && (C <= 136 || H1)) ? 4 : 2) void mlpx_kernel(
     const float* __restrict__ x, const unsigned char* __restrict__ packed, const float* __restrict__ scale,
     const float* __restrict__ shift, const float* __restrict__ res, float* __restrict__ out, int T, int tiles_per_b,
-    const float* __restrict__ ln_gamma, const float* __restrict__ ln_beta, float ln_eps, unsigned* rflag) {
+    const float* __restrict__ ln_gamma, const float* __restrict__ ln_beta, float ln_eps, unsigned* rflag,
+    otp_f32x2* __restrict__ stats, float stats_eps) {
     extern __shared__ __attribute__((aligned(16))) unsigned char mx_lds[];
     const int wave = threadIdx.x >> 6;
     const int b = blockIdx.x / tiles_per_b, tile = blockIdx.x - b * tiles_per_b;
-    mlpx_pass<C, HID, WAVES * 64, LN, NT, H1>(x, packed, scale, shift, res, out, T, (size_t)b * C * T,
-                                          tile * (WAVES * 16 * NT) + wave * 16 * NT, mx_lds, ln_gamma, ln_beta, ln_eps, rflag);
-}
-
-template <int C, int HID, bool LN>
+    mlpx_pass<C, HID, WAVES * 64, LN, NT, H1, STATS>(x, packed, scale, shift, res, out, T, (size_t)b * C * T,
+                                                 tile * (WAVES * 16 * NT) + wave * 16 * NT, mx_lds, ln_gamma, ln_beta, ln_eps, rflag,
+                                                 STATS ? stats + (size_t)b * T : nullptr, stats_eps);
+}
+
+template <int C, int HID, bool LN, bool STATS = false>
 __global__ __launch_bounds__(512, 2) void mlpx_balanced_kernel(
     const float* __restrict__ x, const unsigned char* __restrict__ packed, const float* __restrict__ scale,
     const float* __restrict__ shift, const float* __restrict__ res, float* __restrict__ out, int T, int wgs_per_b,
-    const float* __restrict__ ln_gamma, const float* __restrict__ ln_beta, float ln_eps, unsigned* rflag) {
+    const float* __restrict__ ln_gamma, const float* __restrict__ ln_beta, float ln_eps, unsigned* rflag,
+    otp_f32x2* __restrict__ stats, float stats_eps) {
     extern __shared__ __attribute__((aligned(16))) unsigned char mx_lds[];
     const int wave = __builtin_amdgcn_readfirstlane(threadIdx.x >> 6);
     const int b = blockIdx.x / wgs_per_b, part = blockIdx.x - b * wgs_per_b;
     const size_t base = (size_t)b * C * T;
     const int t0 = part * (27 * 16);
-    mlpx_pass<C, HID, 512, LN, 2>(x, packed, scale, shift, res, out, T, base, t0 + wave * 32, mx_lds, ln_gamma, ln_beta, ln_eps, rflag);
+    otp_f32x2* st = STATS ? stats + (size_t)b * T : nullptr;
+    mlpx_pass<C, HID, 512, LN, 2, false, STATS>(x, packed, scale, shift, res, out, T, base, t0 + wave * 32, mx_lds, ln_gamma, ln_beta,
+                                                ln_eps, rflag, st, stats_eps);
     if (wave < 3) {
-        mlpx_pass<C, HID, 512, LN, 2>(x, packed, scale, shift, res, out, T, base, t0 + (16 + 2 * wave) * 16, mx_lds, ln_gamma,
-                                      ln_beta, ln_eps, rflag);
+        mlpx_pass<C, HID, 512, LN, 2, false, STATS>(x, packed, scale, shift, res, out, T, base, t0 + (16 + 2 * wave) * 16, mx_lds,
+                                                    ln_gamma, ln_beta, ln_eps, rflag, st, stats_eps);
     } else {
         const int tile = wave == 3 ? 25 : (wave == 7 ? 26 : 18 + wave);
-        mlpx_pass<C, HID, 512, LN, 1>(x, packed, scale, shift, res, out, T, base, t0 + tile * 16, mx_lds, ln_gamma, ln_beta,
-                                      ln_eps, rflag);
+        mlpx_pass<C, HID, 512, LN, 1, false, STATS>(x, packed, scale, shift, res, out, T, base, t0 + tile * 16, mx_lds, ln_gamma,
+                                                    ln_beta, ln_eps, rflag, st, stats_eps);
     }
 }
 
@@ -317,8 +375,11 @@
 
 namespace {
 int mlpx_launch(const void* x, const void* packed, const void* scale, const void* shift, const void* res, void* out,
-                const void* ln_gamma, const void* ln_beta, float ln_eps, int B, int C, int HID, int T, void* stream, bool h1 = false) {
+                const void* ln_gamma, const void* ln_beta, float ln_eps, int B, int C, int HID, int T, void* stream, bool h1 = false,
+                void* stats = nullptr, float stats_eps = 0.f) {
     if (!x || !packed || !scale || !shift || !res || !out || B <= 0) return OTP_ERR_BAD_ARG;
+    if (stats && (!ln_gamma || reinterpret_cast<uintptr_t>(stats) & 15)) return OTP_ERR_BAD_ARG;
+    auto sp = static_cast<otp_f32x2*>(stats);
     if (h1 && !ln_gamma) return OTP_ERR_UNSUPPORTED;
     if (!otp_mlp_x3_supported(C, HID, T)) return OTP_ERR_UNSUPPORTED;
     if ((reinterpret_cast<uintptr_t>(x) | reinterpret_cast<uintptr_t>(res) | reinterpret_cast<uintptr_t>(out)) & 7 ||
@@ -330,11 +391,13 @@
         constexpr int WAVES = 8;
         const size_t lds204 = 2 * (size_t)mx_block_bytes(204, h1 ? 1 : 2);
         const int tiles = otp_ceil_div(T, WAVES * 16);
-        auto kern = h1 ? mlpx_kernel<204, 816, WAVES, true, 1, true>
-                       : (ln_gamma ? mlpx_kernel<204, 816, WAVES, true, 1> : mlpx_kernel<204, 816, WAVES, false, 1>);
+        auto kern = stats ? (h1 ? mlpx_kernel<204, 816, WAVES, true, 1, true, true> : mlpx_kernel<204, 816, WAVES, true, 1, false, true>)
+                    : h1  ? mlpx_kernel<204, 816, WAVES, true, 1, true>
+                          : (ln_gamma ? mlpx_kernel<204, 816, WAVES, true, 1> : mlpx_kernel<204, 816, WAVES, false, 1>);
         OTP_ALLOW_BIG_LDS(kern, lds204);
         hipLaunchKernelGGL(kern, dim3((unsigned)(B * tiles)), dim3(WAVES * 64), lds204, static_cast<hipStream_t>(stream), f(x), pk,
-                           f(scale), f(shift), f(res), static_cast<float*>(out), T, tiles, f(ln_gamma), f(ln_beta), ln_eps, otp_range_word());
+                           f(scale), f(shift), f(res), static_cast<float*>(out), T, tiles, f(ln_gamma), f(ln_beta), ln_eps, otp_range_word(),
+                           sp, stats_eps);
         return otp_launch_status();
     }
     const size_t lds = 2 * (size_t)mx_block_bytes(136, h1 ? 1 : 2);
@@ -345,27 +408,33 @@
     if (h1 || (nt1 && !bal_force)) {
         constexpr int WAVES = 8;
         const int tiles = otp_ceil_div(T, WAVES * 16);
-        auto kern = h1 ? mlpx_kernel<136, 544, WAVES, true, 1, true>
-                       : (ln_gamma ? mlpx_kernel<136, 544, WAVES, true, 1> : mlpx_kernel<136, 544, WAVES, false, 1>);
+        auto kern = stats ? (h1 ? mlpx_kernel<136, 544, WAVES, true, 1, true, true> : mlpx_kernel<136, 544, WAVES, true, 1, false, true>)
+                    : h1  ? mlpx_kernel<136, 544, WAVES, true, 1, true>
+                          : (ln_gamma ? mlpx_kernel<136, 544, WAVES, true, 1> : mlpx_kernel<136, 544, WAVES, false, 1>);
         OTP_ALLOW_BIG_LDS(kern, lds);
         hipLaunchKernelGGL(kern, dim3((unsigned)(B * tiles)), dim3(WAVES * 64), lds, static_cast<hipStream_t>(stream), f(x), pk,
-                           f(scale), f(shift), f(res), static_cast<float*>(out), T, tiles, f(ln_gamma), f(ln_beta), ln_eps, otp_range_word());
+                           f(scale), f(shift), f(res), static_cast<float*>(out), T, tiles, f(ln_gamma), f(ln_beta), ln_eps, otp_range_word(),
+                           sp, stats_eps);
         return otp_launch_status();
     }
     if (!bal_off && T % (27 * 16) == 0 && (bal_force || (long)B * (T / (27 * 16)) >= 192)) {
-        auto bk = ln_gamma ? mlpx_balanced_kernel<136, 544, true> : mlpx_balanced_kernel<136, 544, false>;
+        auto bk = stats ? mlpx_balanced_kernel<136, 544, true, true>
+                        : (ln_gamma ? mlpx_balanced_kernel<136, 544, true> : mlpx_balanced_kernel<136, 544, false>);
         OTP_ALLOW_BIG_LDS(bk, lds);
         const int per_b = T / (27 * 16);
         hipLaunchKernelGGL(bk, dim3((unsigned)(B * per_b)), dim3(512), lds, static_cast<hipStream_t>(stream), f(x), pk,
-                           f(scale), f(shift), f(res), static_cast<float*>(out), T, per_b, f(ln_gamma), f(ln_beta), ln_eps, otp_range_word());
+                           f(scale), f(shift), f(res), static_cast<float*>(out), T, per_b, f(ln_gamma), f(ln_beta), ln_eps, otp_range_word(),
+                           sp, stats_eps);
         return otp_launch_status();
     }
     constexpr int WAVES = 8;
     const int tiles = otp_ceil_div(T, WAVES * 32);
-    auto kern = ln_gamma ? mlpx_kernel<136, 544, WAVES, true, 2> : mlpx_kernel<136, 544, WAVES, false, 2>;
+    auto kern = stats ? mlpx_kernel<136, 544, WAVES, true, 2, false, true>
+                      : (ln_gamma ? mlpx_kernel<136, 544, WAVES, true, 2> : mlpx_kernel<136, 544, WAVES, false, 2>);
     OTP_ALLOW_BIG_LDS(kern, lds);
     hipLaunchKernelGGL(kern, dim3((unsigned)(B * tiles)), dim3(WAVES * 64), lds, static_cast<hipStream_t>(stream), f(x), pk,
-                       f(scale), f(shift), f(res), static_cast<float*>(out), T, tiles, f(ln_gamma), f(ln_beta), ln_eps, otp_range_word());
+                       f(scale), f(shift), f(res), static_cast<float*>(out), T, tiles, f(ln_gamma), f(ln_beta), ln_eps, otp_range_word(),
+                           sp, stats_eps);
     return otp_launch_status();
 }
 }
@@ -386,3 +455,17 @@
     if (!ln_gamma || !ln_beta) return OTP_ERR_BAD_ARG;
     return mlpx_launch(y, packed, scale, shift, y, out, ln_gamma, ln_beta, ln_eps, B, C, HID, T, stream, true);
 }
+
+extern "C" int otp_ln_mlp_x3_stats(const void* y, const void* ln_gamma, const void* ln_beta, float ln_eps, const void* packed,
+                                   const void* scale, const void* shift, void* out, int B, int C, int HID, int T, void* stats,
+                                   float stats_eps, void* stream) {
+    if (!ln_gamma || !ln_beta || !stats) return OTP_ERR_BAD_ARG;
+    return mlpx_launch(y, packed, scale, shift, y, out, ln_gamma, ln_beta, ln_eps, B, C, HID, T, stream, false, stats, stats_eps);
+}
+
+extern "C" int otp_ln_mlp_h1_stats(const void* y, const void* ln_gamma, const void* ln_beta, float ln_eps, const void* packed,
+                                   const void* scale, const void* shift, void* out, int B, int C, int HID, int T, void* stats,
+                                   float stats_eps, void* stream) {
+    if (!ln_gamma || !ln_beta || !stats) return OTP_ERR_BAD_ARG;
+    return mlpx_launch(y, packed, scale, shift, y, out, ln_gamma, ln_beta, ln_eps, B, C, HID, T, stream, true, stats, stats_eps);
+}
diff --git a/otpose_amd/engine.py b/otpose_amd/engine.py
--- a/otpose_amd/engine.py
+++ b/otpose_amd/engine.py
@@ -58,6 +58,7 @@
     conv_log: bool = False
     poison: Optional[Tuple[int, int]] = None
     te_serial: bool = False
+    ln1_fold = False
 
     @classmethod
     def from_env(cls) -> "Routes":
@@ -65,7 +66,7 @@
         on = lambda name: env("OTPOSE_" + name, "1") != "0"
         x3 = env("OTPOSE_CONV_MATH", "x3") != "f32"
         poison = env("OTPOSE_POISON")
-        return cls(use_graph=on("HIP_GRAPH"), use_winograd=on("WINOGRAD"), use_x3=x3, use_dcn_fused=x3 and on("DCN_FUSED"),
+        r = cls(use_graph=on("HIP_GRAPH"), use_winograd=on("WINOGRAD"), use_x3=x3, use_dcn_fused=x3 and on("DCN_FUSED"),
                    use_s8=x3 and on("S8"), use_flow_fused=on("FLOW_FUSED"), use_small_conv=on("SMALL_CONV"),
                    use_fused_mlp=on("FUSED_MLP"), fuse_shortcut=on("FUSE_SHORTCUT"), fuse_upsample=on("FUSE_UPSAMPLE"),
                    use_dense_cc=on("DENSE_CC"), use_qkv_front=on("QKV_FRONT"), use_pointx=x3 and on("POINTX"),
@@ -75,6 +76,8 @@
                    s8_stride2=on("S8_STRIDE2"), t1_s8=on("T1_S8"), l1_s8=on("L1_S8"), l1_pair=on("L1_PAIR"), stem_x3=on("STEM_X3"),
                    chain_modules=on("CHAIN_MODULES"), up_any_width=on("UP_ANY_WIDTH"), conv_log=bool(env("OTPOSE_CONV_LOG")),
                    poison=tuple(int(v) for v in poison.split(":")) if poison else None, te_serial=env("OTPOSE_TE_SERIAL") == "1")
+        object.__setattr__(r, "ln1_fold", env("OTPOSE_LN1_FOLD", "0") == "1")
+        return r
 
     @property
     def lazy_nchw(self) -> bool:
@@ -116,6 +119,7 @@
         self.ops: List[Callable] = []
         self._pair_s8 = {}
         self.l1_pairs = 0
+        self.ln1_folds = 0
         self._aux = {}
         self._keep = []
         self._bufs = []
@@ -757,7 +761,7 @@
         b, c, t = t3.shape
         return View(t3.view(b, c, 1, t))
 
-    def tblock(self, blk, x, stride):
+    def tblock(self, blk, x, stride, stats=None, nxt=None):
         B, C, T = x.shape
         To = T if stride == 1 else (T + 2 - 3) // 2 + 1
         L = self.lib
@@ -770,25 +774,34 @@
             self.call(L.otp_flow_front, "otp_flow_front", *ops.flow_front_args(x, fp, q, k, v, blk.ln1.eps))
             self.chan_attn(q, k, v, att, a)
             self.call(L.otp_flow_back, "otp_flow_back", *ops.flow_back_args(x, att, bp, out, blk.mlp[0].out_channels, blk.ln2.eps))
-            return out
-        ln1 = self.new(B, C, T)
+            return out, None
+        p = self.dev_param
         skip = self.new(B, C, To) if stride > 1 else None
-        p = self.dev_param
-        self.call(L.otp_ln_channel, "otp_ln_channel", hip.ptr(x), hip.ptr(p(blk.ln1.weight)), hip.ptr(p(blk.ln1.bias)),
-                  hip.ptr(ln1), hip.ptr(skip), B, C, T, blk.ln1.eps)
+        if stats is None:
+            ln1 = self.new(B, C, T)
+            self.call(L.otp_ln_channel, "otp_ln_channel", hip.ptr(x), hip.ptr(p(blk.ln1.weight)), hip.ptr(p(blk.ln1.bias)),
+                      hip.ptr(ln1), hip.ptr(skip), B, C, T, blk.ln1.eps)
         q, k, v = self.new(B, C, To), self.new(B, C, To), self.new(B, C, To)
         dx3 = r.use_dense_cc and r.use_x3 and ops.dense_x3_supported(C, To)
         dense = dx3 or (r.use_dense_cc and ops.dense_cc_supported(C, To))
         if dense:
             packs = [ops.pack_dense_cc(m.weight.to(self.dev), None, m.bias.to(self.dev), x3=dx3)
                      for m in (a.query, a.key, a.value)]
+        fold = r.ln1_fold and dx3 and stride == 1 and r.use_qkv_front
+        assert stats is None or fold
         if dense and stride == 1 and r.use_qkv_front:
             table = ops.pack_qkv_table(*[p(t) for t in (a.query_conv.weight, a.key_conv.weight, a.value_conv.weight,
                                                          a.query_norm.weight, a.query_norm.bias, a.key_norm.weight,
-                                                         a.key_norm.bias, a.value_norm.weight, a.value_norm.bias)])
+                                                         a.key_norm.bias, a.value_norm.weight, a.value_norm.bias)],
+                                       *((p(blk.ln1.weight), p(blk.ln1.bias)) if stats is not None else ()))
             self._keep += [table, *packs]
-            self.call((L.otp_qkv_front_h1 if self.half_products else L.otp_qkv_front_x3) if dx3 else L.otp_qkv_front, "otp_qkv_front",
-                      *ops.qkv_front_args(ln1, table, packs, (q, k, v), a.query_norm.eps))
+            if stats is not None:
+                self.ln1_folds += 1
+                self.call(L.otp_qkv_front_h1_ln if self.half_products else L.otp_qkv_front_x3_ln, "otp_qkv_front_ln",
+                          *ops.qkv_front_ln_args(x, stats, table, packs, (q, k, v), a.query_norm.eps))
+            else:
+                self.call((L.otp_qkv_front_h1 if self.half_products else L.otp_qkv_front_x3) if dx3 else L.otp_qkv_front,
+                          "otp_qkv_front", *ops.qkv_front_args(ln1, table, packs, (q, k, v), a.query_norm.eps))
         else:
             qn, kn, vn = self.new(B, C, To), self.new(B, C, To), self.new(B, C, To)
             self.call(L.otp_dwconv_ln3, "otp_dwconv_ln3", hip.ptr(ln1), hip.ptr(p(a.query_conv.weight)),
@@ -826,10 +839,16 @@
             scd = dev(sm).contiguous()
             shd = (dev(blk.mlp[3].bias) * scd).contiguous()
             self._keep += [packed, scd, shd]
+            largs = (y, p(blk.ln2.weight), p(blk.ln2.bias), blk.ln2.eps, packed, scd, shd, out, hid)
+            if fold and mlp_x3 and nxt is not None:
+                out_stats = self.new(B, To, 2)
+                self.call(L.otp_ln_mlp_h1_stats if self.half_products else L.otp_ln_mlp_x3_stats, "otp_ln_mlp_x3_stats",
+                          *ops.ln_mlp_stats_args(*largs, out_stats, nxt.ln1.eps))
+                return out, out_stats
             fn, name = ((L.otp_ln_mlp_h1 if self.half_products else L.otp_ln_mlp_x3, "otp_ln_mlp_x3") if mlp_x3
                         else (L.otp_ln_mlp_fused, "otp_ln_mlp_fused"))
-            self.call(fn, name, *ops.ln_mlp_args(y, p(blk.ln2.weight), p(blk.ln2.bias), blk.ln2.eps, packed, scd, shd, out, hid))
-            return out
+            self.call(fn, name, *ops.ln_mlp_args(*largs))
+            return out, None
         ln2 = self.new(B, C, To)
         self.call(L.otp_ln_channel, "otp_ln_channel", hip.ptr(y), hip.ptr(p(blk.ln2.weight)), hip.ptr(p(blk.ln2.bias)),
                   hip.ptr(ln2), None, B, C, To, blk.ln2.eps)
@@ -837,7 +856,7 @@
         self.conv(self.v3(ln2), blk.mlp[0].weight, self.v3(hdn), bias=blk.mlp[0].bias, act=ACT_GELU)
         self.conv(self.v3(hdn), blk.mlp[3].weight, self.v3(out), scale=sm,
                   shift=blk.mlp[3].bias.detach() * sm.to(blk.mlp[3].bias.device), res=self.v3(y))
-        return out
+        return out, None
 
     def chan_attn(self, q, k, v, att, a):
         B, C, T = q.shape
@@ -848,11 +867,12 @@
     def conv_transformer(self, ct, x, stacked):
         _, C, T = x.shape
         L = self.lib
-        for blk in ct.stem:
-            x = self.tblock(blk, x, 1)
+        stats = None
+        for i, blk in enumerate(ct.stem):
+            x, stats = self.tblock(blk, x, 1, stats, ct.stem[i + 1] if i + 1 < len(ct.stem) else None)
         self.call(L.otp_upsample_linear, "otp_upsample_linear", *ops.upsample_linear_args(x, stacked, 1, 0))
         for i, blk in enumerate(ct.branch):
-            x = self.tblock(blk, x, 2)
+            x, _ = self.tblock(blk, x, 2)
             f = 2 ** (i + 1)
             if x.shape[2] * f != T:
                 raise RuntimeError("heat-map size must make every pyramid level divide evenly (T % 4 == 0)")
diff --git a/otpose_amd/hip.py b/otpose_amd/hip.py
--- a/otpose_amd/hip.py
+++ b/otpose_amd/hip.py
@@ -64,6 +64,8 @@
     "otp_ln_mlp_h1": (c_int, [c_void_p] * 3 + [c_float] + [c_void_p] * 4 + [c_int] * 4 + [c_void_p]),
     "otp_dense_h1": (c_int, [ctypes.POINTER(c_void_p)] * 4 + [c_int] * 4 + [c_void_p]),
     "otp_qkv_front_h1": (c_int, [c_void_p] * 8 + [c_int] * 3 + [c_float, c_void_p]),
+    "otp_ln_mlp_h1_stats": (c_int, [c_void_p] * 3 + [c_float] + [c_void_p] * 4 + [c_int] * 4 + [c_void_p, c_float, c_void_p]),
+    "otp_qkv_front_h1_ln": (c_int, [c_void_p] * 9 + [c_int] * 3 + [c_float, c_void_p]),
     "otp_h16_upsample_add": (c_int, [ctypes.POINTER(c_void_p), ctypes.POINTER(c_int), c_int, c_void_p, c_void_p] + [c_int] * 5 + [c_void_p]),
     "otp_mdcn_forward": (c_int, [c_void_p] * 6 + [c_int] * 12 + [c_float, c_float, c_int, c_void_p]),
     "otp_mdcn_forward_ex": (c_int, [c_void_p] * 6 + [c_int] * 15 + [c_float, c_float, c_int, c_void_p]),
@@ -183,6 +185,8 @@
     "otp_flow_front": (c_int, [c_void_p] * 5 + [c_int] * 3 + [c_float, c_void_p]),
     "otp_flow_back": (c_int, [c_void_p] * 4 + [c_int] * 4 + [c_float, c_void_p]),
     "otp_ln_mlp_x3": (c_int, [c_void_p] * 3 + [c_float] + [c_void_p] * 4 + [c_int] * 4 + [c_void_p]),
+    "otp_ln_mlp_x3_stats": (c_int, [c_void_p] * 3 + [c_float] + [c_void_p] * 4 + [c_int] * 4 + [c_void_p, c_float, c_void_p]),
+    "otp_qkv_front_x3_ln": (c_int, [c_void_p] * 9 + [c_int] * 3 + [c_float, c_void_p]),
     "otp_chan_attn": (c_int, [c_void_p] * 4 + [c_void_p, c_size_t] + [c_int] * 4 + [c_float, c_void_p]),
     "otp_chan_attn_splits": (c_int, [c_int, c_int]),
     "otp_chan_attn_scores": (c_int, [c_void_p] * 3 + [c_int] * 3 + [c_void_p]),
diff --git a/otpose_amd/ops.py b/otpose_amd/ops.py
--- a/otpose_amd/ops.py
+++ b/otpose_amd/ops.py
@@ -647,6 +647,11 @@
     return (hip.ptr(y), hip.ptr(gamma), hip.ptr(beta), eps, hip.ptr(packed), hip.ptr(scale), hip.ptr(shift), hip.ptr(out), b, c, hid, t)
 
 
+def ln_mlp_stats_args(y, gamma, beta, eps, packed, scale, shift, out, hid, stats, stats_eps):
+    assert tuple(stats.shape) == (y.shape[0], y.shape[2], 2) and stats.dtype == torch.float32 and stats.is_contiguous()
+    return (*ln_mlp_args(y, gamma, beta, eps, packed, scale, shift, out, hid), hip.ptr(stats), stats_eps)
+
+
 def ln_mlp_fused(y, gamma, beta, eps, packed, scale, shift, out=None, hid=None, stream=None, entry="otp_ln_mlp_fused"):
     _require_gpu(y, packed)
     _check_f32(y)
@@ -831,7 +836,7 @@
     return out_s8
 
 
-def pack_qkv_table(dwq, dwk, dwv, gq, bq, gk, bk, gv, bv):
+def pack_qkv_table(dwq, dwk, dwv, gq, bq, gk, bk, gv, bv, ln1_gamma=None, ln1_beta=None):
     ts = [t.detach().float().contiguous() for t in (dwq, dwk, dwv, gq, bq, gk, bk, gv, bv)]
     _require_gpu(*ts)
     c = ts[3].numel()
@@ -839,6 +844,10 @@
     table = torch.empty(L.otp_qkv_front_table_bytes(c) // 4, dtype=torch.float32, device=ts[0].device)
     hip.check(L.otp_qkv_front_pack_table(*[hip.ptr(t) for t in ts], hip.ptr(table), c, hip.stream_of(ts[0])),
               "otp_qkv_front_pack_table")
+    if ln1_gamma is not None:
+        rows = table.view(3, c, 8)
+        rows[:, :, 6] = ln1_gamma.detach().float()
+        rows[:, :, 7] = ln1_beta.detach().float()
     return table
 
 
@@ -847,9 +856,20 @@
     return (hip.ptr(x), hip.ptr(table), *[hip.ptr(p) for p in packs], *[hip.ptr(o) for o in outs], b, c, t, eps)
 
 
-def qkv_front(x, table, packs, eps=1e-5, outs=None, stream=None, x3=False, half=False):
+def qkv_front_ln_args(x, stats, table, packs, outs, eps):
+    b, c, t = x.shape
+    assert tuple(stats.shape) == (b, t, 2) and stats.dtype == torch.float32 and stats.is_contiguous()
+    return (hip.ptr(x), hip.ptr(stats), hip.ptr(table), *[hip.ptr(p) for p in packs], *[hip.ptr(o) for o in outs], b, c, t, eps)
+
+
+def qkv_front(x, table, packs, eps=1e-5, outs=None, stream=None, x3=False, half=False, stats=None):
     _require_gpu(x, table)
     outs = [torch.empty_like(x) for _ in range(3)] if outs is None else outs
+    if stats is not None:
+        assert x3, "the ln-on-load front end exists for the split-product kernels only"
+        fn = hip.lib().otp_qkv_front_h1_ln if half else hip.lib().otp_qkv_front_x3_ln
+        _launch(fn, "otp_qkv_front_ln", qkv_front_ln_args(x, stats, table, packs, outs, eps), x, stream)
+        return outs
     fn = (hip.lib().otp_qkv_front_h1 if half else hip.lib().otp_qkv_front_x3) if x3 else hip.lib().otp_qkv_front
     _launch(fn, "otp_qkv_front", qkv_front_args(x, table, packs, outs, eps), x, stream)
     return outs
@@ -944,7 +964,16 @@
     return mlp_fused(x, packed, scale, shift, res, out, hid, stream, "otp_mlp_x3")
 
 
-def ln_mlp_x3(y, gamma, beta, eps, packed, scale, shift, out=None, hid=None, stream=None, half=False):
+def ln_mlp_x3(y, gamma, beta, eps, packed, scale, shift, out=None, hid=None, stream=None, half=False, stats=None, stats_eps=1e-5):
+    if stats is not None:
+        _require_gpu(y, packed, stats)
+        _check_f32(y)
+        hid = 4 * y.shape[1] if hid is None else hid
+        out = torch.empty_like(y) if out is None else out
+        entry = "otp_ln_mlp_h1_stats" if half else "otp_ln_mlp_x3_stats"
+        _launch(getattr(hip.lib(), entry), entry, ln_mlp_stats_args(y, gamma, beta, eps, packed, scale, shift, out, hid, stats, stats_eps),
+                y, stream)
+        return out
     return ln_mlp_fused(y, gamma, beta, eps, packed, scale, shift, out, hid, stream, "otp_ln_mlp_h1" if half else "otp_ln_mlp_x3")
 
 
```

Measured after the change: 3249 frames/s, median of 2. About the same (-0.0%).
